# awaelchli/torch-optical-flow

Measured on AMD Instinct MI355X. Metric: image-pairs/sec + corr-lookup HBM GB/s, RAFT 12-iter @ Sintel 1024×436, higher is better.
Workload: dtype corr + convs split-fp16 (22-bit operands: fp16 hi + lo, 3 f16 MFMA per product, fp32 accumulate); lookup fp32; 1 GPU; raft-12iter-sintel-436x1024; pairs_per_gpu=8, global_batch=8, iters=12, padded=440x1024, parallelism=pairs sharded over 1 GPU(s), conv_benchmark=True, update_impl=split, hip_graph=True, steps_in_flight=1, full=False

## Files before the change

include/oflow.h:

```cpp
#ifndef OFLOW_H_
#define OFLOW_H_

#ifdef __cplusplus
extern "C" {
#endif

#define OFLOW_ABI_VERSION 1

#define OFLOW_OK 0
#define OFLOW_E_NULL (-1)
#define OFLOW_E_SHAPE (-2)
#define OFLOW_E_LEVELS (-3)
#define OFLOW_E_TINY (-4)
#define OFLOW_E_RADIUS (-5)
#define OFLOW_E_MODE (-6)
#define OFLOW_E_ALIGN (-7)

#define OFLOW_MAX_LEVELS 8
#define OFLOW_MAX_RADIUS 7

#define OFLOW_INTERP_BILINEAR 0
#define OFLOW_INTERP_NEAREST 1
#define OFLOW_INTERP_BICUBIC 2
#define OFLOW_PAD_ZEROS 0
#define OFLOW_PAD_BORDER 1
#define OFLOW_PAD_REFLECTION 2

#define OFLOW_IN_S32 0
#define OFLOW_IN_F32_NORM 1
#define OFLOW_IN_F32 2
#define OFLOW_IN_IMG7S2 3
#define OFLOW_IN_FLOW7 4
#define OFLOW_EPI_FLOW_HEAD 3

int oflow_abi_version(void);
const char* oflow_status_string(int status);

int oflow_corr_pyramid_dims(int H, int W, int num_levels, int* level_h, int* level_w);

int oflow_corr_pyramid_f32(const float* d_fmap1, const float* d_fmap2, int B, int C, int H, int W,
                           int num_levels, float* const* d_levels, void* stream);

int oflow_corr_lookup_f32(const float* const* d_levels, const int* level_h, const int* level_w,
                          int num_levels, const float* d_coords, int B, int H, int W, int radius,
                          float* d_out, void* stream);

long long oflow_corr_tiled_level_floats(int H_l, int W_l);
int oflow_corr_pyramid_tiled_f32(const float* d_fmap1, const float* d_fmap2, int B, int C, int H, int W,
                                 int num_levels, float* const* d_levels, void* stream);
int oflow_corr_pyramid_tiled_s32(const void* d_fmap1_s32, const void* d_fmap2_s32, int B, int C, int H, int W,
                                 int num_levels, float* const* d_levels, void* stream);
int oflow_corr_lookup_tiled_f32(const float* const* d_levels, const int* level_h, const int* level_w,
                                int num_levels, const float* d_coords, int B, int H, int W, int radius,
                                float* d_out, void* stream);
int oflow_corr_untile_f32(const float* d_tiled, float* d_out, long long Q, int H_l, int W_l, void* stream);

int oflow_grid_warp_f32(const float* d_frame, const float* d_flow, int B, int C, int H, int W, int mode,
                        int padding_mode, int align_corners, float* d_out, void* stream);

int oflow_grid_sample_f32(const float* d_input, const float* d_grid, int B, int C, int H, int W, int Ho, int Wo,
                          int mode, int padding_mode, int align_corners, float* d_out, void* stream);

int oflow_corr_otf_prepare_f16(const float* d_fmap1, const float* d_fmap2, int B, int C, int H, int W,
                               int num_levels, void* d_f1h, void* const* d_f2h, float* d_scratch, void* stream);
int oflow_corr_lookup_otf_f16(const void* d_f1h, const void* const* d_f2h, const int* level_h, const int* level_w,
                              int num_levels, const float* d_coords, int B, int C, int H, int W, int radius,
                              float* d_out, void* stream);

int oflow_bias_act_f32(const float* d_x, long long sx, const float* d_bias, float* d_y0, long long sy0, float* d_y1,
                       long long sy1, int B, int C, int P, int activation, float scale, void* stream);
int oflow_gru_reset_f32(const float* d_zr, long long szr, const float* d_br, const float* d_h, long long sh,
                        float* d_rh, long long srh, int B, int CH, int P, void* stream);
int oflow_gru_blend_f32(const float* d_zr, long long szr, const float* d_bz, const float* d_q, long long sq,
                        const float* d_bq, float* d_h, long long sh, int B, int CH, int P, void* stream);

int oflow_conv_s32(const void* d_x, long long x_pixel_stride, int in_groups, const void* d_wpack, int n_pad,
                   const float* d_wscale, const float* d_bias, int N, int B, int H, int W, int kh, int kw, int block_n,
                   int epilogue, int activation, float out_scale, void* d_y0, long long y0_pixel_stride, void* d_y1,
                   long long y1_pixel_stride, float* d_f32, long long f32_batch_stride, long long f32_channel_stride,
                   int f32_accumulate, float* d_gru_h, float* d_gru_z, int gru_channels, void* stream);
int oflow_pack_s32_f32(const float* d_x, long long x_batch_stride, int C, int B, int H, int W, int activation,
                       int dst_channel, void* d_y0, long long y0_pixel_stride, void* d_y1, long long y1_pixel_stride,
                       float* d_nhwc, int nhwc_pixel_stride, void* stream);
int oflow_flow_prep_s32(const float* d_coords, int B, int H, int W, void* d_patches, void* d_flow0,
                        long long flow0_pixel_stride, void* d_flow1, long long flow1_pixel_stride, void* stream);
int oflow_flow_head_col2im_f32(const float* d_y, const float* d_bias, int B, int H, int W, float* d_coords, void* stream);
int oflow_flow_head_finish_f32(const float* d_partial, int slabs, const float* d_bias, int B, int H, int W,
                               float* d_coords, void* d_flow0, long long flow0_pixel_stride, void* d_flow1,
                               long long flow1_pixel_stride, void* stream);

int oflow_normalize_images_f32(const float* d_x0, const float* d_x1, long long n, float* d_y0, float* d_y1, void* stream);

int oflow_replicate_pad_f32(const float* const* d_src, float* const* d_dst, int count, long long planes, int H, int W,
                            int top, int bottom, int left, int right, void* stream);

int oflow_set_range_flag(unsigned int* d_flag);

int oflow_range_flag_exchange(unsigned int* d_flag, unsigned int* d_out, void* stream);

int oflow_timing_event_create(void** ev);
int oflow_timing_event_destroy(void* ev);
int oflow_timing_event_record(void* ev, void* stream, int external);
int oflow_timing_event_elapsed_ms(void* start, void* end, float* ms);

int oflow_flow_head2_s32(const void* d_x, long long x_pixel_stride, int in_groups, const float* d_weight,
                         const float* d_bias, int B, int H, int W, float* d_coords, void* stream);
int oflow_flow_head2_tiled_s32(const void* d_x, long long x_pixel_stride, int in_groups, const float* d_wr,
                               const float* d_bias, int B, int H, int W, float* d_coords, void* stream);
int oflow_corr_lookup_tiled_nhwc_f32(const float* const* d_levels, const int* level_h, const int* level_w, int num_levels,
                                     const float* d_coords, int B, int H, int W, int radius, float* d_out, int row_floats,
                                     void* stream);
int oflow_corr_lookup_convc1_s32(const float* const* d_levels, const int* level_h, const int* level_w, int num_levels,
                                 const float* d_coords, int B, int H, int W, int radius, const void* d_wpack,
                                 const float* d_wscale, const float* d_bias, void* d_y, long long y_pixel_stride,
                                 void* stream);

int oflow_conv_s32_ex(const void* d_x, long long x_pixel_stride, int in_groups, const void* d_wpack, int n_pad,
                      const float* d_wscale, const float* d_bias, int N, int B, int H, int W, int kh, int kw,
                      int block_n, int epilogue, int activation, float out_scale, void* d_y0, long long y0_pixel_stride,
                      void* d_y1, long long y1_pixel_stride, float* d_f32, long long f32_batch_stride,
                      long long f32_channel_stride, int f32_accumulate, float* d_gru_h, float* d_gru_z,
                      int gru_channels, float* d_nhwc, int nhwc_pixel_stride, float* d_stats, const void* d_res,
                      long long res_pixel_stride, int res_activation, int s2d, void* stream);
int oflow_conv_s32_ex2(const void* d_x, long long x_pixel_stride, int in_groups, const void* d_wpack, int n_pad,
                       const float* d_wscale, const float* d_bias, int N, int B, int H, int W, int kh, int kw,
                       int block_n, int epilogue, int activation, float out_scale, void* d_y0, long long y0_pixel_stride,
                       void* d_y1, long long y1_pixel_stride, float* d_f32, long long f32_batch_stride,
                       long long f32_channel_stride, int f32_accumulate, float* d_gru_h, float* d_gru_z,
                       int gru_channels, float* d_nhwc, int nhwc_pixel_stride, float* d_stats, const void* d_res,
                       long long res_pixel_stride, int res_activation, int s2d, int in_format,
                       const float* d_in_scale, const float* d_in_shift, void* stream);
int oflow_conv_s32_ex3(const void* d_x, long long x_pixel_stride, int in_groups, const void* d_wpack, int n_pad,
                       const float* d_wscale, const float* d_bias, int N, int B, int H, int W, int kh, int kw,
                       int block_n, int epilogue, int activation, float out_scale, void* d_y0, long long y0_pixel_stride,
                       void* d_y1, long long y1_pixel_stride, float* d_f32, long long f32_batch_stride,
                       long long f32_channel_stride, int f32_accumulate, float* d_gru_h, float* d_gru_z,
                       int gru_channels, float* d_nhwc, int nhwc_pixel_stride, float* d_stats, const void* d_res,
                       long long res_pixel_stride, int res_activation, int s2d, int in_format,
                       const float* d_in_scale, const float* d_in_shift, const float* d_addend,
                       long long addend_pixel_stride, void* stream);
int oflow_conv_s32_ex4(const void* d_x, long long x_pixel_stride, int in_groups, const void* d_wpack, int n_pad,
                       const float* d_wscale, const float* d_bias, int N, int B, int H, int W, int kh, int kw,
                       int block_n, int epilogue, int activation, float out_scale, void* d_y0, long long y0_pixel_stride,
                       void* d_y1, long long y1_pixel_stride, float* d_f32, long long f32_batch_stride,
                       long long f32_channel_stride, int f32_accumulate, float* d_gru_h, float* d_gru_z,
                       int gru_channels, float* d_nhwc, int nhwc_pixel_stride, float* d_stats, const void* d_res,
                       long long res_pixel_stride, int res_activation, int s2d, int in_format,
                       const float* d_in_scale, const float* d_in_shift, const float* d_addend,
                       long long addend_pixel_stride, const void* d_wfrag, void* stream);
int oflow_conv_s32_ex5(const void* d_x, long long x_pixel_stride, int in_groups, const void* d_wpack, int n_pad,
                       const float* d_wscale, const float* d_bias, int N, int B, int H, int W, int kh, int kw,
                       int block_n, int epilogue, int activation, float out_scale, void* d_y0, long long y0_pixel_stride,
                       void* d_y1, long long y1_pixel_stride, float* d_f32, long long f32_batch_stride,
                       long long f32_channel_stride, int f32_accumulate, float* d_gru_h, float* d_gru_z,
                       int gru_channels, float* d_nhwc, int nhwc_pixel_stride, float* d_stats, const void* d_res,
                       long long res_pixel_stride, int res_activation, int s2d, int in_format,
                       const float* d_in_scale, const float* d_in_shift, const float* d_addend,
                       long long addend_pixel_stride, const void* d_wfrag, float* d_ksplit_slab,
                       unsigned* d_ksplit_ctr, long long ksplit_tiles, void* stream);
int oflow_conv_s32_ex6(const void* d_x, long long x_pixel_stride, int in_groups, const void* d_wpack, int n_pad,
                       const float* d_wscale, const float* d_bias, int N, int B, int H, int W, int kh, int kw,
                       int block_n, int epilogue, int activation, float out_scale, void* d_y0, long long y0_pixel_stride,
                       void* d_y1, long long y1_pixel_stride, float* d_f32, long long f32_batch_stride,
                       long long f32_channel_stride, int f32_accumulate, float* d_gru_h, float* d_gru_z,
                       int gru_channels, float* d_nhwc, int nhwc_pixel_stride, float* d_stats, const void* d_res,
                       long long res_pixel_stride, int res_activation, int s2d, int in_format,
                       const float* d_in_scale, const float* d_in_shift, const float* d_addend,
                       long long addend_pixel_stride, const void* d_wfrag, float* d_ksplit_slab,
                       unsigned* d_ksplit_ctr, long long ksplit_tiles, const float* d_fh_weights, float* d_fh_partial,
                       int fh_slabs, void* stream);
int oflow_stem_patches_s32(const float* d_img, int B, int C, int H, int W, void* d_out, int out_groups, void* stream);
int oflow_norm_stats_finalize(const float* d_partials, int B, int tiles, int n_pad, int C, double eps, float* d_alpha,
                              float* d_beta, void* stream);
int oflow_norm_apply_s32(const float* d_x, int C, int B, int H, int W, const float* d_alpha, const float* d_beta,
                         int activation, int res_mode, const void* d_res, long long res_pixel_stride, const float* d_x2,
                         const float* d_alpha2, const float* d_beta2, int res_activation, int s2d, void* d_y,
                         long long y_pixel_stride, void* stream);

int oflow_convex_upsample_f32(const float* d_flow, const float* d_mask, int B, int H, int W, float* d_out, void* stream);

int oflow_corr_lookup_backward_f32(const float* d_grad_out, const float* d_coords, int B, int H, int W, int radius,
                                   float* const* d_grad_levels, const int* level_h, const int* level_w, int num_levels,
                                   void* stream);
int oflow_corr_pyramid_grad_combine_f32(float* const* d_grad_levels, const int* level_h, const int* level_w,
                                        int num_levels, long long Q, void* stream);
int oflow_corr_fmap_grad_f32(const float* d_fmap1, const float* d_fmap2, const float* d_g0, int B, int C, int N,
                             float scale, float* d_grad_f1, float* d_grad_f2, void* stream);

int oflow_grid_warp_backward_f32(const float* d_grad_out, const float* d_frame, const float* d_flow, int B, int C, int H,
                                 int W, int mode, int padding_mode, int align_corners, float* d_grad_frame,
                                 float* d_grad_flow, void* stream);
int oflow_grid_sample_backward_f32(const float* d_grad_out, const float* d_input, const float* d_grid, int B, int C,
                                   int H, int W, int Ho, int Wo, int mode, int padding_mode, int align_corners,
                                   float* d_grad_input, float* d_grad_grid, void* stream);

#define OFLOW_FLOW_STATS_CHUNKS 128
#define OFLOW_FLOW2RGB_BAKER 0
#define OFLOW_FLOW2RGB_HSV 1
#define OFLOW_FLOW2RGB_MEISTER 2
int oflow_flow_stats_f32(const float* d_flow, int B, int H, int W, int clip, float clip_lo, float clip_hi,
                         int invert_y, float* d_partials, void* stream);
int oflow_flow2rgb_f32(const float* d_flow, int B, int H, int W, int method, int clip, float clip_lo, float clip_hi,
                       int invert_y, int have_denom, float denom, const float* d_partials, float* d_rgb, void* stream);
int oflow_flow_pack_f32(const float* d_flow, int B, int H, int W, int channels, int flip_rows, float* d_out,
                        void* stream);

#define OFLOW_FLOW_METRICS_PARTIALS 1024
#define OFLOW_MAX_PREDS 32
#define OFLOW_VALID_NONE 0
#define OFLOW_VALID_F32 1
#define OFLOW_VALID_U8 2
int oflow_flow_error_stats_f32(const float* d_pred, long long pred_sb, long long pred_sc, long long pred_sh,
                               const float* d_target, long long target_sb, long long target_sc, long long target_sh,
                               const void* d_valid, int valid_kind, long long valid_sb, long long valid_sh, int B, int H,
                               int W, float abs_threshold, float rel_threshold, float max_flow, float* d_epe_map,
                               double* d_workspace, double* d_accum, void* stream);
int oflow_sequence_loss_f32(const float* const* d_preds, int n_preds, const float* weights, const float* d_flow_gt,
                            const void* d_valid, int valid_kind, int B, int H, int W, float max_flow,
                            double* d_workspace, float* d_loss, double* d_stats, void* stream);
int oflow_sequence_loss_backward_f32(const float* d_grad_out, const float* const* d_preds, float* const* d_grads,
                                     int n_preds, const float* weights, const float* d_flow_gt, const void* d_valid,
                                     int valid_kind, int B, int H, int W, float max_flow, void* stream);

#ifdef __cplusplus
}
#endif

#endif
```

torch-optical-flow_amd/csrc/conv_s32.hip:

```cpp
#include "oflow_internal.h"

namespace oflow {
namespace {

typedef _Float16 half8 __attribute__((ext_vector_type(8)));
typedef float f32x16 __attribute__((ext_vector_type(16)));
typedef unsigned int u32x4 __attribute__((ext_vector_type(4)));

__device__ __forceinline__ int swz(int row) { return (row >> 1) & 7; }
#ifndef OFLOW_BREG_RING
#define OFLOW_BREG_RING 2
#endif
#ifndef OFLOW_VSLIDE
#define OFLOW_VSLIDE 1
#endif
#ifndef OFLOW_XCD_MAP
#define OFLOW_XCD_MAP 0
#endif
#ifndef OFLOW_STEM_SINGLE_A
#define OFLOW_STEM_SINGLE_A 1
#endif
#ifndef OFLOW_PAD_ROWS
#define OFLOW_PAD_ROWS 1
#endif
#ifndef OFLOW_HALO_DB
#define OFLOW_HALO_DB 0
#endif

constexpr int kTY = 4, kTX = 32;

#ifdef OFLOW_ABLATE
#define OFLOW_ABL(bit) ((a.exp_flags & (bit)) != 0)
#else
#define OFLOW_ABL(bit) false
#endif
constexpr int kAinGroups = 4;


struct ConvArgs {
  const uint8_t* x;
  long long xps;
  int kg;
  const uint8_t* w;
  int npad;
  const float* wsc;
  const float* bias;
  int N;
  int B, H, W, tiles_x, tiles_y;
  int act;
  float oscale;
  uint8_t* y0;
  long long y0ps;
  uint8_t* y1;
  long long y1ps;
  float* f;
  long long fbs, fcs;
  int faccum;
  float* h;
  float* z;
  int gch;
  const float* add;
  long long addps;
  float* fn;
  int fnps;
  float* stats;
  const uint8_t* res;
  long long resps;
  int res_act;
  int s2d;
  const float* ia;
  const float* ib;
  int ain;
  int cin;
  int wbytes;
  const uint8_t* wf;
  int exp_flags;
  float* ks_slab;
  unsigned* ks_ctr;
  long long ks_tiles;
  const float* fhw;
  float* fhy;
};
constexpr int kEpiFlowHead = OFLOW_EPI_FLOW_HEAD;
constexpr int kInS32 = OFLOW_IN_S32, kInF32Norm = OFLOW_IN_F32_NORM, kInF32 = OFLOW_IN_F32, kInImg = OFLOW_IN_IMG7S2,
              kInFlow = OFLOW_IN_FLOW7;
constexpr int kImgC = 3, kImgK = 7, kImgRows = (kTY - 1) * 2 + kImgK, kImgCols = (kTX - 1) * 2 + kImgK;
constexpr int kImgHalf = (kImgCols + 1) / 2, kImgPitch = 2 * kImgHalf, kImgPlane = kImgRows * kImgPitch;

__device__ __forceinline__ float sigmoid_hw(float v) {
  return __builtin_amdgcn_rcpf(1.0f + __builtin_amdgcn_exp2f(v * -1.4426950408889634f));
}
__device__ __forceinline__ float tanh_hw(float v) {
  return 1.0f - 2.0f * __builtin_amdgcn_rcpf(__builtin_amdgcn_exp2f(v * 2.8853900817779268f) + 1.0f);
}

__device__ __forceinline__ float act_fn(float v, int act) {
  if (act == 1) return v < 0.f ? 0.f : v;
  if (act == 2) return 1.0f / (1.0f + expf(-v));
  if (act == 3) return tanhf(v);
  return v;
}

__device__ __forceinline__ void split8(const float* v, half8& hi, half8& lo) { split_vec(v, hi, lo); }

__device__ __forceinline__ void store_s32(uint8_t* y, long long ps, long long P, int n, int N, const float* v, float& gm) {
  uint8_t* line = y + P * ps + (long long)(n >> 5) * 128 + ((n & 31) >> 3) * 16;
  if (n + 8 <= N) {
    half8 hi, lo;
    split8(v, hi, lo);
    gm = fmaxf(gm, fmaxf(fmaxf(fmaxf(fabsf(v[0]), fabsf(v[1])), fmaxf(fabsf(v[2]), fabsf(v[3]))),
                         fmaxf(fmaxf(fabsf(v[4]), fabsf(v[5])), fmaxf(fabsf(v[6]), fabsf(v[7])))));
    *reinterpret_cast<half8*>(line) = hi;
    *reinterpret_cast<half8*>(line + 64) = lo;
  } else {
    _Float16* hp = reinterpret_cast<_Float16*>(line);
    _Float16* lp = reinterpret_cast<_Float16*>(line + 64);
#pragma unroll
    for (int j = 0; j < 8; ++j) {
      if (n + j < N) {
        gm = fmaxf(gm, fabsf(v[j]));
        _Float16 h_, l_;
        split_f16(v[j], h_, l_);
        hp[j] = h_;
        lp[j] = l_;
      }
    }
  }
}

typedef __attribute__((address_space(4))) const float cfloat;
template <int T0, int T1>
__device__ __forceinline__ void flow_head_partials(const float* tp, cfloat* w, float* yp, long long plane, bool in) {
  constexpr int NO = 2 * (T1 - T0);
  float acc[2][NO];
#pragma unroll
  for (int j = 0; j < NO; ++j) acc[0][j] = acc[1][j] = 0.f;
  float wn[2][NO];
#pragma unroll
  for (int e = 0; e < 2; ++e)
#pragma unroll
    for (int j = 0; j < NO; ++j) wn[e][j] = w[e * 18 + 2 * T0 + j];
  float2 tn = *reinterpret_cast<const float2*>(tp);
#pragma unroll
  for (int e = 0; e < 2; ++e)
#pragma unroll
    for (int j = 0; j < NO; ++j) asm volatile("" : "+s"(wn[e][j]));
  asm volatile("" : "+v"(tn.x), "+v"(tn.y));
#pragma unroll 2
  for (int c0 = 0; c0 < 64; c0 += 2) {
    float wc[2][NO];
#pragma unroll
    for (int e = 0; e < 2; ++e)
#pragma unroll
      for (int j = 0; j < NO; ++j) wc[e][j] = wn[e][j];
    const float2 t = tn;
    const int c1 = c0 + 2 < 64 ? c0 + 2 : c0;
#pragma unroll
    for (int e = 0; e < 2; ++e)
#pragma unroll
      for (int j = 0; j < NO; ++j) wn[e][j] = w[(c1 + e) * 18 + 2 * T0 + j];
    tn = *reinterpret_cast<const float2*>(tp + c1);
    __builtin_amdgcn_sched_barrier(0);
#pragma unroll
    for (int j = 0; j < NO; ++j) {
      acc[0][j] = fmaf(t.x, wc[0][j], acc[0][j]);
      acc[1][j] = fmaf(t.y, wc[1][j], acc[1][j]);
    }
    __builtin_amdgcn_sched_barrier(0);
#pragma unroll
    for (int e = 0; e < 2; ++e)
#pragma unroll
      for (int j = 0; j < NO; ++j) asm volatile("" : "+s"(wn[e][j]));
    asm volatile("" : "+v"(tn.x), "+v"(tn.y));
  }
  if (in) {
#pragma unroll
    for (int j = 0; j < NO; ++j) yp[(2 * T0 + j) * plane] = acc[0][j] + acc[1][j];
  }
}

template <int KH, int KW, int BN, int WM, int WN, int EPI, int TY = kTY, int AIN = kInS32, bool BREG = false, int BD = 1>
__global__ __launch_bounds__(64 * WM * WN, WM * WN == 8 ? 1 : 2) void conv_s32_kernel(ConvArgs a) {
  constexpr int NTH = 64 * WM * WN;
  constexpr int T = KH * KW;
  constexpr int BM = TY * kTX;
  constexpr int PH = KH / 2, PW = KW / 2;
  constexpr int HY = TY + KH - 1, HX = kTX + KW - 1, NPIX = HY * HX;
  constexpr int AITEMS = NPIX * 8, APER = (AITEMS + NTH - 1) / NTH;
  constexpr int BITEMS = BN * 8, BPER = (BITEMS + NTH - 1) / NTH;
  constexpr int MT = TY / WM;
  constexpr int NT = BN / WN / 32;
  static_assert((WM * WN == 4 || WM * WN == 8) && MT >= 1 && NT >= 1, "bad wave grid");
  static_assert(NTH % 8 == 0, "an A item's 16-B chunk is tid & 7");
  constexpr bool WIN = AIN == kInImg || AIN == kInFlow;
  constexpr int WC = AIN == kInFlow ? 2 : kImgC, WS = AIN == kInFlow ? 1 : 2;
  constexpr int WROWS = (kTY - 1) * WS + kImgK, WCOLS = (kTX - 1) * WS + kImgK;
  constexpr int WHALF = WS == 2 ? (WCOLS + 1) / 2 : WCOLS, WPITCH = WS == 2 ? 2 * WHALF : WCOLS;
  constexpr int WPLANE = WROWS * WPITCH;
  constexpr int WKPAD = AIN == kInFlow ? 128 : 160;
  constexpr int WAPER = WIN ? BM * 4 / NTH : 1;
  static_assert(!WIN || (BM * 4) % NTH == 0, "window items");
  static_assert(AIN != kInImg || (WHALF == kImgHalf && WPITCH == kImgPitch && WPLANE == kImgPlane), "stem window");
  constexpr bool ADB = (T == 1) && !(WIN && OFLOW_STEM_SINGLE_A);
  constexpr int RS = 128;
  constexpr int RSA = (BREG || OFLOW_PAD_ROWS) ? 144 : RS, RSB = OFLOW_PAD_ROWS ? 144 : RS;
  constexpr int A_BYTES = NPIX * RSA, B_BYTES = BN * RSB;
  static_assert(!BREG || (T > 1 && (WM == 1 || WM == 2 || WM == 4) && BN == 32 * WN && AIN == kInS32),
                "register-direct B: T > 1, WM x WN waves of one 32-channel tile each");
  constexpr bool HDB = BREG && OFLOW_HALO_DB;
  constexpr int MAIN_BYTES = ((ADB || HDB) ? 2 : 1) * A_BYTES + (BREG ? 0 : 2 * B_BYTES);
  constexpr int TS = BN + 4;
  constexpr int EPI_BYTES = BM * TS * 4;
  constexpr int LDS_BYTES = MAIN_BYTES > EPI_BYTES ? MAIN_BYTES : EPI_BYTES;
  constexpr int kImgZero = WC * WPLANE;
  constexpr int IMG_FLOATS = (kImgZero + 1 + 3) & ~3;
  constexpr int AFF_BYTES = AIN == kInF32Norm ? kAinGroups * 32 * 8
                            : WIN ? IMG_FLOATS * 4 + WKPAD * 4
                            : 0;
  static_assert(!WIN || (T == 1 && TY == kTY), "window input: 1x1 geometry over the patch channels, 4-row tiles");
  __shared__ __attribute__((aligned(16))) uint8_t smem[LDS_BYTES + AFF_BYTES];
  __shared__ float2 sSB[BN];
  __shared__ float3 sStat[EPI == 0 ? WM * BN : 1];
  float2* sAff = reinterpret_cast<float2*>(smem + LDS_BYTES);
  float* sImg = reinterpret_cast<float*>(smem + LDS_BYTES);
  int* sKoff = reinterpret_cast<int*>(smem + LDS_BYTES + (WIN ? IMG_FLOATS * 4 : 0));
  uint8_t* sA = smem;
  uint8_t* sB = smem + (ADB ? 2 : 1) * A_BYTES;

  const int tid = threadIdx.x, lane = tid & 63, wave = tid >> 6;
  const int wm = wave / WN, wn = wave % WN;
  const int r = lane & 31, hh = lane >> 5;
  if constexpr (BREG) {
    if (a.ks_slab != nullptr) {
      const int z = blockIdx.z;
      a.x += (long long)z * a.kg * 128;
      a.wf += (long long)z * a.kg * T * a.npad * 128;
    }
  }
  auto aswz = [](int p) { return (BREG || OFLOW_PAD_ROWS) ? 0 : swz(p); };
  auto bswz = [](int n) { return OFLOW_PAD_ROWS ? 0 : swz(n); };

  int tile, cblk;
  if constexpr (OFLOW_XCD_MAP) {
    const int nblk = a.npad / BN, ntiles = a.tiles_x * a.tiles_y * a.B, bid = blockIdx.x;
    const int full = (ntiles >> 3) * 8 * nblk;
    if (bid < full) {
      const int grp = bid / (8 * nblk), rem = bid - grp * 8 * nblk;
      cblk = rem >> 3;
      tile = grp * 8 + (rem & 7);
    } else {
      const int ntail = ntiles & 7, rem = bid - full;
      cblk = rem / ntail;
      tile = (ntiles & ~7) + (rem - cblk * ntail);
    }
  } else {
    tile = blockIdx.x;
    cblk = blockIdx.y;
  }
  const int tx0 = (tile % a.tiles_x) * kTX;
  tile /= a.tiles_x;
  const int ty0 = (tile % a.tiles_y) * TY;
  const int b = tile / a.tiles_y;
  const int n0 = cblk * BN;
  const long long pix0 = (long long)b * a.H * a.W;

  u32x4 ra[APER], rb[BPER];
  const __amdgpu_buffer_rsrc_t rsA = __builtin_amdgcn_make_buffer_rsrc(
      const_cast<uint8_t*>(a.x + pix0 * a.xps), (short)0, (int)((long long)a.H * a.W * a.xps), 0x00020000);
  const __amdgpu_buffer_rsrc_t rsB =
      __builtin_amdgcn_make_buffer_rsrc(const_cast<uint8_t*>(a.w), (short)0, a.wbytes, 0x00020000);
  auto a_off = [&](int s_, int& col) {
    int t_ = tid;
    asm volatile("" : "+v"(t_));
    const int item = (AITEMS % NTH == 0) ? t_ + s_ * NTH : min(t_ + s_ * NTH, AITEMS - 1);
    const int p = item >> 3, c = item & 7;
    const int gy = ty0 - PH + p / HX, gx = tx0 - PW + p % HX;
    const int cy = min(max(gy, 0), a.H - 1), cx = min(max(gx, 0), a.W - 1);
    col = c * 16;
    return (cy * a.W + cx) * (int)a.xps + (AIN == kInF32 ? 0 : c * 16);
  };
  unsigned aok = 0u;
#pragma unroll
  for (int s_ = 0; s_ < APER; ++s_) {
    const int item = (AITEMS % NTH == 0) ? tid + s_ * NTH : min(tid + s_ * NTH, AITEMS - 1);
    const int p = item >> 3;
    const int gy = ty0 - PH + p / HX, gx = tx0 - PW + p % HX;
    const bool ok = static_cast<unsigned>(gy) < static_cast<unsigned>(a.H) && static_cast<unsigned>(gx) < static_cast<unsigned>(a.W);
    aok |= (ok ? 1u : 0u) << s_;
  }
  int boff[BPER];
#pragma unroll
  for (int s_ = 0; s_ < BPER; ++s_) boff[s_] = (n0 + (tid + s_ * NTH) / 8) * 128 + ((tid + s_ * NTH) & 7) * 16;
#define OFLOW_LOAD_A(RA, G)                                                                                          \
  if constexpr (!WIN) _Pragma("unroll") for (int s_ = 0; s_ < APER; ++s_) {                                        \
    int col_;                                                                                                        \
    const int off_ = a_off(s_, col_);                                                                                \
    if constexpr (AIN == kInF32)    \
      RA[s_] = __builtin_amdgcn_raw_buffer_load_b128(rsA, off_ + min((G) * 128 + col_, a.cin * 4 - 16), 0, 0);      \
    else                                                                                                             \
      RA[s_] = __builtin_amdgcn_raw_buffer_load_b128(rsA, off_, (G) * 128, 0);                                      \
  }
#define OFLOW_WRITE_A(RA, BUF, G)                                                                                    \
  if (!OFLOW_ABL(4)) {                                                                                               \
  float amx_ = 0.f;                                                                                                  \
  float2 af4_[4];                                                                                                    \
  if constexpr (AIN == kInF32Norm) _Pragma("unroll") for (int e_ = 0; e_ < 4; ++e_)                                  \
    af4_[e_] = sAff[(G) * 32 + 4 * (tid & 7) + e_];                                                                  \
  if constexpr (WIN) {                                                                                               \
                                                                                                        \
    _Pragma("unroll") for (int s_ = 0; s_ < WAPER; ++s_) {                                                           \
      const int item = tid + s_ * NTH;                                                                               \
      const int p = item % BM, cp = item / BM;                                                                       \
      const int pb_ = WS * (p >> 5) * WPITCH + (p & 31);                                                             \
      const int4 k0_ = *reinterpret_cast<const int4*>(sKoff + (G) * 32 + 8 * cp);                                    \
      const int4 k1_ = *reinterpret_cast<const int4*>(sKoff + (G) * 32 + 8 * cp + 4);                                \
      const int kov_[8] = {k0_.x, k0_.y, k0_.z, k0_.w, k1_.x, k1_.y, k1_.z, k1_.w};                                  \
      float v8_[8];                                                                                                  \
      _Pragma("unroll") for (int e_ = 0; e_ < 8; ++e_) {                                                             \
        v8_[e_] = sImg[kov_[e_] < 0 ? kImgZero : pb_ + kov_[e_]];                                                    \
        amx_ = fmaxf(amx_, fabsf(v8_[e_]));                                                                          \
      }                                                                                                              \
      half8 h8_, l8_;                                                                                                \
      split_vec(v8_, h8_, l8_);                                                                                      \
      uint8_t* rw_ = sA + (BUF) * A_BYTES + p * RSA;                                                                 \
      *reinterpret_cast<half8*>(rw_ + ((cp ^ aswz(p)) << 4)) = h8_;                                                  \
      *reinterpret_cast<half8*>(rw_ + (((4 + cp) ^ aswz(p)) << 4)) = l8_;                                            \
    }                                                                                                                \
  } else                                                                                                             \
  _Pragma("unroll") for (int s_ = 0; s_ < APER; ++s_) {                                                              \
    const int item = tid + s_ * NTH;                                                                            \
                                                     \
    const int p = item >> 3, c = item & 7;                                                                           \
    if (AITEMS % NTH == 0 || item < AITEMS) {                                                                   \
      if constexpr (AIN != kInS32) {                                                                                 \
                   \
        typedef _Float16 half4_ __attribute__((ext_vector_type(4)));                                                 \
        half4_ h4 = {0, 0, 0, 0}, l4 = {0, 0, 0, 0};                                                                 \
        if (((aok >> s_) & 1u) && (AIN != kInF32 || (G) * 32 + 4 * c < a.cin)) {                                     \
          const float* fv = reinterpret_cast<const float*>(&RA[s_]);                                                 \
          float mx_ = 0.f, v4_[4];                                                                                   \
          _Pragma("unroll") for (int e_ = 0; e_ < 4; ++e_) {                                                         \
            float v_ = fv[e_];                                                                                       \
            if constexpr (AIN == kInF32Norm) {                                                                       \
              const float2 af = af4_[e_];                                                                            \
              v_ = v_ * af.x + af.y;                                                                                 \
              v_ = v_ < 0.f ? 0.f : v_;                                                                              \
            }                                                                                                        \
            mx_ = fmaxf(mx_, fabsf(v_));                                                                             \
            v4_[e_] = v_;                                                                                            \
          }                                                                                                          \
          split_vec(v4_, h4, l4);                                                                                    \
          amx_ = fmaxf(amx_, mx_);                                                                                   \
        }                                                                                                            \
        uint8_t* rw_ = sA + (BUF) * A_BYTES + p * RSA + (c & 1) * 8;                                                 \
        *reinterpret_cast<half4_*>(rw_ + (((c >> 1) ^ aswz(p)) << 4)) = h4;                                          \
        *reinterpret_cast<half4_*>(rw_ + (((4 + (c >> 1)) ^ aswz(p)) << 4)) = l4;                                    \
      } else {                                                                                                       \
        *reinterpret_cast<u32x4*>(sA + (BUF) * A_BYTES + p * RSA + ((c ^ aswz(p)) << 4)) =                          \
            ((aok >> s_) & 1u) ? RA[s_] : u32x4{0u, 0u, 0u, 0u};                                                     \
      }                                                                                                              \
    }                                                                                                                \
  }                                                                                                                  \
  if constexpr (AIN != kInS32) range_guard(amx_);                                                                    \
  }
#define OFLOW_LOAD_B(RB, STEP)                                                                                       \
  _Pragma("unroll") for (int s_ = 0; s_ < BPER; ++s_) {                                                              \
    const int item = tid + s_ * NTH;                                                                            \
    if (BITEMS % NTH == 0 || item < BITEMS)                                                                     \
      RB[s_] = __builtin_amdgcn_raw_buffer_load_b128(rsB, boff[s_], (STEP) * a.npad * 128, 0);                      \
  }
#define OFLOW_WRITE_B(RB, BUF)                                                                                       \
  if (!OFLOW_ABL(32)) _Pragma("unroll") for (int s_ = 0; s_ < BPER; ++s_) {                                          \
    const int item = tid + s_ * NTH;                                                                            \
    const int n = item >> 3, c = item & 7;                                                                           \
    if (BITEMS % NTH == 0 || item < BITEMS)                                                                     \
      *reinterpret_cast<u32x4*>(sB + (BUF) * B_BYTES + n * RSB + ((c ^ bswz(n)) << 4)) = RB[s_];                    \
  }
#define OFLOW_READ_OPS(AH, AL, BH, BL, I, S_)                                                                        \
  {                                                                                                                  \
    const int ii_ = (I);                                                                                              \
    const int t_ = ii_ % T, ky_ = t_ / KW, kx_ = t_ - ky_ * KW;                                                       \
    const uint8_t* bufA_ = sA + (ADB ? (ii_ & 1) * A_BYTES : 0);                                                      \
    const uint8_t* bufB_ = sB + (ii_ & 1) * B_BYTES;                                                                  \
    const int chi_ = 2 * (S_) + hh, clo_ = 4 + 2 * (S_) + hh;                                                        \
    _Pragma("unroll") for (int mt_ = 0; mt_ < MT; ++mt_) {                                                           \
      const int p_ = (wm * MT + mt_ + ky_) * HX + r + kx_;                                                           \
      const uint8_t* row_ = bufA_ + p_ * RSA;                                                                        \
      AH[mt_] = *reinterpret_cast<const half8*>(row_ + ((chi_ ^ aswz(p_)) << 4));                                    \
      AL[mt_] = *reinterpret_cast<const half8*>(row_ + ((clo_ ^ aswz(p_)) << 4));                                    \
    }                                                                                                                \
    _Pragma("unroll") for (int nt_ = 0; nt_ < NT; ++nt_) {                                                           \
      const int n_ = wn * (BN / WN) + nt_ * 32 + r;                                                                  \
      const uint8_t* row_ = bufB_ + n_ * RSB;                                                                        \
      BH[nt_] = *reinterpret_cast<const half8*>(row_ + ((chi_ ^ bswz(n_)) << 4));                                    \
      BL[nt_] = *reinterpret_cast<const half8*>(row_ + ((clo_ ^ bswz(n_)) << 4));                                    \
    }                                                                                                                \
  }
#define OFLOW_MFMAS(AH, AL, BH, BL)                                                                                  \
  if (!OFLOW_ABL(2)) _Pragma("unroll") for (int mt = 0; mt < MT; ++mt)                                               \
    _Pragma("unroll") for (int nt = 0; nt < NT; ++nt) {                                                              \
      acc[mt][nt] = __builtin_amdgcn_mfma_f32_32x32x16_f16(AH[mt], BL[nt], acc[mt][nt], 0, 0, 0);                    \
      acc[mt][nt] = __builtin_amdgcn_mfma_f32_32x32x16_f16(AL[mt], BH[nt], acc[mt][nt], 0, 0, 0);                    \
      acc[mt][nt] = __builtin_amdgcn_mfma_f32_32x32x16_f16(AH[mt], BH[nt], acc[mt][nt], 0, 0, 0);                    \
    }

  f32x16 acc[MT][NT];
#pragma unroll
  for (int i = 0; i < MT; ++i)
#pragma unroll
    for (int j = 0; j < NT; ++j)
#pragma unroll
      for (int e = 0; e < 16; ++e) acc[i][j][e] = 0.f;

  const int S = a.kg * T;
  for (int c = tid; c < BN; c += NTH) {
    const int n = min(n0 + c, a.N - 1);
    sSB[c] = make_float2(a.wsc[n], a.bias ? a.bias[n] : 0.f);
  }
  if constexpr (AIN == kInF32Norm) {
    for (int e = tid; e < a.kg * 32; e += NTH)
      sAff[e] = make_float2(a.ia[(long long)b * a.kg * 32 + e], a.ib[(long long)b * a.kg * 32 + e]);
    __syncthreads();
  }
  if constexpr (AIN == kInImg) {
    const float* img = reinterpret_cast<const float*>(a.x) + (long long)b * kImgC * (2 * a.H) * (2 * a.W);
    const int iy0 = 2 * ty0 - kImgK / 2, ix0 = 2 * tx0 - kImgK / 2;
    constexpr int IMG_N = kImgC * kImgRows * kImgCols, IMG_PER = (IMG_N + NTH - 1) / NTH;
    if (a.exp_flags & 1) {
      for (int e = tid; e < IMG_N; e += NTH) {
        const int ch = e / (kImgRows * kImgCols), rem = e - ch * (kImgRows * kImgCols);
        const int ry = rem / kImgCols, rx = rem - ry * kImgCols;
        const int iy = iy0 + ry, ix = ix0 + rx;
        float v = 0.f;
        if (static_cast<unsigned>(iy) < static_cast<unsigned>(2 * a.H) && static_cast<unsigned>(ix) < static_cast<unsigned>(2 * a.W))
          v = img[((long long)ch * (2 * a.H) + iy) * (2 * a.W) + ix];
        sImg[ch * kImgPlane + ry * kImgPitch + (rx & 1) * kImgHalf + (rx >> 1)] = v;
      }
    } else {
    float iv[IMG_PER];
    int io[IMG_PER];
#pragma unroll
    for (int s_ = 0; s_ < IMG_PER; ++s_) {
      const int e = min(tid + s_ * NTH, IMG_N - 1);
      const int ch = e / (kImgRows * kImgCols), rem = e - ch * (kImgRows * kImgCols);
      const int ry = rem / kImgCols, rx = rem - ry * kImgCols;
      const int iy = iy0 + ry, ix = ix0 + rx;
      const bool in = static_cast<unsigned>(iy) < static_cast<unsigned>(2 * a.H) && static_cast<unsigned>(ix) < static_cast<unsigned>(2 * a.W);
      const int cy = min(max(iy, 0), 2 * a.H - 1), cx = min(max(ix, 0), 2 * a.W - 1);
      const float v = img[((long long)ch * (2 * a.H) + cy) * (2 * a.W) + cx];
      iv[s_] = in ? v : 0.f;
      io[s_] = ch * kImgPlane + ry * kImgPitch + (rx & 1) * kImgHalf + (rx >> 1);
    }
#pragma unroll
    for (int s_ = 0; s_ < IMG_PER; ++s_)
      if (tid + s_ * NTH < IMG_N) sImg[io[s_]] = iv[s_];
    }
  }
  if constexpr (AIN == kInFlow) {
    const float* co = reinterpret_cast<const float*>(a.x) + (long long)b * 2 * a.H * a.W;
    const int iy0 = ty0 - kImgK / 2, ix0 = tx0 - kImgK / 2;
    constexpr int FL_N = 2 * WROWS * WCOLS, FL_PER = (FL_N + NTH - 1) / NTH;
    float iv[FL_PER];
    int io[FL_PER];
#pragma unroll
    for (int s_ = 0; s_ < FL_PER; ++s_) {
      const int e = min(tid + s_ * NTH, FL_N - 1);
      const int ch = e / (WROWS * WCOLS), rem = e - ch * (WROWS * WCOLS);
      const int ry = rem / WCOLS, rx = rem - ry * WCOLS;
      const int iy = iy0 + ry, ix = ix0 + rx;
      const bool in = static_cast<unsigned>(iy) < static_cast<unsigned>(a.H) && static_cast<unsigned>(ix) < static_cast<unsigned>(a.W);
      const int cy = min(max(iy, 0), a.H - 1), cx = min(max(ix, 0), a.W - 1);
      const float v = co[((long long)ch * a.H + cy) * a.W + cx] - static_cast<float>(ch == 0 ? ix : iy);
      iv[s_] = in ? v : 0.f;
      io[s_] = ch * WPLANE + ry * WPITCH + rx;
    }
#pragma unroll
    for (int s_ = 0; s_ < FL_PER; ++s_)
      if (tid + s_ * NTH < FL_N) sImg[io[s_]] = iv[s_];
  }
  if constexpr (WIN) {
    for (int k = tid; k < WKPAD; k += NTH) {
      const int t = k / WC, ch = k - t * WC;
      const int ky = t / kImgK, kx = t - ky * kImgK;
      sKoff[k] = t < kImgK * kImgK
                     ? ch * WPLANE + ky * WPITCH + (WS == 2 ? (kx & 1) * WHALF + (kx >> 1) : kx)
                     : -1;
    }
    if (tid == 0) sImg[kImgZero] = 0.f;
    __syncthreads();
  }
  if constexpr (BREG) {
  const __amdgpu_buffer_rsrc_t rsW =
      __builtin_amdgcn_make_buffer_rsrc(const_cast<uint8_t*>(a.wf), (short)0, a.wbytes, 0x00020000);
  const int wlane = ((n0 >> 5) + wn) * 4096 + lane * 16;
  const int wstep = a.npad * 128;
  constexpr int RING = (T == 5 && KH == 5 && EPI == 0) ? 2 : OFLOW_BREG_RING;
  u32x4 bq[RING][4];
  auto load_b = [&](u32x4 (&d)[4], int step) {
#pragma unroll
    for (int e = 0; e < 4; ++e) d[e] = __builtin_amdgcn_raw_buffer_load_b128(rsW, wlane + e * 1024, step * wstep, 0);
  };
#define OFLOW_READ_A(AH, AL, I, S_)                                                                                   \
  {                                                                                                                  \
    const int ii_ = (I);                                                                                              \
    const int t_ = ii_ % T, ky_ = t_ / KW, kx_ = t_ - ky_ * KW;                                                       \
    const int chi_ = 2 * (S_) + hh, clo_ = 4 + 2 * (S_) + hh;                                                        \
    const uint8_t* sAb_ = sA + (HDB && ((ii_ / T) & 1) ? A_BYTES : 0);           \
    _Pragma("unroll") for (int mt_ = 0; mt_ < MT; ++mt_) {                                                           \
      const int p_ = (wm * MT + mt_ + ky_) * HX + r + kx_;                                                           \
      const uint8_t* row_ = sAb_ + p_ * RSA;                                                                         \
      AH[mt_] = *reinterpret_cast<const half8*>(row_ + (chi_ << 4));                                                 \
      AL[mt_] = *reinterpret_cast<const half8*>(row_ + (clo_ << 4));                                                 \
    }                                                                                                                \
  }
#define OFLOW_MFMAS_R(AH, AL, BC, S_)                                                                                 \
  if (!OFLOW_ABL(2)) _Pragma("unroll") for (int mt = 0; mt < MT; ++mt) {                                             \
    const half8 bh_ = __builtin_bit_cast(half8, BC[2 * (S_)]), bl_ = __builtin_bit_cast(half8, BC[2 * (S_) + 1]);     \
    acc[mt][0] = __builtin_amdgcn_mfma_f32_32x32x16_f16(AH[mt], bl_, acc[mt][0], 0, 0, 0);                           \
    acc[mt][0] = __builtin_amdgcn_mfma_f32_32x32x16_f16(AL[mt], bh_, acc[mt][0], 0, 0, 0);                           \
    acc[mt][0] = __builtin_amdgcn_mfma_f32_32x32x16_f16(AH[mt], bh_, acc[mt][0], 0, 0, 0);                           \
  }
#pragma unroll
  for (int q = 0; q < RING; ++q) load_b(bq[q], q < S ? q : S - 1);
  OFLOW_LOAD_A(ra, 0);
  OFLOW_WRITE_A(ra, 0, 0);
  OFLOW_LOAD_A(ra, a.kg > 1 ? 1 : 0);
  __syncthreads();
  constexpr int GPB = (T % RING == 0) ? 1 : RING;
  constexpr bool VSLIDE = OFLOW_VSLIDE && KW == 1 && KH > 1 && WM == 1 && !(EPI == 0 && KH == 5);
  if constexpr (VSLIDE) {
    constexpr int NR = MT + KH - 1;
    half8 V[NR][2][2];
    auto rd = [&](int hr, int sub, int grp) {
      const uint8_t* row_ = sA + (HDB && (grp & 1) ? A_BYTES : 0) + (hr * HX + r) * RSA;
      V[hr][sub][0] = *reinterpret_cast<const half8*>(row_ + ((2 * sub + hh) << 4));
      V[hr][sub][1] = *reinterpret_cast<const half8*>(row_ + ((4 + 2 * sub + hh) << 4));
    };
    auto mf = [&](int ky, int sub, u32x4 (&bc)[4]) {
      if (OFLOW_ABL(2)) return;
      const half8 bh_ = __builtin_bit_cast(half8, bc[2 * sub]), bl_ = __builtin_bit_cast(half8, bc[2 * sub + 1]);
#pragma unroll
      for (int mt = 0; mt < MT; ++mt) {
        acc[mt][0] = __builtin_amdgcn_mfma_f32_32x32x16_f16(V[mt + ky][sub][0], bl_, acc[mt][0], 0, 0, 0);
        acc[mt][0] = __builtin_amdgcn_mfma_f32_32x32x16_f16(V[mt + ky][sub][1], bh_, acc[mt][0], 0, 0, 0);
        acc[mt][0] = __builtin_amdgcn_mfma_f32_32x32x16_f16(V[mt + ky][sub][0], bh_, acc[mt][0], 0, 0, 0);
      }
    };
#pragma unroll
    for (int m = 0; m < MT; ++m) rd(m, 0, 0);
    for (int g0 = 0; g0 < a.kg; g0 += GPB) {
#pragma unroll
      for (int j = 0; j < GPB * T; ++j) {
        const int gg = g0 + j / T, t = j % T;
        if (GPB > 1 && j > 0 && t == 0 && gg >= a.kg) break;
        const int i_ = gg * T + t;
        u32x4 (&bc)[4] = bq[j % RING];
        if (t == 0) {
#pragma unroll
          for (int m = 0; m < MT; ++m) rd(m, 1, gg);
        } else {
          rd(t + MT - 1, 1, gg);
        }
        mf(t, 0, bc);
        if (t == T - 1) {
          if constexpr (HDB) {
            OFLOW_WRITE_A(ra, (gg + 1) & 1, gg + 1 < a.kg ? gg + 1 : gg);
          } else {
            __syncthreads();
            OFLOW_WRITE_A(ra, 0, gg + 1 < a.kg ? gg + 1 : gg);
          }
          const int g2 = gg + 2 < a.kg ? gg + 2 : a.kg - 1;
          OFLOW_LOAD_A(ra, g2);
          __syncthreads();
#pragma unroll
          for (int m = 0; m < MT; ++m) rd(m, 0, gg + 1);
        } else {
          rd(t + MT, 0, gg);
        }
        mf(t, 1, bc);
        load_b(bc, i_ + RING < S ? i_ + RING : S - 1);
      }
    }
  } else {
  half8 xah[MT], xal[MT], yah[MT], yal[MT];
  OFLOW_READ_A(xah, xal, 0, 0);
  for (int g0 = 0; g0 < a.kg; g0 += GPB) {
#pragma unroll
    for (int j = 0; j < GPB * T; ++j) {
      const int gg = g0 + j / T, t = j % T;
      if (GPB > 1 && j > 0 && t == 0 && gg >= a.kg) break;
      const int i_ = gg * T + t;
      u32x4 (&bc)[4] = bq[j % RING];
      OFLOW_READ_A(yah, yal, i_, 1);
      OFLOW_MFMAS_R(xah, xal, bc, 0);
      if (t == T - 1) {
        if constexpr (HDB) {
          OFLOW_WRITE_A(ra, (gg + 1) & 1, gg + 1 < a.kg ? gg + 1 : gg);
        } else {
          __syncthreads();
          OFLOW_WRITE_A(ra, 0, gg + 1 < a.kg ? gg + 1 : gg);
        }
        const int g2 = gg + 2 < a.kg ? gg + 2 : a.kg - 1;
        OFLOW_LOAD_A(ra, g2);
        __syncthreads();
      }
      OFLOW_READ_A(xah, xal, i_ + 1, 0);
      OFLOW_MFMAS_R(yah, yal, bc, 1);
      load_b(bc, i_ + RING < S ? i_ + RING : S - 1);
    }
  }
  }
#undef OFLOW_READ_A
#undef OFLOW_MFMAS_R
  } else {
  u32x4 rbr[BD][BPER];
  u32x4 rar[ADB ? BD : 1][APER];
  OFLOW_LOAD_B(rbr[0], 0);
  OFLOW_LOAD_A(rar[0], 0);
  OFLOW_WRITE_A(rar[0], 0, 0);
  OFLOW_WRITE_B(rbr[0], 0);
#pragma unroll
  for (int d = 1; d <= BD; ++d) {
    const int id = d < S ? d : S - 1;
    OFLOW_LOAD_B(rbr[d % BD], id);
    if constexpr (ADB) { OFLOW_LOAD_A(rar[d % BD], id); }
  }
  if constexpr (!ADB) { OFLOW_LOAD_A(rar[0], a.kg > 1 ? 1 : 0); }
  __syncthreads();
  half8 xah[MT], xal[MT], xbh[NT], xbl[NT];
  half8 yah[MT], yal[MT], ybh[NT], ybl[NT];
  OFLOW_READ_OPS(xah, xal, xbh, xbl, 0, 0);

  constexpr int GPB2 = (BD > 1 && (T % BD) != 0) ? BD : 1;
  for (int g0 = 0; g0 < a.kg; g0 += GPB2) {
#pragma unroll
    for (int j = 0; j < GPB2 * T; ++j) {
      const int g = g0 + j / T, t = j % T;
      if (GPB2 > 1 && j > 0 && t == 0 && g >= a.kg) break;
      const int i_ = g * T + t;
      u32x4 (&rb)[BPER] = rbr[(j + 1) % BD];
      OFLOW_WRITE_B(rb, (i_ + 1) & 1);
      if constexpr (ADB) { OFLOW_WRITE_A(rar[(j + 1) % BD], (i_ + 1) & 1, i_ + 1 < S ? i_ + 1 : S - 1); }
      {
        const int i2 = i_ + 1 + BD < S ? i_ + 1 + BD : S - 1;
        OFLOW_LOAD_B(rb, i2);
        if constexpr (ADB) { OFLOW_LOAD_A(rar[(j + 1) % BD], i2); }
      }
      OFLOW_READ_OPS(yah, yal, ybh, ybl, i_, 1);
      OFLOW_MFMAS(xah, xal, xbh, xbl);
      if constexpr (!ADB) {
        if (t == T - 1) {
          __syncthreads();
          OFLOW_WRITE_A(rar[0], 0, g + 1 < a.kg ? g + 1 : g);
          const int g2 = g + 2 < a.kg ? g + 2 : a.kg - 1;
          OFLOW_LOAD_A(rar[0], g2);
        }
      }
      if (!OFLOW_ABL(64)) __syncthreads();
      OFLOW_READ_OPS(xah, xal, xbh, xbl, i_ + 1, 0);
      OFLOW_MFMAS(yah, yal, ybh, ybl);
    }
  }
  }
#undef OFLOW_MFMAS
#undef OFLOW_READ_OPS
#undef OFLOW_LOAD_A
#undef OFLOW_WRITE_A
#undef OFLOW_LOAD_B
#undef OFLOW_WRITE_B

  if constexpr (BREG) {
    if (a.ks_slab != nullptr) {
      typedef __attribute__((address_space(1))) unsigned gu32;
      __shared__ unsigned sTicket;
      const int tile_id = blockIdx.y * gridDim.x + blockIdx.x;
      gu32* ctr = (gu32*)(a.ks_ctr) + 2 * tile_id;
      if (tid == 0) sTicket = __hip_atomic_fetch_add(ctr, 1u, __ATOMIC_RELAXED, __HIP_MEMORY_SCOPE_AGENT);
      __syncthreads();
      const unsigned ticket = sTicket;
      const __amdgpu_buffer_rsrc_t rsS = __builtin_amdgcn_make_buffer_rsrc(
          a.ks_slab + (size_t)tile_id * (BM * BN), (short)0, BM * BN * 4, 0x00020000);
      const int sbase = wave * (MT * NT * 4096) + lane * 16;
      if ((ticket & 1u) == 0u) {
#pragma unroll
        for (int mt = 0; mt < MT; ++mt)
#pragma unroll
          for (int nt = 0; nt < NT; ++nt)
#pragma unroll
            for (int e4 = 0; e4 < 4; ++e4) {
              const u32x4 v = {__float_as_uint(acc[mt][nt][4 * e4]), __float_as_uint(acc[mt][nt][4 * e4 + 1]),
                               __float_as_uint(acc[mt][nt][4 * e4 + 2]), __float_as_uint(acc[mt][nt][4 * e4 + 3])};
              __builtin_amdgcn_raw_buffer_store_b128(v, rsS, sbase + ((mt * NT + nt) * 4 + e4) * 1024, 0, 16);
            }
        asm volatile("s_waitcnt vmcnt(0)" ::: "memory");
        __syncthreads();
        if (tid == 0) __hip_atomic_fetch_add(ctr + 1, 1u, __ATOMIC_RELAXED, __HIP_MEMORY_SCOPE_AGENT);
        return;
      }
      if (tid == 0) {
        const unsigned want = (ticket >> 1) + 1u;
        for (unsigned spin = 0; spin < (1u << 24); ++spin) {
          if (static_cast<int>(__hip_atomic_load(ctr + 1, __ATOMIC_RELAXED, __HIP_MEMORY_SCOPE_AGENT) - want) >= 0) break;
          __builtin_amdgcn_s_sleep(1);
        }
        __builtin_amdgcn_fence(__ATOMIC_ACQUIRE, "agent");
        asm volatile("s_waitcnt vmcnt(0)" ::: "memory");
      }
      __syncthreads();
#pragma unroll
      for (int mt = 0; mt < MT; ++mt)
#pragma unroll
        for (int nt = 0; nt < NT; ++nt) {
          u32x4 pv[4];
#pragma unroll
          for (int e4 = 0; e4 < 4; ++e4)
            pv[e4] = __builtin_amdgcn_raw_buffer_load_b128(rsS, sbase + ((mt * NT + nt) * 4 + e4) * 1024, 0, 0);
#pragma unroll
          for (int e4 = 0; e4 < 4; ++e4)
#pragma unroll
            for (int j = 0; j < 4; ++j) acc[mt][nt][4 * e4 + j] += __uint_as_float(pv[e4][j]);
        }
    }
  }

  constexpr int C8 = BN / 8;
  constexpr int KIT = (BM * C8 + NTH - 1) / NTH;
  constexpr bool GRU = EPI == 1 || EPI == 2;
  const bool has_add = GRU && a.add != nullptr;
  u32x4 ad[GRU ? KIT : 1][2];
  if (has_add) {
#pragma unroll
    for (int k = 0; k < (GRU ? KIT : 0); ++k) {
      const int item = tid + k * NTH;
      const int pl = item / C8, n = n0 + (item - pl * C8) * 8;
      const int y = ty0 + pl / kTX, x = tx0 + (pl % kTX);
      if (item >= BM * C8 || n >= a.N || y >= a.H || x >= a.W) continue;
      const u32x4* ap = reinterpret_cast<const u32x4*>(a.add + (pix0 + (long long)y * a.W + x) * a.addps + n);
      ad[k][0] = ap[0];
      ad[k][1] = ap[1];
    }
  }
  __syncthreads();
  float* sT = reinterpret_cast<float*>(smem);
#pragma unroll
  for (int mt = 0; mt < MT; ++mt)
#pragma unroll
    for (int nt = 0; nt < NT; ++nt) {
      const int nl = wn * (BN / WN) + nt * 32 + r;
      const int pbase = (wm * MT + mt) * kTX;
      if constexpr (EPI == kEpiFlowHead) {
        const float2 sb = sSB[nl];
#pragma unroll
        for (int e = 0; e < 16; ++e) {
          const int m = (e & 3) + 8 * (e >> 2) + 4 * hh;
          const float v = fmaf(acc[mt][nt][e], sb.x, sb.y);
          sT[(pbase + m) * TS + nl] = v < 0.f ? 0.f : v;
        }
      } else {
#pragma unroll
      for (int e = 0; e < 16; ++e) {
        const int m = (e & 3) + 8 * (e >> 2) + 4 * hh;
        sT[(pbase + m) * TS + nl] = acc[mt][nt][e];
      }
      }
    }
  if constexpr (EPI == 0 && TY >= kTY) {
    if (a.stats != nullptr && !OFLOW_ABL(8)) {
#pragma unroll
      for (int nt = 0; nt < NT; ++nt) {
        const int nl = wn * (BN / WN) + nt * 32 + r;
        const float2 sb = sSB[nl];
        float cnt = 0.f, sum = 0.f, q = 0.f;
        const bool full = ty0 + TY <= a.H && tx0 + kTX <= a.W;
        if (full) {
#pragma unroll
          for (int mt = 0; mt < MT; ++mt)
#pragma unroll
            for (int e = 0; e < 16; ++e) sum += acc[mt][nt][e] * sb.x + sb.y;
          cnt = 16.f * MT;
        } else {
#pragma unroll
          for (int mt = 0; mt < MT; ++mt) {
            const bool yok = ty0 + wm * MT + mt < a.H;
#pragma unroll
            for (int e = 0; e < 16; ++e) {
              const bool ok = yok && tx0 + (e & 3) + 8 * (e >> 2) + 4 * hh < a.W;
              sum += ok ? acc[mt][nt][e] * sb.x + sb.y : 0.f;
              cnt += ok ? 1.f : 0.f;
            }
          }
        }
        const float mean = cnt > 0.f ? sum / cnt : 0.f;
        if (full) {
#pragma unroll
          for (int mt = 0; mt < MT; ++mt)
#pragma unroll
            for (int e = 0; e < 16; ++e) {
              const float d = (acc[mt][nt][e] * sb.x + sb.y) - mean;
              float dd = d * d;
              asm volatile("" : "+v"(dd));
              q += dd;
            }
        } else {
#pragma unroll
          for (int mt = 0; mt < MT; ++mt) {
            const bool yok = ty0 + wm * MT + mt < a.H;
#pragma unroll
            for (int e = 0; e < 16; ++e) {
              const bool ok = yok && tx0 + (e & 3) + 8 * (e >> 2) + 4 * hh < a.W;
              const float d = (acc[mt][nt][e] * sb.x + sb.y) - mean;
              q += ok ? d * d : 0.f;
            }
          }
        }
        const float nb = __shfl_xor(cnt, 32), mb = __shfl_xor(mean, 32), qb = __shfl_xor(q, 32);
        const float n0_ = hh ? nb : cnt, m0_ = hh ? mb : mean, q0_ = hh ? qb : q;
        const float n1_ = hh ? cnt : nb, m1_ = hh ? mean : mb, q1_ = hh ? q : qb;
        const float nn = n0_ + n1_;
// ... 89 lines not shown
          float N0 = 0.f, M0 = 0.f, Q0 = 0.f;
#pragma unroll
          for (int j = 0; j < WPS; ++j) {
            const float3 t = sStat[(sub * WPS + j) * BN + c];
            const float nn = N0 + t.x;
            if (t.x > 0.f) {
              if (N0 > 0.f) {
                const float d = t.y - M0;
                M0 = M0 + d * (t.x / nn);
                Q0 = Q0 + t.z + d * d * (N0 * t.x / nn);
              } else {
                M0 = t.y;
                Q0 = t.z;
              }
              N0 = nn;
            }
          }
          if (n < a.N && ty0 + sub * kTY < a.H) {
            const int tiles4_y = (a.H + kTY - 1) / kTY;
            const int tile_in_img = (ty0 / kTY + sub) * a.tiles_x + tx0 / kTX;
            float* st = a.stats + (((long long)b * a.tiles_x * tiles4_y + tile_in_img) * a.npad + n) * 3;
            st[0] = N0;
            st[1] = M0;
            st[2] = Q0;
          }
        }
      }
    }
    if ((a.y0 == nullptr && a.fn == nullptr) || OFLOW_ABL(16)) return;
  }

  if (OFLOW_ABL(16)) return;
  u32x4 pre[EPI == 0 ? 1 : KIT][EPI == 2 ? 4 : 2];
#pragma unroll
  for (int k = 0; k < (EPI == 0 ? 0 : KIT); ++k) {
    const int item = tid + k * NTH;
    const int pl = item / C8, nl = (item - pl * C8) * 8, n = n0 + nl;
    const int y = ty0 + pl / kTX, x = tx0 + (pl % kTX);
    if (item >= BM * C8 || n >= a.N || y >= a.H || x >= a.W) continue;
    const long long P = pix0 + (long long)y * a.W + x;
    if constexpr (EPI == 1) {
      if (n >= a.gch) {
        const u32x4* hp = reinterpret_cast<const u32x4*>(a.h + P * a.gch + (n - a.gch));
        pre[k][0] = hp[0];
        pre[k][1] = hp[1];
      }
    } else if constexpr (EPI == 2) {
      const u32x4* hp = reinterpret_cast<const u32x4*>(a.h + P * a.gch + n);
      const u32x4* zp = reinterpret_cast<const u32x4*>(a.z + P * a.gch + n);
      pre[k][0] = hp[0];
      pre[k][1] = hp[1];
      pre[k][2] = zp[0];
      pre[k][3] = zp[1];
    }
  }
  const bool hwx = (a.exp_flags & 256) == 0;
  constexpr int UNR = EPI == 0 ? 1 : KIT;
  float gmx = 0.f;
  constexpr bool FIXED_OCT = NTH % C8 == 0;
  float2 sbv[8];
  if constexpr (FIXED_OCT) {
#pragma unroll
    for (int j = 0; j < 8; ++j) sbv[j] = sSB[(tid % C8) * 8 + j];
  }
#pragma unroll UNR
  for (int k = 0; k < KIT; ++k) {
    const int item = tid + k * NTH;
    const int pl = item / C8, c8 = item - pl * C8;
    const int nl = c8 * 8, n = n0 + nl;
    const int y = ty0 + pl / kTX, x = tx0 + (pl % kTX);
    if (item >= BM * C8 || n >= a.N || y >= a.H || x >= a.W) continue;
    const long long P = pix0 + (long long)y * a.W + x;
    const float* pf = reinterpret_cast<const float*>(&pre[EPI == 0 ? 0 : k][0]);
    const float4 t0 = *reinterpret_cast<const float4*>(&sT[pl * TS + nl]);
    const float4 t1 = *reinterpret_cast<const float4*>(&sT[pl * TS + nl + 4]);
    float v[8] = {t0.x, t0.y, t0.z, t0.w, t1.x, t1.y, t1.z, t1.w};
    if (!has_add) {
#pragma unroll
      for (int j = 0; j < 8; ++j) {
        const float2 sb = FIXED_OCT ? sbv[j] : sSB[nl + j];
        v[j] = v[j] * sb.x + sb.y;
      }
    }
    if constexpr (EPI == 0) {
#pragma unroll
      for (int j = 0; j < 8; ++j) v[j] = act_fn(v[j], a.act) * a.oscale;
      if (a.res) {
        const uint8_t* rl = a.res + P * a.resps + (long long)(n >> 5) * 128 + ((n & 31) >> 3) * 16;
        const half8 rh = *reinterpret_cast<const half8*>(rl), rlo = *reinterpret_cast<const half8*>(rl + 64);
#pragma unroll
        for (int j = 0; j < 8; ++j) {
          v[j] = v[j] + (static_cast<float>(rh[j]) + static_cast<float>(rlo[j]));
          if (a.res_act) v[j] = act_fn(v[j], a.res_act);
        }
      }
      if (a.fn) {
        float* fp = a.fn + P * a.fnps + n;
        if (n + 8 <= a.N) {
          *reinterpret_cast<float4*>(fp) = make_float4(v[0], v[1], v[2], v[3]);
          *reinterpret_cast<float4*>(fp + 4) = make_float4(v[4], v[5], v[6], v[7]);
        } else {
#pragma unroll
          for (int j = 0; j < 8; ++j)
            if (n + j < a.N) fp[j] = v[j];
        }
      }
      if (a.y0) {
        long long Pd = P;
        int nd = n;
        if (a.s2d) {
          const int W2 = a.W >> 1, H2 = a.H >> 1;
          Pd = ((long long)b * H2 + (y >> 1)) * W2 + (x >> 1);
          nd = n + ((y & 1) * 2 + (x & 1)) * a.N;
        }
        store_s32(a.y0, a.y0ps, Pd, nd, a.s2d ? 4 * a.N : a.N, v, gmx);
        if (a.y1) store_s32(a.y1, a.y1ps, Pd, nd, a.s2d ? 4 * a.N : a.N, v, gmx);
      }
    } else if constexpr (EPI == 1) {
      if (n < a.gch) {
        float4* zp = reinterpret_cast<float4*>(a.z + P * a.gch + n);
        float zv[8];
#pragma unroll
        for (int j = 0; j < 8; ++j) zv[j] = hwx ? sigmoid_hw(v[j]) : 1.0f / (1.0f + expf(-v[j]));
        zp[0] = make_float4(zv[0], zv[1], zv[2], zv[3]);
        zp[1] = make_float4(zv[4], zv[5], zv[6], zv[7]);
      } else {
        float rh[8];
#pragma unroll
        for (int j = 0; j < 8; ++j) rh[j] = (hwx ? sigmoid_hw(v[j]) : 1.0f / (1.0f + expf(-v[j]))) * pf[j];
        store_s32(a.y0, a.y0ps, P, n - a.gch, a.gch, rh, gmx);
      }
    } else {
      float* hp = a.h + P * a.gch + n;
      float hn[8];
#pragma unroll
      for (int j = 0; j < 8; ++j) {
        const float q = hwx ? tanh_hw(v[j]) : tanhf(v[j]);
        const float z = pf[8 + j];
        hn[j] = (1.0f - z) * pf[j] + z * q;
      }
#pragma unroll
      for (int j = 0; j < 8; ++j) hp[j] = hn[j];
      store_s32(a.y0, a.y0ps, P, n, a.N, hn, gmx);
    }
  }
  range_guard(gmx);
}

inline dim3 conv_grid(const ConvArgs& a, int bn) {
  const int ntiles = a.tiles_x * a.tiles_y * a.B;
  return OFLOW_XCD_MAP ? dim3(ntiles * (a.npad / bn)) : dim3(ntiles, a.npad / bn);
}

template <int KH, int KW, int BN, int WM, int WN, int EPI, int TY, int AIN>
void launch_staged(const ConvArgs& a, dim3 grid, hipStream_t s) {
  hipLaunchKernelGGL((conv_s32_kernel<KH, KW, BN, WM, WN, EPI, TY, AIN, false, 2>), grid, dim3(64 * WM * WN), 0, s, a);
}

template <int KH, int KW, int BN, int WM, int WN, int EPI, int TY = kTY, bool BREG = false>
int launch_conv(const ConvArgs& a0, hipStream_t s) {
  ConvArgs a = a0;
  if constexpr (BREG) {
    a.tiles_y = (a.H + TY - 1) / TY;
    dim3 grid = conv_grid(a, BN);
    if (a.ks_slab != nullptr) {
      if (OFLOW_XCD_MAP || (long long)grid.x * grid.y > a.ks_tiles) return OFLOW_E_SHAPE;
      grid.z = 2;
    }
    hipLaunchKernelGGL((conv_s32_kernel<KH, KW, BN, WM, WN, EPI, TY, kInS32, true>), grid, dim3(64 * WM * WN), 0, s, a);
    return launch_status();
  } else {
  a.tiles_y = (a.H + TY - 1) / TY;
  dim3 grid = conv_grid(a, BN);
  if constexpr (KH == 3 && KW == 3 && EPI == 0) {
    if (a.ain == kInF32Norm) {
      launch_staged<KH, KW, BN, WM, WN, EPI, TY, kInF32Norm>(a, grid, s);
      return launch_status();
    }
  }
  if constexpr (KH == 1 && KW == 1 && EPI == 0 && BN == 64 && TY == kTY) {
    if (a.ain == kInImg) {
      launch_staged<KH, KW, BN, WM, WN, EPI, TY, kInImg>(a, grid, s);
      return launch_status();
    }
  }
  if constexpr (KH == 1 && KW == 1 && EPI == 0 && BN == 128 && TY == kTY) {
    if (a.ain == kInFlow) {
      launch_staged<KH, KW, BN, WM, WN, EPI, TY, kInFlow>(a, grid, s);
      return launch_status();
    }
  }
  if constexpr (KH == 1 && KW == 1 && EPI == 0 && BN == 128) {
    if (a.ain == kInF32) {
      launch_staged<KH, KW, BN, WM, WN, EPI, TY, kInF32>(a, grid, s);
      return launch_status();
    }
  }
  if (a.ain != kInS32) return OFLOW_E_MODE;
  launch_staged<KH, KW, BN, WM, WN, EPI, TY, kInS32>(a, grid, s);
  return launch_status();
  }
}

int g_small_grid_px = 16384;
int g_stats_8row = 1;
int g_conv_exp_flags = 0;
int g_bn64_8row = 0;
inline bool small_grid(const ConvArgs& a, int bn) {
  return (long long)a.B * a.H * a.W < g_small_grid_px && a.stats == nullptr && a.ain == kInS32 && a.npad % 64 == 0 &&
         bn >= 64 && a.ks_slab == nullptr;
}

inline bool use_breg(const ConvArgs& a, int bn, int taps) {
  return a.wf != nullptr && (bn == 128 || bn == 64 || bn == 32) && taps > 1 && a.ain == kInS32 && a.stats == nullptr &&
         !small_grid(a, bn);
}

template <int KH, int KW, int EPI>
int launch_bn(const ConvArgs& a, int bn, hipStream_t s) {
  if (small_grid(a, bn)) return launch_conv<KH, KW, 64, 2, 2, EPI, 2>(a, s);
  if constexpr (KH * KW > 1 && KH * KW != 4)
    if (use_breg(a, bn, KH * KW)) {
      if (bn == 128) return launch_conv<KH, KW, 128, 1, 4, EPI, kTY, true>(a, s);
      if constexpr (KH == 3 && KW == 3) {
        if (bn == 64) return launch_conv<KH, KW, 64, 2, 2, EPI, kTY, true>(a, s);
        return launch_conv<KH, KW, 32, 4, 1, EPI, kTY, true>(a, s);
      }
    }
  switch (bn) {
    case 128: return launch_conv<KH, KW, 128, 2, 2, EPI>(a, s);
    case 96: return launch_conv<KH, KW, 96, 4, 1, EPI>(a, s);
    case 64:
      if constexpr (KH * KW > 1)
        if (a.stats == nullptr ? g_bn64_8row != 0 : g_stats_8row != 0) return launch_conv<KH, KW, 64, 4, 1, EPI, 8>(a, s);
      return launch_conv<KH, KW, 64, 2, 2, EPI>(a, s);
    case 32: return launch_conv<KH, KW, 32, 4, 1, EPI>(a, s);
    default: return OFLOW_E_SHAPE;
  }
}

int dispatch_conv(const ConvArgs& a, int kh, int kw, int block_n, int epilogue, hipStream_t s) {
  const int key = kh * 16 + kw;
  switch (epilogue) {
    case 0:
      switch (key) {
        case 0x11: return launch_bn<1, 1, 0>(a, block_n, s);
        case 0x22: return launch_bn<2, 2, 0>(a, block_n, s);
        case 0x33: return launch_bn<3, 3, 0>(a, block_n, s);
        case 0x15: return launch_bn<1, 5, 0>(a, block_n, s);
        case 0x51: return launch_bn<5, 1, 0>(a, block_n, s);
        default: return OFLOW_E_SHAPE;
      }
    case 1:
      if (block_n != 128) return OFLOW_E_SHAPE;
      if (small_grid(a, block_n)) {
        if (key == 0x15) return launch_conv<1, 5, 64, 2, 2, 1, 2>(a, s);
        if (key == 0x51) return launch_conv<5, 1, 64, 2, 2, 1, 2>(a, s);
      }
      if (use_breg(a, block_n, kh * kw)) {
        if (key == 0x15) return launch_conv<1, 5, 128, 1, 4, 1, kTY, true>(a, s);
        if (key == 0x51) return launch_conv<5, 1, 128, 1, 4, 1, kTY, true>(a, s);
      }
      if (key == 0x15) return launch_conv<1, 5, 128, 2, 2, 1>(a, s);
      if (key == 0x51) return launch_conv<5, 1, 128, 2, 2, 1>(a, s);
      return OFLOW_E_SHAPE;
    case kEpiFlowHead:
      if (key != 0x33) return OFLOW_E_SHAPE;
      if (block_n == 64) return launch_conv<3, 3, 64, 2, 2, kEpiFlowHead>(a, s);
      if (block_n == 128) return a.wf != nullptr ? launch_conv<3, 3, 128, 1, 4, kEpiFlowHead, kTY, true>(a, s) : OFLOW_E_MODE;
      return OFLOW_E_SHAPE;
    default:
      if (block_n != 128) return OFLOW_E_SHAPE;
      if (small_grid(a, block_n)) {
        if (key == 0x15) return launch_conv<1, 5, 64, 2, 2, 2, 2>(a, s);
        if (key == 0x51) return launch_conv<5, 1, 64, 2, 2, 2, 2>(a, s);
      }
      if (use_breg(a, block_n, kh * kw)) {
        if (key == 0x15) return launch_conv<1, 5, 128, 1, 4, 2, kTY, true>(a, s);
        if (key == 0x51) return launch_conv<5, 1, 128, 1, 4, 2, kTY, true>(a, s);
      }
      if (key == 0x15) return launch_conv<1, 5, 128, 2, 2, 2>(a, s);
      if (key == 0x51) return launch_conv<5, 1, 128, 2, 2, 2>(a, s);
      return OFLOW_E_SHAPE;
  }
}

int build_conv_args(ConvArgs& a, const void* d_x, long long x_pixel_stride, int in_groups, const void* d_wpack,
                    int n_pad, const float* d_wscale, const float* d_bias, int N, int B, int H, int W, int kh, int kw,
                    int block_n, int epilogue, int activation, float out_scale, void* d_y0, long long y0_pixel_stride,
                    void* d_y1, long long y1_pixel_stride, float* d_f32, long long f32_batch_stride,
                    long long f32_channel_stride, int f32_accumulate, float* d_gru_h, float* d_gru_z, int gru_channels,
                    float* d_nhwc, int nhwc_pixel_stride, float* d_stats, const void* d_res, long long res_pixel_stride,
                    int res_activation, int s2d) {
  if (!d_x || !d_wpack || !d_wscale) return OFLOW_E_NULL;
  if (B <= 0 || H <= 0 || W <= 0 || N <= 0 || in_groups <= 0 || n_pad < N || n_pad % block_n) return OFLOW_E_SHAPE;
  if (activation < 0 || activation > 3 || res_activation < 0 || res_activation > 3 || epilogue < 0 || epilogue > 2)
    return OFLOW_E_MODE;
  if ((x_pixel_stride & 15) || ((uintptr_t)d_x & 15) || ((uintptr_t)d_wpack & 15)) return OFLOW_E_ALIGN;
  if (epilogue == 0 && !d_y0 && !d_f32 && !d_nhwc && !d_stats) return OFLOW_E_NULL;
  if (epilogue != 0 && (!d_y0 || !d_gru_h || !d_gru_z || gru_channels <= 0 || gru_channels % 8)) return OFLOW_E_NULL;
  if (epilogue != 0 && (((uintptr_t)d_gru_h & 15) || ((uintptr_t)d_gru_z & 15))) return OFLOW_E_ALIGN;
  if (epilogue == 1 && N != 2 * gru_channels) return OFLOW_E_SHAPE;
  if (epilogue == 2 && N != gru_channels) return OFLOW_E_SHAPE;
  if (epilogue != 0 && (d_nhwc || d_stats || d_res || s2d)) return OFLOW_E_MODE;
  if (s2d && ((H | W) & 1 || N % 8)) return OFLOW_E_SHAPE;
  if (d_nhwc && (nhwc_pixel_stride < N || ((uintptr_t)d_nhwc & 15) || (nhwc_pixel_stride & 3))) return OFLOW_E_ALIGN;
  if ((d_y0 && ((y0_pixel_stride & 127) || ((uintptr_t)d_y0 & 15))) ||
      (d_y1 && ((y1_pixel_stride & 127) || ((uintptr_t)d_y1 & 15))) ||
      (d_res && ((res_pixel_stride & 127) || ((uintptr_t)d_res & 15))))
    return OFLOW_E_ALIGN;
  a = ConvArgs{};
  a.x = static_cast<const uint8_t*>(d_x);
  a.xps = x_pixel_stride;
  a.kg = in_groups;
  a.w = static_cast<const uint8_t*>(d_wpack);
  a.npad = n_pad;
  a.wsc = d_wscale;
  a.bias = d_bias;
  a.N = N;
  a.B = B;
  a.H = H;
  a.W = W;
  a.tiles_x = (W + kTX - 1) / kTX;
  a.tiles_y = (H + kTY - 1) / kTY;
  a.act = activation;
  a.oscale = out_scale;
  a.y0 = static_cast<uint8_t*>(d_y0);
  a.y0ps = y0_pixel_stride;
  a.y1 = static_cast<uint8_t*>(d_y1);
  a.y1ps = y1_pixel_stride;
  a.f = d_f32;
  a.fbs = f32_batch_stride;
  a.fcs = f32_channel_stride;
  a.faccum = f32_accumulate;
  a.h = d_gru_h;
  a.z = d_gru_z;
  a.gch = gru_channels;
  a.fn = d_nhwc;
  a.fnps = nhwc_pixel_stride;
  a.stats = d_stats;
  a.res = static_cast<const uint8_t*>(d_res);
  a.resps = res_pixel_stride;
  a.res_act = res_activation;
  a.s2d = s2d;
  a.cin = in_groups * 32;
  const long long wbytes = (long long)in_groups * kh * kw * n_pad * 128;
  if (wbytes >= (1ll << 31) || (long long)H * W * x_pixel_stride >= (1ll << 31)) return OFLOW_E_SHAPE;
  a.wbytes = static_cast<int>(wbytes);
  a.exp_flags = g_conv_exp_flags;
  (void)block_n;
  return OFLOW_OK;
}

}
OFLOW_RANGE_FLAG_SETTER(conv)
}

using namespace oflow;

extern "C" int oflow_conv_s32_ex5(const void* d_x, long long x_pixel_stride, int in_groups, const void* d_wpack,
                                  int n_pad, const float* d_wscale, const float* d_bias, int N, int B, int H, int W, int kh,
                                  int kw, int block_n, int epilogue, int activation, float out_scale, void* d_y0,
                                  long long y0_pixel_stride, void* d_y1, long long y1_pixel_stride, float* d_f32,
                                  long long f32_batch_stride, long long f32_channel_stride, int f32_accumulate,
                                  float* d_gru_h, float* d_gru_z, int gru_channels, float* d_nhwc, int nhwc_pixel_stride,
                                  float* d_stats, const void* d_res, long long res_pixel_stride, int res_activation,
                                  int s2d, int in_format, const float* d_in_scale, const float* d_in_shift,
                                  const float* d_addend, long long addend_pixel_stride, const void* d_wfrag,
                                  float* d_ksplit_slab, unsigned* d_ksplit_ctr, long long ksplit_tiles, void* stream);

extern "C" int oflow_conv_s32_ex4(const void* d_x, long long x_pixel_stride, int in_groups, const void* d_wpack,
                                  int n_pad, const float* d_wscale, const float* d_bias, int N, int B, int H, int W, int kh,
                                  int kw, int block_n, int epilogue, int activation, float out_scale, void* d_y0,
                                  long long y0_pixel_stride, void* d_y1, long long y1_pixel_stride, float* d_f32,
                                  long long f32_batch_stride, long long f32_channel_stride, int f32_accumulate,
                                  float* d_gru_h, float* d_gru_z, int gru_channels, float* d_nhwc, int nhwc_pixel_stride,
                                  float* d_stats, const void* d_res, long long res_pixel_stride, int res_activation,
                                  int s2d, int in_format, const float* d_in_scale, const float* d_in_shift,
                                  const float* d_addend, long long addend_pixel_stride, const void* d_wfrag, void* stream) {
  return oflow_conv_s32_ex5(d_x, x_pixel_stride, in_groups, d_wpack, n_pad, d_wscale, d_bias, N, B, H, W, kh, kw,
                            block_n, epilogue, activation, out_scale, d_y0, y0_pixel_stride, d_y1, y1_pixel_stride,
                            d_f32, f32_batch_stride, f32_channel_stride, f32_accumulate, d_gru_h, d_gru_z, gru_channels,
                            d_nhwc, nhwc_pixel_stride, d_stats, d_res, res_pixel_stride, res_activation, s2d, in_format,
                            d_in_scale, d_in_shift, d_addend, addend_pixel_stride, d_wfrag, nullptr, nullptr, 0, stream);
}

extern "C" int oflow_conv_s32_ex5(const void* d_x, long long x_pixel_stride, int in_groups, const void* d_wpack,
                                  int n_pad, const float* d_wscale, const float* d_bias, int N, int B, int H, int W, int kh,
                                  int kw, int block_n, int epilogue, int activation, float out_scale, void* d_y0,
                                  long long y0_pixel_stride, void* d_y1, long long y1_pixel_stride, float* d_f32,
                                  long long f32_batch_stride, long long f32_channel_stride, int f32_accumulate,
                                  float* d_gru_h, float* d_gru_z, int gru_channels, float* d_nhwc, int nhwc_pixel_stride,
                                  float* d_stats, const void* d_res, long long res_pixel_stride, int res_activation,
                                  int s2d, int in_format, const float* d_in_scale, const float* d_in_shift,
                                  const float* d_addend, long long addend_pixel_stride, const void* d_wfrag,
                                  float* d_ksplit_slab, unsigned* d_ksplit_ctr, long long ksplit_tiles, void* stream) {
  ConvArgs a;
  const int st = build_conv_args(a, d_x, x_pixel_stride, in_groups, d_wpack, n_pad, d_wscale, d_bias, N, B, H, W, kh, kw,
                                 block_n, epilogue, activation, out_scale, d_y0, y0_pixel_stride, d_y1, y1_pixel_stride,
                                 d_f32, f32_batch_stride, f32_channel_stride, f32_accumulate, d_gru_h, d_gru_z,
                                 gru_channels, d_nhwc, nhwc_pixel_stride, d_stats, d_res, res_pixel_stride,
                                 res_activation, s2d);
  if (st != OFLOW_OK) return st;
  if (d_wfrag) {
    if ((uintptr_t)d_wfrag & 15) return OFLOW_E_ALIGN;
    if (n_pad % 32) return OFLOW_E_SHAPE;
    a.wf = static_cast<const uint8_t*>(d_wfrag);
  }
  if (in_format < kInS32 || in_format > kInFlow) return OFLOW_E_MODE;
  if (in_format == kInFlow) {
    if (kh != 1 || kw != 1 || epilogue != 0 || block_n != 128 || in_groups != (kImgK * kImgK * 2 + 31) / 32)
      return OFLOW_E_MODE;
    if ((long long)2 * B * H * W >= (1ll << 31) || d_addend) return OFLOW_E_SHAPE;
    a.ain = in_format;
    return dispatch_conv(a, kh, kw, block_n, epilogue, static_cast<hipStream_t>(stream));
  }
  if (in_format == kInImg) {
    if (kh != 1 || kw != 1 || epilogue != 0 || block_n != 64 || in_groups != (kImgK * kImgK * kImgC + 31) / 32)
      return OFLOW_E_MODE;
    if ((long long)kImgC * 4 * H * W >= (1ll << 31)) return OFLOW_E_SHAPE;
    a.ain = in_format;
    if (d_addend) return OFLOW_E_MODE;
    return dispatch_conv(a, kh, kw, block_n, epilogue, static_cast<hipStream_t>(stream));
  }
  if (in_format != kInF32 && (x_pixel_stride & 127)) return OFLOW_E_ALIGN;
  if (in_format == kInF32Norm && x_pixel_stride != (long long)in_groups * 128) return OFLOW_E_SHAPE;
  if (in_format == kInF32) {
    const long long cin = x_pixel_stride / 4;
    if ((x_pixel_stride & 15) || cin > (long long)in_groups * 32 || cin <= (long long)(in_groups - 1) * 32) return OFLOW_E_SHAPE;
    a.cin = static_cast<int>(cin);
  }
  if (in_format == kInF32Norm) {
    if (!d_in_scale || !d_in_shift) return OFLOW_E_NULL;
    if (kh != 3 || kw != 3 || epilogue != 0 || in_groups > kAinGroups) return OFLOW_E_MODE;
    a.ia = d_in_scale;
    a.ib = d_in_shift;
  } else if (in_format == kInF32) {
    if (kh != 1 || kw != 1 || epilogue != 0 || block_n != 128) return OFLOW_E_MODE;
  }
  a.ain = in_format;
  if (d_addend) {
    if (epilogue == 0) return OFLOW_E_MODE;
    if (N % 8) return OFLOW_E_SHAPE;
    if (((uintptr_t)d_addend & 15) || (addend_pixel_stride & 3) || addend_pixel_stride < N) return OFLOW_E_ALIGN;
    a.add = d_addend;
    a.addps = addend_pixel_stride;
  }
  if (d_ksplit_slab || d_ksplit_ctr) {
    if (!d_ksplit_slab || !d_ksplit_ctr) return OFLOW_E_NULL;
    if (((uintptr_t)d_ksplit_slab & 15) || ((uintptr_t)d_ksplit_ctr & 7)) return OFLOW_E_ALIGN;
    if (ksplit_tiles <= 0) return OFLOW_E_SHAPE;
    a.ks_slab = d_ksplit_slab;
    const bool breg = in_format == kInS32 && a.wf != nullptr && use_breg(a, block_n, kh * kw) && kh * kw != 4 &&
                      (block_n == 128 || (kh == 3 && kw == 3)) && (epilogue == 0 || kh * kw == 5);
    a.ks_slab = nullptr;
    if (breg && (in_groups % 2) == 0) {
      if ((long long)B * ((H + kTY - 1) / kTY) * ((W + kTX - 1) / kTX) * (n_pad / block_n) > ksplit_tiles)
        return OFLOW_E_SHAPE;
      a.ks_slab = d_ksplit_slab;
      a.ks_ctr = d_ksplit_ctr;
      a.ks_tiles = ksplit_tiles;
      a.kg = in_groups / 2;
      a.wbytes /= 2;
    }
  }
  return dispatch_conv(a, kh, kw, block_n, epilogue, static_cast<hipStream_t>(stream));
}

extern "C" int oflow_conv_s32_ex6(const void* d_x, long long x_pixel_stride, int in_groups, const void* d_wpack,
                                  int n_pad, const float* d_wscale, const float* d_bias, int N, int B, int H, int W, int kh,
                                  int kw, int block_n, int epilogue, int activation, float out_scale, void* d_y0,
                                  long long y0_pixel_stride, void* d_y1, long long y1_pixel_stride, float* d_f32,
                                  long long f32_batch_stride, long long f32_channel_stride, int f32_accumulate,
                                  float* d_gru_h, float* d_gru_z, int gru_channels, float* d_nhwc, int nhwc_pixel_stride,
                                  float* d_stats, const void* d_res, long long res_pixel_stride, int res_activation,
                                  int s2d, int in_format, const float* d_in_scale, const float* d_in_shift,
                                  const float* d_addend, long long addend_pixel_stride, const void* d_wfrag,
                                  float* d_ksplit_slab, unsigned* d_ksplit_ctr, long long ksplit_tiles,
                                  const float* d_fh_weights, float* d_fh_partial, int fh_slabs, void* stream) {
  if (epilogue != kEpiFlowHead)
    return oflow_conv_s32_ex5(d_x, x_pixel_stride, in_groups, d_wpack, n_pad, d_wscale, d_bias, N, B, H, W, kh, kw,
                              block_n, epilogue, activation, out_scale, d_y0, y0_pixel_stride, d_y1, y1_pixel_stride,
                              d_f32, f32_batch_stride, f32_channel_stride, f32_accumulate, d_gru_h, d_gru_z,
                              gru_channels, d_nhwc, nhwc_pixel_stride, d_stats, d_res, res_pixel_stride, res_activation,
                              s2d, in_format, d_in_scale, d_in_shift, d_addend, addend_pixel_stride, d_wfrag,
                              d_ksplit_slab, d_ksplit_ctr, ksplit_tiles, stream);
  if (!d_fh_weights || !d_fh_partial) return OFLOW_E_NULL;
  if (N != 256 || n_pad != 256 || fh_slabs != N / 64 || kh != 3 || kw != 3 || (block_n != 64 && block_n != 128))
    return OFLOW_E_SHAPE;
  if (in_format != kInS32 || activation != 1 || out_scale != 1.0f || d_y0 || d_y1 || d_f32 || d_gru_h || d_gru_z ||
      d_nhwc || d_stats || d_res || s2d || d_addend || d_ksplit_slab || d_ksplit_ctr)
    return OFLOW_E_MODE;
  if ((x_pixel_stride & 127) || ((uintptr_t)d_fh_weights & 3) || ((uintptr_t)d_fh_partial & 3)) return OFLOW_E_ALIGN;
  ConvArgs a;
  const int st = build_conv_args(a, d_x, x_pixel_stride, in_groups, d_wpack, n_pad, d_wscale, d_bias, N, B, H, W, kh, kw,
                                 block_n, 0, activation, out_scale, nullptr, 0, nullptr, 0, d_fh_partial, 0, 0, 0, nullptr,
                                 nullptr, 0, nullptr, 0, nullptr, nullptr, 0, 0, 0);
  if (st != OFLOW_OK) return st;
  a.f = nullptr;
  a.fhw = d_fh_weights;
  a.fhy = d_fh_partial;
  if (d_wfrag) {
    if ((uintptr_t)d_wfrag & 15) return OFLOW_E_ALIGN;
    a.wf = static_cast<const uint8_t*>(d_wfrag);
  }
  a.ain = kInS32;
  return dispatch_conv(a, kh, kw, block_n, epilogue, static_cast<hipStream_t>(stream));
}

extern "C" int oflow_conv_s32_ex3(const void* d_x, long long x_pixel_stride, int in_groups, const void* d_wpack,
                                  int n_pad, const float* d_wscale, const float* d_bias, int N, int B, int H, int W, int kh,
                                  int kw, int block_n, int epilogue, int activation, float out_scale, void* d_y0,
                                  long long y0_pixel_stride, void* d_y1, long long y1_pixel_stride, float* d_f32,
                                  long long f32_batch_stride, long long f32_channel_stride, int f32_accumulate,
                                  float* d_gru_h, float* d_gru_z, int gru_channels, float* d_nhwc, int nhwc_pixel_stride,
                                  float* d_stats, const void* d_res, long long res_pixel_stride, int res_activation,
                                  int s2d, int in_format, const float* d_in_scale, const float* d_in_shift,
                                  const float* d_addend, long long addend_pixel_stride, void* stream) {
  return oflow_conv_s32_ex4(d_x, x_pixel_stride, in_groups, d_wpack, n_pad, d_wscale, d_bias, N, B, H, W, kh, kw,
                            block_n, epilogue, activation, out_scale, d_y0, y0_pixel_stride, d_y1, y1_pixel_stride,
                            d_f32, f32_batch_stride, f32_channel_stride, f32_accumulate, d_gru_h, d_gru_z, gru_channels,
                            d_nhwc, nhwc_pixel_stride, d_stats, d_res, res_pixel_stride, res_activation, s2d, in_format,
                            d_in_scale, d_in_shift, d_addend, addend_pixel_stride, nullptr, stream);
}

extern "C" int oflow_conv_s32_ex2(const void* d_x, long long x_pixel_stride, int in_groups, const void* d_wpack,
                                  int n_pad, const float* d_wscale, const float* d_bias, int N, int B, int H, int W, int kh,
                                  int kw, int block_n, int epilogue, int activation, float out_scale, void* d_y0,
                                  long long y0_pixel_stride, void* d_y1, long long y1_pixel_stride, float* d_f32,
                                  long long f32_batch_stride, long long f32_channel_stride, int f32_accumulate,
                                  float* d_gru_h, float* d_gru_z, int gru_channels, float* d_nhwc, int nhwc_pixel_stride,
                                  float* d_stats, const void* d_res, long long res_pixel_stride, int res_activation,
                                  int s2d, int in_format, const float* d_in_scale, const float* d_in_shift,
                                  void* stream) {
  return oflow_conv_s32_ex3(d_x, x_pixel_stride, in_groups, d_wpack, n_pad, d_wscale, d_bias, N, B, H, W, kh, kw,
                            block_n, epilogue, activation, out_scale, d_y0, y0_pixel_stride, d_y1, y1_pixel_stride,
                            d_f32, f32_batch_stride, f32_channel_stride, f32_accumulate, d_gru_h, d_gru_z, gru_channels,
                            d_nhwc, nhwc_pixel_stride, d_stats, d_res, res_pixel_stride, res_activation, s2d, in_format,
                            d_in_scale, d_in_shift, nullptr, 0, stream);
}

extern "C" int oflow_conv_s32_ex(const void* d_x, long long x_pixel_stride, int in_groups, const void* d_wpack,
                                 int n_pad, const float* d_wscale, const float* d_bias, int N, int B, int H, int W, int kh,
                                 int kw, int block_n, int epilogue, int activation, float out_scale, void* d_y0,
                                 long long y0_pixel_stride, void* d_y1, long long y1_pixel_stride, float* d_f32,
                                 long long f32_batch_stride, long long f32_channel_stride, int f32_accumulate,
                                 float* d_gru_h, float* d_gru_z, int gru_channels, float* d_nhwc, int nhwc_pixel_stride,
                                 float* d_stats, const void* d_res, long long res_pixel_stride, int res_activation,
                                 int s2d, void* stream) {
  return oflow_conv_s32_ex2(d_x, x_pixel_stride, in_groups, d_wpack, n_pad, d_wscale, d_bias, N, B, H, W, kh, kw,
                            block_n, epilogue, activation, out_scale, d_y0, y0_pixel_stride, d_y1, y1_pixel_stride,
                            d_f32, f32_batch_stride, f32_channel_stride, f32_accumulate, d_gru_h, d_gru_z, gru_channels,
                            d_nhwc, nhwc_pixel_stride, d_stats, d_res, res_pixel_stride, res_activation, s2d, kInS32,
                            nullptr, nullptr, stream);
}

extern "C" int oflow_conv_s32(const void* d_x, long long x_pixel_stride, int in_groups, const void* d_wpack, int n_pad,
                              const float* d_wscale, const float* d_bias, int N, int B, int H, int W, int kh, int kw,
                              int block_n, int epilogue, int activation, float out_scale, void* d_y0,
                              long long y0_pixel_stride, void* d_y1, long long y1_pixel_stride, float* d_f32,
                              long long f32_batch_stride, long long f32_channel_stride, int f32_accumulate,
                              float* d_gru_h, float* d_gru_z, int gru_channels, void* stream) {
// ... 11 lines not shown
```

torch-optical-flow_amd/csrc/encoder_s32.hip:

```cpp
#include "oflow_internal.h"

namespace oflow {
namespace {

typedef _Float16 half8 __attribute__((ext_vector_type(8)));

__device__ __forceinline__ float act_fn(float v, int act) {
  if (act == 1) return v < 0.f ? 0.f : v;
  if (act == 2) return 1.0f / (1.0f + expf(-v));
  if (act == 3) return tanhf(v);
  return v;
}

__device__ __forceinline__ void put8(uint8_t* line, const float* v) {
  range_guard8(v);
  half8 hi, lo;
  split_vec(v, hi, lo);
  *reinterpret_cast<half8*>(line) = hi;
  *reinterpret_cast<half8*>(line + 64) = lo;
}

constexpr int kStemPX = 64, kStemMaxC = 4;
template <int C>
__global__ __launch_bounds__(256) void stem_patches_kernel(const float* __restrict__ img, int B, int H, int W, int Ho,
                                                           int Wo, int G, uint8_t* out) {
  constexpr int KS = 7, PAD = 3, ST = 2, IX = ST * kStemPX + KS - ST;
  __shared__ float sImg[C][KS][IX];
  const int xb = blockIdx.x, oy = blockIdx.y, b = blockIdx.z;
  const int ox0 = xb * kStemPX;
  const int iy0 = oy * ST - PAD, ix0 = ox0 * ST - PAD;
  const float* src = img + (long long)b * C * H * W;
  for (int e = threadIdx.x; e < C * KS * IX; e += 256) {
    const int c = e / (KS * IX), rem = e - c * (KS * IX);
    const int ky = rem / IX, xx = rem - ky * IX;
    const int iy = iy0 + ky, ix = ix0 + xx;
    float v = 0.f;
    if (static_cast<unsigned>(iy) < static_cast<unsigned>(H) && static_cast<unsigned>(ix) < static_cast<unsigned>(W))
      v = src[((long long)c * H + iy) * W + ix];
    sImg[c][ky][xx] = v;
  }
  __syncthreads();
  const int npx = min(kStemPX, Wo - ox0);
  uint8_t* dst = out + (((long long)b * Ho + oy) * Wo + ox0) * G * 128;
  for (int item = threadIdx.x; item < npx * G * 8; item += 256) {
    const int line = item >> 3, piece = item & 7, q = piece & 3;
    const int px = line / G, g = line - px * G;
    float v[8];
#pragma unroll
    for (int e = 0; e < 8; ++e) v[e] = 0.f;
#pragma unroll
    for (int gg = 0; gg < (KS * KS * C + 31) / 32; ++gg) {
#pragma unroll
      for (int qq = 0; qq < 4; ++qq) {
        if (g == gg && q == qq) {
#pragma unroll
          for (int e = 0; e < 8; ++e) {
            const int k = gg * 32 + qq * 8 + e;
            const int t = k / C, c = k - t * C;
            if (t < KS * KS) v[e] = sImg[c][t / KS][px * ST + t % KS];
          }
        }
      }
    }
    half8 h;
    if (piece < 4) range_guard8(v);
#pragma unroll
    for (int e = 0; e < 8; ++e) {
      _Float16 h_, l_;
      split_f16(v[e], h_, l_);
      h[e] = piece < 4 ? h_ : l_;
    }
    *reinterpret_cast<half8*>(dst + (long long)line * 128 + (piece < 4 ? q * 16 : 64 + q * 16)) = h;
  }
}

constexpr int kStatWaves = 16;
__global__ __launch_bounds__(64 * kStatWaves) void norm_stats_kernel(const float* __restrict__ part, int B, int tiles,
                                                                     int npad, int C, double eps, float* alpha,
                                                                     float* beta) {
  __shared__ double sN[kStatWaves][64], sS[kStatWaves][64], sQ[kStatWaves][64];
  const int lane = threadIdx.x & 63, wave = threadIdx.x >> 6;
  const int cblocks = (C + 63) / 64;
  const int b = blockIdx.x / cblocks, c = (blockIdx.x - b * cblocks) * 64 + lane;
  double n = 0.0, s = 0.0, q = 0.0;
  if (c < C) {
    const float* base = part + ((long long)b * tiles * npad + c) * 3;
    const long long tstride = (long long)npad * 3;
    int t = wave;
    for (; t + 3 * kStatWaves < tiles; t += 4 * kStatWaves) {
      float pv[4][3];
#pragma unroll
      for (int u = 0; u < 4; ++u) {
        const float* p = base + (t + u * kStatWaves) * tstride;
        pv[u][0] = p[0];
        pv[u][1] = p[1];
        pv[u][2] = p[2];
      }
#pragma unroll
      for (int u = 0; u < 4; ++u) {
        const double nb = pv[u][0], mb = pv[u][1];
        n += nb;
        s += nb * mb;
        q += static_cast<double>(pv[u][2]) + nb * mb * mb;
      }
    }
    for (; t < tiles; t += kStatWaves) {
      const float* p = base + t * tstride;
      const double nb = p[0], mb = p[1];
      n += nb;
      s += nb * mb;
      q += static_cast<double>(p[2]) + nb * mb * mb;
    }
  }
  sN[wave][lane] = n;
  sS[wave][lane] = s;
  sQ[wave][lane] = q;
  __syncthreads();
  if (wave == 0 && c < C) {
    for (int w = 1; w < kStatWaves; ++w) {
      n += sN[w][lane];
      s += sS[w][lane];
      q += sQ[w][lane];
    }
    const double mean = n > 0.0 ? s / n : 0.0;
    double var = n > 0.0 ? q / n - mean * mean : 0.0;
    if (var < 0.0) var = 0.0;
    const float invstd = static_cast<float>(1.0 / sqrt(var + eps));
    alpha[(long long)b * C + c] = invstd;
    beta[(long long)b * C + c] = -static_cast<float>(mean) * invstd;
  }
}

__global__ __launch_bounds__(256) void norm_apply_kernel(const float* __restrict__ x, int C, int B, int H, int W,
                                                         const float* __restrict__ alpha, const float* __restrict__ beta,
                                                         int act, int res_mode, const uint8_t* res, long long resps,
                                                         const float* __restrict__ x2, const float* __restrict__ alpha2,
                                                         const float* __restrict__ beta2, int res_act, int s2d,
                                                         uint8_t* y, long long yps) {
  const int C8 = C / 8;
  const int HW = H * W, P = B * HW;
  const int item = blockIdx.x * blockDim.x + threadIdx.x;
  if (item >= P * C8) return;
  const int p = item / C8, c8 = item - p * C8;
  const int b = p / HW;
  const int c0 = c8 * 8;
  auto ld8 = [](const float* q, float (&o)[8]) {
    const float4 u0 = reinterpret_cast<const float4*>(q)[0], u1 = reinterpret_cast<const float4*>(q)[1];
    o[0] = u0.x; o[1] = u0.y; o[2] = u0.z; o[3] = u0.w; o[4] = u1.x; o[5] = u1.y; o[6] = u1.z; o[7] = u1.w;
  };
  float v[8], al[8], be[8];
  ld8(x + (long long)p * C + c0, v);
  ld8(alpha + b * C + c0, al);
  ld8(beta + b * C + c0, be);
#pragma unroll
  for (int j = 0; j < 8; ++j) v[j] = act_fn(v[j] * al[j] + be[j], act);
  if (res_mode == 1) {
    const uint8_t* rl = res + p * resps + (long long)(c0 >> 5) * 128 + ((c0 & 31) >> 3) * 16;
    const half8 rh = *reinterpret_cast<const half8*>(rl), rlo = *reinterpret_cast<const half8*>(rl + 64);
#pragma unroll
    for (int j = 0; j < 8; ++j) v[j] = act_fn(v[j] + (static_cast<float>(rh[j]) + static_cast<float>(rlo[j])), res_act);
  } else if (res_mode >= 2) {
    float r[8], a2[8], b2[8];
    ld8(x2 + (long long)p * C + c0, r);
    ld8(alpha2 + b * C + c0, a2);
    ld8(beta2 + b * C + c0, b2);
#pragma unroll
    for (int j = 0; j < 8; ++j) {
      float rn = r[j] * a2[j] + b2[j];
      if (res_mode == 3) rn = act_fn(rn, 1);
      v[j] = act_fn(rn + v[j], res_act);
    }
  }
  long long pd = p;
  int cd = c0;
  if (s2d) {
    const int pix = p - b * HW;
    const int yy = pix / W, xx = pix - yy * W;
    pd = ((long long)b * (H >> 1) + (yy >> 1)) * (W >> 1) + (xx >> 1);
    cd = c0 + ((yy & 1) * 2 + (xx & 1)) * C;
  }
  put8(y + pd * yps + (long long)(cd >> 5) * 128 + ((cd & 31) >> 3) * 16, v);
}

}
OFLOW_RANGE_FLAG_SETTER(encoder)
}

using namespace oflow;

extern "C" int oflow_stem_patches_s32(const float* d_img, int B, int C, int H, int W, void* d_out, int out_groups,
                                      void* stream) {
  if (!d_img || !d_out) return OFLOW_E_NULL;
  if (B <= 0 || C <= 0 || H <= 0 || W <= 0 || out_groups * 32 < 49 * C) return OFLOW_E_SHAPE;
  if ((uintptr_t)d_out & 15) return OFLOW_E_ALIGN;
  if (C > kStemMaxC || B > 65535) return OFLOW_E_SHAPE;
  const int Ho = (H - 1) / 2 + 1, Wo = (W - 1) / 2 + 1;
  if (Ho > 65535) return OFLOW_E_SHAPE;
  const dim3 grid((Wo + kStemPX - 1) / kStemPX, Ho, B);
  hipStream_t s = static_cast<hipStream_t>(stream);
  uint8_t* o = static_cast<uint8_t*>(d_out);
  switch (C) {
    case 1: hipLaunchKernelGGL(stem_patches_kernel<1>, grid, dim3(256), 0, s, d_img, B, H, W, Ho, Wo, out_groups, o); break;
    case 2: hipLaunchKernelGGL(stem_patches_kernel<2>, grid, dim3(256), 0, s, d_img, B, H, W, Ho, Wo, out_groups, o); break;
    case 3: hipLaunchKernelGGL(stem_patches_kernel<3>, grid, dim3(256), 0, s, d_img, B, H, W, Ho, Wo, out_groups, o); break;
    default: hipLaunchKernelGGL(stem_patches_kernel<4>, grid, dim3(256), 0, s, d_img, B, H, W, Ho, Wo, out_groups, o); break;
  }
  return launch_status();
}

extern "C" int oflow_norm_stats_finalize(const float* d_partials, int B, int tiles, int n_pad, int C, double eps,
                                         float* d_alpha, float* d_beta, void* stream) {
  if (!d_partials || !d_alpha || !d_beta) return OFLOW_E_NULL;
  if (B <= 0 || tiles <= 0 || C <= 0 || n_pad < C) return OFLOW_E_SHAPE;
  hipLaunchKernelGGL(norm_stats_kernel, dim3(B * ((C + 63) / 64)), dim3(64 * kStatWaves), 0, static_cast<hipStream_t>(stream),
                     d_partials, B, tiles, n_pad, C, eps, d_alpha, d_beta);
  return launch_status();
}

extern "C" int oflow_norm_apply_s32(const float* d_x, int C, int B, int H, int W, const float* d_alpha,
                                    const float* d_beta, int activation, int res_mode, const void* d_res,
                                    long long res_pixel_stride, const float* d_x2, const float* d_alpha2,
                                    const float* d_beta2, int res_activation, int s2d, void* d_y,
                                    long long y_pixel_stride, void* stream) {
  if (!d_x || !d_alpha || !d_beta || !d_y) return OFLOW_E_NULL;
  if (B <= 0 || C <= 0 || C % 8 || H <= 0 || W <= 0) return OFLOW_E_SHAPE;
  if (activation < 0 || activation > 3 || res_activation < 0 || res_activation > 3 || res_mode < 0 || res_mode > 3)
    return OFLOW_E_MODE;
  if (res_mode == 1 && !d_res) return OFLOW_E_NULL;
  if (res_mode >= 2 && (!d_x2 || !d_alpha2 || !d_beta2)) return OFLOW_E_NULL;
  if (s2d && ((H | W) & 1)) return OFLOW_E_SHAPE;
  if (((uintptr_t)d_x & 15) || ((uintptr_t)d_y & 15) || (y_pixel_stride & 127) ||
      (d_res && (((uintptr_t)d_res & 15) || (res_pixel_stride & 127))) || (d_x2 && ((uintptr_t)d_x2 & 15)) ||
      (((uintptr_t)d_alpha | (uintptr_t)d_beta) & 15) || (((uintptr_t)d_alpha2 | (uintptr_t)d_beta2) & 15))
    return OFLOW_E_ALIGN;
  const long long items = (long long)B * H * W * (C / 8);
  if ((items + 255) / 256 * 256 >= (1ll << 31)) return OFLOW_E_SHAPE;
  hipLaunchKernelGGL(norm_apply_kernel, dim3((unsigned)((items + 255) / 256)), dim3(256), 0, static_cast<hipStream_t>(stream),
                     d_x, C, B, H, W, d_alpha, d_beta, activation, res_mode, static_cast<const uint8_t*>(d_res),
                     res_pixel_stride, d_x2, d_alpha2, d_beta2, res_activation, s2d, static_cast<uint8_t*>(d_y),
                     y_pixel_stride);
  return launch_status();
}
```

torch-optical-flow_amd/methods/raft/model/extractor.py:

```python
from __future__ import annotations

import os

from typing import Optional, List, Sequence, Tuple, Union

import torch
import torch.nn as nn
from torch import Tensor

from optical_flow import _native

from .update import CONV_BLOCKS, parse_block_overrides


def _norm_layer(norm_fn: str, planes: int, groups: int) -> nn.Module:
    if norm_fn == "group":
        return nn.GroupNorm(num_groups=groups, num_channels=planes)
    if norm_fn == "batch":
        return nn.BatchNorm2d(planes)
    if norm_fn == "instance":
        return nn.InstanceNorm2d(planes)
    if norm_fn == "none":
        return nn.Sequential()
    raise ValueError(f"unknown norm_fn {norm_fn!r}")
# ... 25 lines not shown

class BasicEncoder(nn.Module):

    def __init__(self, output_dim: int = 128, norm_fn: str = "batch", dropout: float = 0.0) -> None:
        super().__init__()
        self.norm_fn = norm_fn
        self.norm1 = _norm_layer(norm_fn, 64, 8)
        self.conv1 = nn.Conv2d(3, 64, kernel_size=7, stride=2, padding=3)
        self.relu1 = nn.ReLU(inplace=True)
        self.in_planes = 64
        self.layer1 = self._make_layer(64, stride=1)
        self.layer2 = self._make_layer(96, stride=2)
        self.layer3 = self._make_layer(128, stride=2)
        self.conv2 = nn.Conv2d(128, output_dim, kernel_size=1)
        self.dropout = nn.Dropout2d(p=dropout) if dropout > 0 else None
        for m in self.modules():
            if isinstance(m, nn.Conv2d):
                nn.init.kaiming_normal_(m.weight, mode="fan_out", nonlinearity="relu")
            elif isinstance(m, (nn.BatchNorm2d, nn.InstanceNorm2d, nn.GroupNorm)):
                if m.weight is not None:
                    nn.init.constant_(m.weight, 1)
                if m.bias is not None:
                    nn.init.constant_(m.bias, 0)

    def _make_layer(self, dim: int, stride: int = 1) -> nn.Module:
        blocks = (ResidualBlock(self.in_planes, dim, self.norm_fn, stride=stride), ResidualBlock(dim, dim, self.norm_fn, 1))
        self.in_planes = dim
        return nn.Sequential(*blocks)

    def forward(self, x: Union[Tensor, Sequence[Tensor]]) -> Union[Tensor, Tuple[Tensor, ...]]:
        is_list = isinstance(x, (tuple, list))
        if is_list:
            batch_dim = x[0].shape[0]
            x = torch.cat(list(x), dim=0)
        x = self.relu1(self.norm1(self.conv1(x)))
        x = self.layer3(self.layer2(self.layer1(x)))
        x = self.conv2(x)
        if self.training and self.dropout is not None:
            x = self.dropout(x)
        if is_list:
            return torch.split(x, [batch_dim, batch_dim], dim=0)
        return x




def _s2d_weight(w: Tensor) -> Tensor:
    n, c = w.shape[:2]
    out = torch.zeros((n, 4, c, 2, 2), device=w.device, dtype=w.dtype)
    for kyp in range(2):
        for a in range(2):
            ky = 2 * kyp + a - 1
            if not 0 <= ky <= 2:
                continue
            for kxp in range(2):
                for b in range(2):
                    kx = 2 * kxp + b - 1
                    if 0 <= kx <= 2:
                        out[:, a * 2 + b, :, kyp, kxp] = w[:, :, ky, kx]
    return out.reshape(n, 4 * c, 2, 2)


def _fold_bn(conv: nn.Conv2d, bn: nn.Module):
    w = conv.weight.detach().double()
    b = conv.bias.detach().double() if conv.bias is not None else torch.zeros(w.shape[0], device=w.device, dtype=w.dtype)
    alpha = bn.weight.detach().double() / torch.sqrt(bn.running_var.detach().double() + bn.eps)
    beta = bn.bias.detach().double() - bn.running_mean.detach().double() * alpha
    return (w * alpha.view(-1, 1, 1, 1)).float(), (b * alpha + beta).float()


_ENC_BN_OVERRIDE = {int(k): v for k, v in
                    parse_block_overrides("OFLOW_ENC_BN", {str(b) for b in CONV_BLOCKS}).items()}


class SplitEncoder:

    def __init__(self, enc: BasicEncoder) -> None:
        if enc.norm_fn not in ("instance", "batch"):
            raise RuntimeError(f"SplitEncoder: norm_fn {enc.norm_fn!r} not supported")
        if enc.norm_fn == "batch" and enc.training:
            raise RuntimeError("SplitEncoder: batch norm needs eval mode (running statistics)")
        self.enc = enc
        self.inorm = enc.norm_fn == "instance"
        from .update import cached_pack, tensor_key

        key = tuple(tensor_key(q) for q in enc.parameters()) + tuple(tensor_key(q) for q in enc.buffers())
        self.w = cached_pack(enc, key, lambda: self._pack(enc))

    def _cw(self, conv: nn.Conv2d, norm, **kw):
        if self.inorm or norm is None:
            w, b = conv.weight, conv.bias
        else:
            w, b = _fold_bn(conv, norm)
        if kw.pop("s2d", False):
            w = _s2d_weight(w.detach().float())
        n = w.shape[0]
        return _native.ConvWeights(w, b, ((n + 31) // 32) * 32, **kw)

    def _pack(self, enc: BasicEncoder):
        W = {"stem": self._cw(enc.conv1, enc.norm1, patches=True)}
        for li, layer in enumerate((enc.layer1, enc.layer2, enc.layer3)):
            for bi, blk in enumerate(layer):
                s2 = blk.downsample is not None
                W[f"{li}.{bi}.conv1"] = self._cw(blk.conv1, blk.norm1, s2d=s2)
                W[f"{li}.{bi}.conv2"] = self._cw(blk.conv2, blk.norm2)
                if s2:
                    W[f"{li}.{bi}.down"] = self._cw(blk.downsample[0], blk.downsample[1])
        W["head"] = _native.ConvWeights(enc.conv2.weight, enc.conv2.bias, ((enc.conv2.out_channels + 31) // 32) * 32)
        return W

    @staticmethod
    def _bn(n: int) -> int:
        bn = {64: 64, 96: 96, 128: 128}.get(n, 128 if n % 128 == 0 else 64 if n % 64 == 0 else 32)
        return _ENC_BN_OVERRIDE.get(bn, bn)

    def _conv_norm(self, x, cw, shape, act, out=None, res=None, s2d=False, raw_only=False):
        b, h, w = shape
        bn = self._bn(cw.n)
        V = _native.S32Slice
        dev = x.device
        if self.inorm:
            raw = torch.empty((b * h * w, cw.n), device=dev, dtype=torch.float32)
            tiles = _native.conv_tiles(h, w)
            part = torch.empty((b, tiles, cw.n_pad, 3), device=dev, dtype=torch.float32)
            _native.conv_s32(x, cw, bn, nhwc=raw, stats=part)
            alpha, beta = _native.norm_stats(part, b, tiles, cw.n_pad, cw.n, 1e-5)
            if raw_only:
                return raw, alpha, beta
            if out is None:
                out = _native.s32_empty(b, h // 2 if s2d else h, w // 2 if s2d else w, (cw.n * (4 if s2d else 1) + 31) // 32, dev)
            if isinstance(res, _native.NhwcNormIn):
                _native.norm_apply(raw, (b, cw.n, h, w), alpha, beta, act, V(out), res_raw=(res.raw, res.scale, res.shift),
                                   res_act="relu", s2d=s2d, res_raw_relu=True)
            elif isinstance(res, tuple):
                _native.norm_apply(raw, (b, cw.n, h, w), alpha, beta, act, V(out), res_raw=res, res_act="relu", s2d=s2d)
            else:
                _native.norm_apply(raw, (b, cw.n, h, w), alpha, beta, act, V(out), res=res, res_act="relu" if res is not None else "none", s2d=s2d)
            return out
        if raw_only:
            out = _native.s32_empty(b, h, w, (cw.n + 31) // 32, dev)
            _native.conv_s32(x, cw, bn, y0=V(out))
            return out
        if out is None:
            out = _native.s32_empty(b, h // 2 if s2d else h, w // 2 if s2d else w, (cw.n * (4 if s2d else 1) + 31) // 32, dev)
        _native.conv_s32(x, cw, bn, act=act, y0=V(out), res=res, res_act="relu" if res is not None else "none", s2d=s2d)
        return out

    def _conv1(self, x, cw, shape):
        if self.inorm:
            raw, alpha, beta = self._conv_norm(x, cw, shape, "relu", raw_only=True)
            return _native.NhwcNormIn(raw, *shape, alpha, beta)
        return _native.S32Slice(self._conv_norm(x, cw, shape, "relu"))

    def stem_patches(self, x: Tensor) -> Tensor:
        x = x.float().contiguous()
        n, _, hh, ww = x.shape
        patches = _native.s32_empty(n, hh // 2, ww // 2, self.w["stem"].kg, x.device)
        _native.stem_patches(x, patches)
        return patches

    def __call__(self, x: Union[Tensor, Sequence[Tensor]], patches: Optional[Tensor] = None,
                 split_out: bool = False, stem_from_image: bool = False) -> Union[Tensor, Tuple[Tensor, ...]]:
        is_list = isinstance(x, (tuple, list))
        if is_list:
            batch_dim = x[0].shape[0]
            n, _, hh, ww = x[0].shape
            n *= len(x)
            if patches is None or tuple(patches.shape[:4]) != (n, hh // 2, ww // 2, self.w["stem"].kg):
                x = torch.cat(list(x), dim=0)
        if not isinstance(x, (tuple, list)):
            x = x.float().contiguous()
            n, _, hh, ww = x.shape
            dev = x.device
        else:
            dev = x[0].device
        if hh % 8 or ww % 8:
            raise RuntimeError("SplitEncoder: H and W must be multiples of 8")
        V = _native.S32Slice
        h, w = hh // 2, ww // 2
        if stem_from_image:
            if isinstance(x, (tuple, list)):
                x = torch.cat([t.float() for t in x], dim=0)
            stem_in = _native.ImgIn(x.float().contiguous())
            self.patches = None
        else:
            if patches is None or tuple(patches.shape[:4]) != (n, h, w, self.w["stem"].kg):
                patches = _native.s32_empty(n, h, w, self.w["stem"].kg, dev)
                _native.stem_patches(x, patches)
            self.patches = patches
            stem_in = V(patches)
        cur = (self._conv1(stem_in, self.w["stem"], (n, h, w)) if self.inorm
               else self._conv_norm(stem_in, self.w["stem"], (n, h, w), "relu"))
        layers = (self.enc.layer1, self.enc.layer2, self.enc.layer3)
        for li, layer in enumerate(layers):
            for bi, blk in enumerate(layer):
                last_of_stage = bi == len(layer) - 1
                out_s2d = last_of_stage and li + 1 < len(layers)
                pre = f"{li}.{bi}."
                if blk.downsample is None:
                    x_in = cur if isinstance(cur, _native.NhwcNormIn) else V(cur)
                    t = self._conv1(x_in, self.w[pre + "conv1"], (n, h, w))
                    cur = self._conv_norm(t, self.w[pre + "conv2"], (n, h, w), "relu", res=x_in, s2d=out_s2d)
                else:
                    h, w = h // 2, w // 2
                    t = self._conv1(V(cur), self.w[pre + "conv1"], (n, h, w))
                    cin = self.w[pre + "down"].kg
                    d = self._conv_norm(V(cur, 0, cin), self.w[pre + "down"], (n, h, w), "none", raw_only=True)
                    res = d if self.inorm else V(d)
                    cur = self._conv_norm(t, self.w[pre + "conv2"], (n, h, w), "relu", res=res, s2d=out_s2d)
                if out_s2d:
                    pass
        head = self.w["head"]
        if split_out:
            out = _native.s32_empty(n, h, w, (head.n + 31) // 32, dev)
            _native.conv_s32(V(cur), head, self._bn(head.n), y0=V(out))
        else:
            out = torch.empty((n, head.n, h, w), device=dev, dtype=torch.float32)
            _native.conv_s32(V(cur), head, self._bn(head.n), f32=out)
        if is_list:
            return torch.split(out, [batch_dim, batch_dim], dim=0)
        return out
```

torch-optical-flow_amd/optical_flow/_native.py:

```python
from __future__ import annotations

import ctypes
import os
from typing import List, Optional, Sequence

import torch

from . import _ops

_LIB_PATH = os.environ.get(
    "OFLOW_LIB", os.path.join(os.path.dirname(os.path.abspath(__file__)), "_lib", "liboflow_hip.so")
)
ABI_VERSION = 1
MAX_LEVELS = 8
MAX_RADIUS = 7
FLOW_HEAD2_MAX_PIXELS = 16384
E_TINY = -4

INTERP = {"bilinear": 0, "nearest": 1, "bicubic": 2}
PADDING = {"zeros": 0, "border": 1, "reflection": 2}

SYMBOLS = (
    "oflow_abi_version",
    "oflow_status_string",
    "oflow_corr_pyramid_dims",
    "oflow_corr_pyramid_f32",
    "oflow_corr_lookup_f32",
    "oflow_corr_tiled_level_floats",
    "oflow_corr_pyramid_tiled_f32",
    "oflow_corr_lookup_tiled_f32",
    "oflow_corr_untile_f32",
    "oflow_grid_warp_f32",
    "oflow_grid_sample_f32",
    "oflow_corr_otf_prepare_f16",
    "oflow_corr_lookup_otf_f16",
    "oflow_bias_act_f32",
    "oflow_gru_reset_f32",
    "oflow_gru_blend_f32",
    "oflow_conv_s32",
    "oflow_pack_s32_f32",
    "oflow_flow_prep_s32",
    "oflow_conv_s32_ex",
    "oflow_stem_patches_s32",
    "oflow_norm_stats_finalize",
    "oflow_norm_apply_s32",
    "oflow_convex_upsample_f32",
    "oflow_conv_s32_ex2",
    "oflow_corr_lookup_tiled_nhwc_f32",
    "oflow_corr_lookup_backward_f32",
    "oflow_corr_pyramid_grad_combine_f32",
    "oflow_flow_stats_f32",
    "oflow_flow2rgb_f32",
    "oflow_flow_pack_f32",
    "oflow_corr_lookup_convc1_s32",
    "oflow_corr_pyramid_tiled_s32",
    "oflow_flow_head2_s32",
    "oflow_flow_head2_tiled_s32",
    "oflow_conv_s32_ex3",
    "oflow_conv_s32_ex4",
    "oflow_conv_s32_ex5",
    "oflow_normalize_images_f32",
    "oflow_replicate_pad_f32",
    "oflow_corr_fmap_grad_f32",
    "oflow_grid_warp_backward_f32",
    "oflow_grid_sample_backward_f32",
    "oflow_set_range_flag",
    "oflow_range_flag_exchange",
    "oflow_flow_head_col2im_f32",
    "oflow_conv_s32_ex6",
    "oflow_flow_head_finish_f32",
    "oflow_timing_event_create",
    "oflow_timing_event_destroy",
    "oflow_timing_event_record",
    "oflow_timing_event_elapsed_ms",
    "oflow_flow_error_stats_f32",
    "oflow_sequence_loss_f32",
    "oflow_sequence_loss_backward_f32",
)

_lib = None
_recorder = None
_flops = None


def set_flop_counter(counter):
    global _flops
    _flops = counter


def _count(exec_f16: int, useful: int, fma: int = 0) -> None:
    _flops["exec_f16"] = _flops.get("exec_f16", 0) + exec_f16
    _flops["useful"] = _flops.get("useful", 0) + useful
    _flops["fma_f32"] = _flops.get("fma_f32", 0) + fma


def set_event_recorder(recorder):
    global _recorder
    _recorder = recorder


class TimingEvent:

    __slots__ = ("ev",)

    def __init__(self):
        ev = ctypes.c_void_p()
        _check(load().oflow_timing_event_create(ctypes.byref(ev)), "timing_event_create")
        self.ev = ev

    def record(self, stream: "torch.cuda.Stream") -> None:
        _check(load().oflow_timing_event_record(self.ev, ctypes.c_void_p(stream.cuda_stream), 1), "timing_event_record")

    def elapsed_time(self, end: "TimingEvent") -> float:
        ms = ctypes.c_float()
        _check(load().oflow_timing_event_elapsed_ms(self.ev, end.ev, ctypes.byref(ms)), "timing_event_elapsed_ms")
        return float(ms.value)

    def __del__(self):
        try:
            if _lib is not None and self.ev:
                _lib.oflow_timing_event_destroy(self.ev)
        except Exception:
            pass


_TIMED_DEFAULT = ("corr_lookup", "corr_lookup_convc1", "corr_pyramid", "corr_lookup_otf", "corr_otf_prepare", "grid_warp")


class _Timed:
    __slots__ = ("what", "stream", "ev0")

    def __init__(self, what: str, device: torch.device):
        self.what = what
        on = _recorder is not None and (what in _TIMED_DEFAULT or _recorder.get("*", False))
        self.stream = torch.cuda.current_stream(device) if on else None
        self.ev0 = None

    def __enter__(self):
        if self.stream is not None:
            self.ev0 = TimingEvent() if _recorder.get("_native") else torch.cuda.Event(enable_timing=True)
            self.ev0.record(self.stream)
        return self

    def __exit__(self, *exc):
        if self.stream is not None and exc[0] is None and _recorder is not None:
            ev1 = TimingEvent() if _recorder.get("_native") else torch.cuda.Event(enable_timing=True)
            ev1.record(self.stream)
            _recorder.setdefault(self.what, []).append((self.ev0, ev1))
        return False


def library_path() -> str:
    return _LIB_PATH


def load() -> ctypes.CDLL:
    global _lib
    if _lib is not None:
        return _lib
    if not os.path.exists(_LIB_PATH):
        raise RuntimeError(
            f"liboflow_hip.so not found at {_LIB_PATH}: build it with `make -C torch-optical-flow_amd/csrc` "
            "(or __graft_entry__.build()); the MI355X path has no CPU fallback"
        )
    lib = ctypes.CDLL(_LIB_PATH)
    P, I, F = ctypes.c_void_p, ctypes.c_int, ctypes.c_float
    IP = ctypes.POINTER(ctypes.c_int)
    PP = ctypes.POINTER(ctypes.c_void_p)
    lib.oflow_abi_version.restype = I
    lib.oflow_abi_version.argtypes = []
    lib.oflow_status_string.restype = ctypes.c_char_p
    lib.oflow_status_string.argtypes = [I]
    lib.oflow_corr_pyramid_dims.restype = I
    lib.oflow_corr_pyramid_dims.argtypes = [I, I, I, IP, IP]
    lib.oflow_corr_pyramid_f32.restype = I
    lib.oflow_corr_pyramid_f32.argtypes = [P, P, I, I, I, I, I, PP, P]
    lib.oflow_corr_lookup_f32.restype = I
    lib.oflow_corr_lookup_f32.argtypes = [PP, IP, IP, I, P, I, I, I, I, P, P]
    lib.oflow_corr_tiled_level_floats.restype = ctypes.c_longlong
    lib.oflow_corr_tiled_level_floats.argtypes = [I, I]
    lib.oflow_corr_pyramid_tiled_f32.restype = I
    lib.oflow_corr_pyramid_tiled_f32.argtypes = [P, P, I, I, I, I, I, PP, P]
    lib.oflow_corr_lookup_tiled_f32.restype = I
    lib.oflow_corr_lookup_tiled_f32.argtypes = [PP, IP, IP, I, P, I, I, I, I, P, P]
    lib.oflow_corr_untile_f32.restype = I
    lib.oflow_corr_untile_f32.argtypes = [P, P, ctypes.c_longlong, I, I, P]
    lib.oflow_grid_warp_f32.restype = I
    lib.oflow_grid_warp_f32.argtypes = [P, P, I, I, I, I, I, I, I, P, P]
    lib.oflow_grid_sample_f32.restype = I
    lib.oflow_grid_sample_f32.argtypes = [P, P, I, I, I, I, I, I, I, I, I, P, P]
    lib.oflow_corr_otf_prepare_f16.restype = I
    lib.oflow_corr_otf_prepare_f16.argtypes = [P, P, I, I, I, I, I, P, PP, P, P]
    L = ctypes.c_longlong
    lib.oflow_bias_act_f32.restype = I
    lib.oflow_bias_act_f32.argtypes = [P, L, P, P, L, P, L, I, I, I, I, F, P]
    lib.oflow_gru_reset_f32.restype = I
    lib.oflow_gru_reset_f32.argtypes = [P, L, P, P, L, P, L, I, I, I, P]
    lib.oflow_gru_blend_f32.restype = I
    lib.oflow_gru_blend_f32.argtypes = [P, L, P, P, L, P, P, L, I, I, I, P]
    lib.oflow_conv_s32.restype = I
    lib.oflow_conv_s32.argtypes = [P, L, I, P, I, P, P, I, I, I, I, I, I, I, I, I, F, P, L, P, L, P, L, L, I, P, P, I, P]
    lib.oflow_conv_s32_ex.restype = I
    lib.oflow_conv_s32_ex.argtypes = [P, L, I, P, I, P, P, I, I, I, I, I, I, I, I, I, F, P, L, P, L, P, L, L, I, P, P, I,
                                      P, I, P, P, L, I, I, P]
    lib.oflow_stem_patches_s32.restype = I
    lib.oflow_stem_patches_s32.argtypes = [P, I, I, I, I, P, I, P]
    lib.oflow_norm_stats_finalize.restype = I
    lib.oflow_norm_stats_finalize.argtypes = [P, I, I, I, I, ctypes.c_double, P, P, P]
    lib.oflow_norm_apply_s32.restype = I
    lib.oflow_norm_apply_s32.argtypes = [P, I, I, I, I, P, P, I, I, P, L, P, P, P, I, I, P, L, P]
    lib.oflow_pack_s32_f32.restype = I
    lib.oflow_pack_s32_f32.argtypes = [P, L, I, I, I, I, I, I, P, L, P, L, P, I, P]
    lib.oflow_flow_prep_s32.restype = I
    lib.oflow_flow_prep_s32.argtypes = [P, I, I, I, P, P, L, P, L, P]
    lib.oflow_corr_lookup_otf_f16.restype = I
    lib.oflow_corr_lookup_otf_f16.argtypes = [P, PP, IP, IP, I, P, I, I, I, I, I, P, P]
    lib.oflow_conv_s32_ex2.restype = I
    lib.oflow_conv_s32_ex2.argtypes = list(lib.oflow_conv_s32_ex.argtypes[:-1]) + [I, P, P, P]
    lib.oflow_conv_s32_ex3.restype = I
    lib.oflow_conv_s32_ex3.argtypes = list(lib.oflow_conv_s32_ex2.argtypes[:-1]) + [P, L, P]
    lib.oflow_conv_s32_ex4.restype = I
    lib.oflow_normalize_images_f32.restype = I
    lib.oflow_normalize_images_f32.argtypes = [P, P, L, P, P, P]
    lib.oflow_replicate_pad_f32.restype = I
    lib.oflow_replicate_pad_f32.argtypes = [P, P, I, L, I, I, I, I, I, I, P]
    lib.oflow_conv_s32_ex4.argtypes = list(lib.oflow_conv_s32_ex3.argtypes[:-1]) + [P, P]
    lib.oflow_conv_s32_ex5.restype = I
    lib.oflow_conv_s32_ex5.argtypes = list(lib.oflow_conv_s32_ex4.argtypes[:-1]) + [P, P, L, P]
    lib.oflow_corr_lookup_backward_f32.restype = I
    lib.oflow_corr_lookup_backward_f32.argtypes = [P, P, I, I, I, I, PP, IP, IP, I, P]
    lib.oflow_corr_pyramid_grad_combine_f32.restype = I
    lib.oflow_corr_pyramid_grad_combine_f32.argtypes = [PP, IP, IP, I, L, P]
    lib.oflow_corr_lookup_tiled_nhwc_f32.restype = I
    lib.oflow_corr_lookup_tiled_nhwc_f32.argtypes = [PP, IP, IP, I, P, I, I, I, I, P, I, P]
    lib.oflow_convex_upsample_f32.restype = I
    lib.oflow_flow_head2_s32.restype = I
    lib.oflow_flow_head2_s32.argtypes = [P, ctypes.c_longlong, I, P, P, I, I, I, P, P]
    lib.oflow_flow_head2_tiled_s32.restype = I
    lib.oflow_flow_head2_tiled_s32.argtypes = [P, ctypes.c_longlong, I, P, P, I, I, I, P, P]
    lib.oflow_corr_pyramid_tiled_s32.restype = I
    lib.oflow_corr_pyramid_tiled_s32.argtypes = [P, P, I, I, I, I, I, PP, P]
    lib.oflow_corr_lookup_convc1_s32.restype = I
    lib.oflow_corr_lookup_convc1_s32.argtypes = [PP, IP, IP, I, P, I, I, I, I, P, P, P, P, ctypes.c_longlong, P]
    lib.oflow_convex_upsample_f32.argtypes = [P, P, I, I, I, P, P]
    lib.oflow_flow_stats_f32.restype = I
    lib.oflow_flow_stats_f32.argtypes = [P, I, I, I, I, F, F, I, P, P]
    lib.oflow_flow2rgb_f32.restype = I
    lib.oflow_flow2rgb_f32.argtypes = [P, I, I, I, I, I, F, F, I, I, F, P, P, P]
    lib.oflow_flow_pack_f32.restype = I
    lib.oflow_flow_pack_f32.argtypes = [P, I, I, I, I, I, P, P]
    lib.oflow_set_range_flag.restype = I
    lib.oflow_set_range_flag.argtypes = [P]
    lib.oflow_range_flag_exchange.restype = I
    lib.oflow_range_flag_exchange.argtypes = [P, P, P]
    lib.oflow_timing_event_create.restype = I
    lib.oflow_timing_event_create.argtypes = [ctypes.POINTER(ctypes.c_void_p)]
    lib.oflow_timing_event_destroy.restype = I
    lib.oflow_timing_event_destroy.argtypes = [P]
    lib.oflow_timing_event_record.restype = I
    lib.oflow_timing_event_record.argtypes = [P, P, I]
    lib.oflow_timing_event_elapsed_ms.restype = I
    lib.oflow_timing_event_elapsed_ms.argtypes = [P, P, ctypes.POINTER(ctypes.c_float)]
    lib.oflow_flow_head_col2im_f32.restype = I
    lib.oflow_flow_head_col2im_f32.argtypes = [P, P, I, I, I, P, P]
    lib.oflow_conv_s32_ex6.restype = I
    lib.oflow_conv_s32_ex6.argtypes = list(lib.oflow_conv_s32_ex5.argtypes[:-1]) + [P, P, I, P]
    lib.oflow_flow_head_finish_f32.restype = I
    lib.oflow_flow_head_finish_f32.argtypes = [P, I, P, I, I, I, P, P, L, P, L, P]
    FP = ctypes.POINTER(F)
    lib.oflow_flow_error_stats_f32.restype = I
    lib.oflow_flow_error_stats_f32.argtypes = [P, L, L, L, P, L, L, L, P, I, L, L, I, I, I, F, F, F, P, P, P, P]
    lib.oflow_sequence_loss_f32.restype = I
    lib.oflow_sequence_loss_f32.argtypes = [PP, I, FP, P, P, I, I, I, I, F, P, P, P, P]
    lib.oflow_sequence_loss_backward_f32.restype = I
    lib.oflow_sequence_loss_backward_f32.argtypes = [P, PP, PP, I, FP, P, P, I, I, I, I, F, P]
    v = lib.oflow_abi_version()
    if v != ABI_VERSION:
        raise RuntimeError(f"liboflow_hip.so ABI version {v}, expected {ABI_VERSION}: rebuild the library")
    _ops.load()
    _lib = lib
    return lib


def ops():
    if _lib is None:
        load()
    return torch.ops.oflow


def _run(what: str, device: torch.device, op, *args):
    if _recorder is None:
        return op(*args)
    with _Timed(what, device):
        return op(*args)


def _tensor(t, name: str, what: str) -> torch.Tensor:
    if not isinstance(t, torch.Tensor):
        raise TypeError(f"{what}: {name} must be a torch.Tensor")
    return t


def _no_grad_input(t: torch.Tensor, name: str, what: str) -> None:
    if t.requires_grad and torch.is_grad_enabled():
        raise RuntimeError(
            f"{what}: {name} requires grad; this layout is inference-only (no backward): use CorrBlock's canonical "
            "pyramid (corr_pyramid / corr_lookup have autograd), or run under torch.no_grad()"
        )


def _check(status: int, what: str) -> None:
    if status == 0:
        return
    msg = load().oflow_status_string(status).decode()
    if status == E_TINY:
        raise ValueError(f"{what}: {msg}")
    raise RuntimeError(f"{what} failed ({status}): {msg}")


def _gpu_f32(t: torch.Tensor, name: str, what: str) -> torch.Tensor:
    if not isinstance(t, torch.Tensor):
        raise TypeError(f"{what}: {name} must be a torch.Tensor")
    if t.device.type != "cuda":
        raise RuntimeError(
            f"{what}: {name} is on {t.device}; this MI355X build runs only on ROCm GPU tensors (no CPU fallback)"
        )
    if t.requires_grad and torch.is_grad_enabled():
        raise RuntimeError(
            f"{what}: {name} requires grad; this entry point is an inference layout with no autograd formula: use "
            "CorrBlock / optical_flow.warp (native backward kernels), or run under torch.no_grad() / "
            "torch.inference_mode(), or detach the input"
        )
    if t.dtype != torch.float32:
        t = t.float()
    return t.contiguous()


def _stream(device: torch.device) -> ctypes.c_void_p:
    return ctypes.c_void_p(torch.cuda.current_stream(device).cuda_stream)


def pyramid_dims(h: int, w: int, num_levels: int):
    hs = (ctypes.c_int * MAX_LEVELS)()
    ws = (ctypes.c_int * MAX_LEVELS)()
    _check(load().oflow_corr_pyramid_dims(h, w, num_levels, hs, ws), "corr_pyramid_dims")
    return [(hs[i], ws[i]) for i in range(num_levels)]


def corr_pyramid(fmap1: torch.Tensor, fmap2: torch.Tensor, num_levels: int = 4) -> List[torch.Tensor]:
    f1, f2 = _tensor(fmap1, "fmap1", "corr_pyramid"), _tensor(fmap2, "fmap2", "corr_pyramid")
    return list(_run("corr_pyramid", f1.device, ops().corr_pyramid, f1, f2, int(num_levels)))


class TiledPyramid:

    __slots__ = ("levels", "dims", "queries")

    def __init__(self, levels, dims, queries):
        self.levels, self.dims, self.queries = levels, dims, queries

    def batch_slice(self, b0: int, b1: int) -> "TiledPyramid":
        hw = self.dims[0][0] * self.dims[0][1]
        return TiledPyramid([t[b0 * hw : b1 * hw] for t in self.levels], self.dims, (b1 - b0) * hw)

    def untile(self, l: int) -> torch.Tensor:
        hl, wl = self.dims[l]
        src = self.levels[l]
        out = torch.empty((self.queries, 1, hl, wl), device=src.device, dtype=torch.float32)
        if out.numel():
            with torch.cuda.device(src.device):
                _check(load().oflow_corr_untile_f32(src.data_ptr(), out.data_ptr(), self.queries, hl, wl, _stream(src.device)), "untile")
        return out


def corr_pyramid_tiled(fmap1: torch.Tensor, fmap2: torch.Tensor, num_levels: int = 4) -> TiledPyramid:
    what = "corr_pyramid"
    f1, f2 = _tensor(fmap1, "fmap1", what), _tensor(fmap2, "fmap2", what)
    _no_grad_input(f1, "fmap1", what)
    _no_grad_input(f2, "fmap2", what)
    levels = list(_run(what, f1.device, ops().corr_pyramid_tiled, f1, f2, int(num_levels)))
    return TiledPyramid(levels, pyramid_dims(f1.shape[2], f1.shape[3], num_levels), int(levels[0].shape[0]))


def corr_pyramid_tiled_s32(f1: torch.Tensor, f2: torch.Tensor, num_levels: int = 4) -> TiledPyramid:
    what = "corr_pyramid"
    for t in (f1, f2):
        if t.dtype != torch.float16 or t.dim() != 6 or tuple(t.shape[-2:]) != (2, 32) or not t.is_contiguous():
            raise RuntimeError(f"{what}: S32 feature maps must be contiguous fp16 (B, H, W, G, 2, 32)")
        if t.device.type != "cuda":
            raise RuntimeError(f"{what}: S32 feature maps must be on the GPU (no CPU fallback)")
    if f1.shape != f2.shape or f1.device != f2.device:
        raise RuntimeError(f"{what}: feature maps differ in shape or device")
    b, h, w, g = (int(v) for v in f1.shape[:4])
    dims = pyramid_dims(h, w, num_levels)
    lib = load()
    per_q = [int(lib.oflow_corr_tiled_level_floats(hl, wl)) for hl, wl in dims]
    q = b * h * w
    store = torch.empty((q * sum(per_q),), device=f1.device, dtype=torch.float32)
    levels, off = [], 0
    for n in per_q:
        levels.append(store[off * q : (off + n) * q].view(q, n))
        off += n
    ptrs = (ctypes.c_void_p * MAX_LEVELS)(*[t.data_ptr() for t in levels])
    if _flops is not None:
        _count(3 * 2 * b * (h * w) ** 2 * g * 32, 2 * b * (h * w) ** 2 * g * 32)
    with torch.cuda.device(f1.device), _Timed(what, f1.device):
        _check(lib.oflow_corr_pyramid_tiled_s32(f1.data_ptr(), f2.data_ptr(), b, g * 32, h, w, int(num_levels), ptrs,
                                                _stream(f1.device)), what)
    return TiledPyramid(levels, dims, q)


def corr_lookup_tiled(pyr: TiledPyramid, coords: torch.Tensor, radius: int) -> torch.Tensor:
    co = _tensor(coords, "coords", "corr_lookup")
    _no_grad_input(co, "coords", "corr_lookup")
    return _run("corr_lookup", co.device, ops().corr_lookup_tiled, pyr.levels, co, int(radius))


# ... 24 lines not shown
    fl = _gpu_f32(flow, "flow", what)
    mk = _gpu_f32(mask, "mask", what)
    if fl.dim() != 4 or fl.shape[1] != 2 or mk.dim() != 4 or mk.shape[1] != 576 or mk.shape[0] != fl.shape[0] or mk.shape[2:] != fl.shape[2:]:
        raise RuntimeError(f"{what}: flow {tuple(flow.shape)} must be (B, 2, H, W) and mask {tuple(mask.shape)} (B, 576, H, W)")
    if fl.device != mk.device:
        raise RuntimeError(f"{what}: flow and mask are on different devices")
    b, _, h, w = fl.shape
    out = torch.empty((b, 2, 8 * h, 8 * w), device=fl.device, dtype=torch.float32)
    if out.numel() == 0:
        return out
    with torch.cuda.device(fl.device), _Timed("upsample_flow", fl.device):
        _check(load().oflow_convex_upsample_f32(fl.data_ptr(), mk.data_ptr(), b, h, w, out.data_ptr(), _stream(fl.device)), what)
    return out


FLOW2RGB_METHODS = {"baker": 0, "hsv": 1, "meister": 2}
FLOW_STATS_CHUNKS = 128


def _flow_b2hw(flow: torch.Tensor, what: str) -> torch.Tensor:
    fl = _gpu_f32(flow, "flow", what)
    if fl.dim() != 4 or fl.shape[1] != 2:
        raise RuntimeError(f"{what}: flow {tuple(flow.shape)} must be (B, 2, H, W)")
    return fl


def flow2rgb(flow: torch.Tensor, method: str, clip, denom, invert_y: bool) -> torch.Tensor:
    what = "flow2rgb"
    if method not in FLOW2RGB_METHODS:
        raise ValueError(f"Unknown method: '{method}'.")
    fl = _flow_b2hw(flow, what)
    b, _, h, w = fl.shape
    out = torch.empty((b, 3, h, w), device=fl.device, dtype=torch.float32)
    if out.numel() == 0:
        return out
    do_clip = clip is not None
    lo, hi = (float(clip[0]), float(clip[1])) if do_clip else (0.0, 0.0)
    have_denom = denom is not None
    denom = float(denom) if have_denom else 0.0
    need_stats = (not have_denom) or method == "meister"
    lib = load()
    with torch.cuda.device(fl.device), _Timed("flow2rgb", fl.device):
        stream = _stream(fl.device)
        parts = None
        if need_stats:
            parts = torch.empty((b, FLOW_STATS_CHUNKS, 2), device=fl.device, dtype=torch.float32)
            _check(lib.oflow_flow_stats_f32(fl.data_ptr(), b, h, w, int(do_clip), lo, hi, int(bool(invert_y)),
                                            parts.data_ptr(), stream), what)
        _check(lib.oflow_flow2rgb_f32(fl.data_ptr(), b, h, w, FLOW2RGB_METHODS[method], int(do_clip), lo, hi,
                                      int(bool(invert_y)), int(have_denom), denom,
                                      parts.data_ptr() if parts is not None else None, out.data_ptr(), stream), what)
    return out


def flow_pack(flow: torch.Tensor, channels: int, flip_rows: bool) -> torch.Tensor:
    what = "flow_pack"
    fl = _flow_b2hw(flow, what)
    b, _, h, w = fl.shape
    out = torch.empty((b, h, w, channels), device=fl.device, dtype=torch.float32)
    if out.numel() == 0:
        return out
    with torch.cuda.device(fl.device), _Timed("flow_pack", fl.device):
        _check(load().oflow_flow_pack_f32(fl.data_ptr(), b, h, w, int(channels), int(bool(flip_rows)),
                                          out.data_ptr(), _stream(fl.device)), what)
    return out


def grid_sample(inp: torch.Tensor, grid: torch.Tensor, mode: str, padding_mode: str, align_corners: bool) -> torch.Tensor:
    what = "grid_sample"
    m, p = _modes(mode, padding_mode, what)
    x, g = _tensor(inp, "input", what), _tensor(grid, "grid", what)
    return _run("grid_sample", x.device, ops().grid_sample, x, g, m, p, bool(align_corners))


def otf_prepare(fmap1: torch.Tensor, fmap2: torch.Tensor, num_levels: int = 4):
    what = "corr_otf_prepare"
    f1, f2 = _tensor(fmap1, "fmap1", what), _tensor(fmap2, "fmap2", what)
    _no_grad_input(f1, "fmap1", what)
    _no_grad_input(f2, "fmap2", what)
    f1h, f2h = _run(what, f1.device, ops().corr_otf_prepare, f1, f2, int(num_levels))
    return f1h, list(f2h)


def corr_lookup_otf(f1h: torch.Tensor, f2h: Sequence[torch.Tensor], coords: torch.Tensor, radius: int) -> torch.Tensor:
    co = _tensor(coords, "coords", "corr_lookup_otf")
    _no_grad_input(co, "coords", "corr_lookup_otf")
    return _run("corr_lookup_otf", co.device, ops().corr_lookup_otf, f1h, list(f2h), co, int(radius))


ACT = {"none": 0, "relu": 1, "sigmoid": 2, "tanh": 3}

_range_flags = {}


def range_flag(device: torch.device) -> torch.Tensor:
    device = torch.device(device)
    idx = device.index if device.index is not None else torch.cuda.current_device()
    flag = _range_flags.get(idx)
    if flag is None:
        flag = torch.zeros(1, dtype=torch.int32, device=torch.device("cuda", idx))
        with torch.cuda.device(idx):
            torch.cuda.synchronize(idx)
            _check(load().oflow_set_range_flag(ctypes.c_void_p(flag.data_ptr())), "set_range_flag")
        _range_flags[idx] = flag
    return flag


class RangeSnapshot:

    __slots__ = ("dev_word", "host", "event", "device")

    def __init__(self, device: torch.device) -> None:
        self.device = device
        self.dev_word = torch.empty(1, dtype=torch.int32, device=device)
        self.host = torch.empty(1, dtype=torch.int32, pin_memory=True)
        self.event = torch.cuda.Event()

    def take(self) -> "RangeSnapshot":
        flag = range_flag(self.device)
        stream = torch.cuda.current_stream(self.device)
        with torch.cuda.device(self.device):
            _check(load().oflow_range_flag_exchange(ctypes.c_void_p(flag.data_ptr()),
                                                    ctypes.c_void_p(self.dev_word.data_ptr()),
                                                    ctypes.c_void_p(stream.cuda_stream)), "range_flag_exchange")
            self.host.copy_(self.dev_word, non_blocking=True)
            self.event.record(stream)
        return self

    def done(self) -> bool:
        return self.event.query()

    def overflowed(self) -> bool:
        self.event.synchronize()
        return bool(int(self.host[0]))


RANGE_ERROR = ("a split-fp16 operand exceeded the fp16 range (|x| >= 65520) -- an activation outside the range these "
               "kernels represent exactly; the output is not valid (OFLOW_CHECK=1 names the convolution)")


def range_flag_raise_if_set(device: torch.device, what: str = "RAFT forward", all_streams: bool = False) -> None:
    device = torch.device(device)
    if all_streams:
        torch.cuda.synchronize(device)
    if RangeSnapshot(device).take().overflowed():
        raise RuntimeError(f"{what}: {RANGE_ERROR}")


CHECK_RANGE = os.environ.get("OFLOW_CHECK", "0") not in ("", "0")
F16_MAX = 65504.0
CONV_BREG = True
CONV_BREG64 = False
CONV_BREG32 = False


def _range_check(x, what: str) -> None:
    if isinstance(x, S32Slice):
        v = x.t[:, :, :, x.g0 : x.g0 + x.ng, 0]
    elif isinstance(x, NhwcNormIn):
        b, h, w = x.bhw
        c = x.raw.shape[1]
        v = torch.relu(x.raw.view(b, h * w, c) * x.scale.view(b, 1, c) + x.shift.view(b, 1, c))
    else:
        v = x.raw
    m = float(v.abs().amax().float()) if v.numel() else 0.0
    if not m <= F16_MAX:
        raise RuntimeError(
            f"{what}: input max |x| = {m:g} is outside the fp16 range (65504) of the split-fp16 operands (OFLOW_CHECK)"
        )


def _chan_view(t: torch.Tensor, what: str):
    if t.device.type != "cuda" or t.dtype != torch.float32 or t.dim() != 4:
        raise RuntimeError(f"{what}: expected a 4-D fp32 ROCm tensor, got {t.dtype} {tuple(t.shape)} on {t.device}")
    b, c, h, w = t.shape
    if t.stride(3) != 1 or t.stride(2) != w or t.stride(1) != h * w:
        raise RuntimeError(f"{what}: the (C, H, W) part must be contiguous")
    return t.data_ptr(), t.stride(0), c, h * w


def bias_act_(x: torch.Tensor, bias, act: str = "relu", scale: float = 1.0, out=None, out2=None) -> torch.Tensor:
    px, sx, c, p = _chan_view(x, "bias_act")
    y = x if out is None else out
    py, sy, cy, py_ = _chan_view(y, "bias_act out")
    p2, s2 = (0, 0)
    if out2 is not None:
        p2, s2, c2, _ = _chan_view(out2, "bias_act out2")
        if c2 != c:
            raise RuntimeError("bias_act: out2 channel count differs")
    if cy != c or py_ != p or y.shape[0] != x.shape[0]:
        raise RuntimeError("bias_act: output shape differs from input")
    if bias is not None and (bias.numel() != c or bias.dtype != torch.float32 or not bias.is_contiguous()):
        raise RuntimeError("bias_act: bias must be a contiguous fp32 vector of C elements")
    with torch.cuda.device(x.device):
        _check(
            load().oflow_bias_act_f32(
                px, sx, bias.data_ptr() if bias is not None else None, py, sy, p2 or None, s2, x.shape[0], c, p,
                ACT[act], float(scale), _stream(x.device)
            ),
            "bias_act",
        )
    return y


def gru_reset(zr: torch.Tensor, br: torch.Tensor, h: torch.Tensor, rh: torch.Tensor) -> None:
    pz, sz, c2, p = _chan_view(zr, "gru_reset zr")
    ph, sh, ch, p1 = _chan_view(h, "gru_reset h")
    pr, sr, cr, p2 = _chan_view(rh, "gru_reset rh")
    if c2 != 2 * ch or cr != ch or p1 != p or p2 != p or br.numel() != ch:
        raise RuntimeError("gru_reset: inconsistent shapes")
    with torch.cuda.device(h.device):
        _check(load().oflow_gru_reset_f32(pz, sz, br.data_ptr(), ph, sh, pr, sr, h.shape[0], ch, p, _stream(h.device)), "gru_reset")


def gru_blend_(zr: torch.Tensor, bz: torch.Tensor, q: torch.Tensor, bq: torch.Tensor, h: torch.Tensor) -> None:
    pz, sz, c2, p = _chan_view(zr, "gru_blend zr")
    pq, sq, cq, p1 = _chan_view(q, "gru_blend q")
    ph, sh, ch, p2 = _chan_view(h, "gru_blend h")
    if c2 != 2 * ch or cq != ch or p1 != p or p2 != p or bz.numel() != ch or bq.numel() != ch:
        raise RuntimeError("gru_blend: inconsistent shapes")
    with torch.cuda.device(h.device):
        _check(
            load().oflow_gru_blend_f32(pz, sz, bz.data_ptr(), pq, sq, bq.data_ptr(), ph, sh, h.shape[0], ch, p, _stream(h.device)),
            "gru_blend",
        )




class S32Slice:

    __slots__ = ("t", "g0", "ng")

    def __init__(self, t: torch.Tensor, g0: int = 0, ng: int = -1):
        if t.dtype != torch.float16 or t.dim() != 6 or tuple(t.shape[-2:]) != (2, 32) or not t.is_contiguous():
            raise RuntimeError(f"S32 tensor must be contiguous fp16 (B, H, W, G, 2, 32), got {t.dtype} {tuple(t.shape)}")
        self.t, self.g0 = t, int(g0)
        self.ng = int(t.shape[3]) - self.g0 if ng < 0 else int(ng)
        if self.g0 < 0 or self.g0 + self.ng > t.shape[3]:
            raise RuntimeError("S32Slice: group range outside the tensor")

    @property
    def ptr(self) -> int:
        return self.t.data_ptr() + self.g0 * 128

    @property
    def ps(self) -> int:
        return int(self.t.shape[3]) * 128

    def channel_ptr(self, c: int) -> int:
        return self.ptr + (c // 32) * 128 + (c % 32) * 2

    @property
    def bhw(self):
        return tuple(int(v) for v in self.t.shape[:3])

    @property
    def device(self):
        return self.t.device


class F32In:

    __slots__ = ("raw", "bhw")
    in_format = 2

    def __init__(self, raw: torch.Tensor, b: int, h: int, w: int):
        if raw.dtype != torch.float32 or not raw.is_contiguous() or raw.shape[0] != b * h * w or raw.shape[1] % 4:
            raise RuntimeError("F32In: raw must be contiguous fp32 [B*H*W, C], C % 4 == 0")
        self.raw, self.bhw = raw, (int(b), int(h), int(w))

    @property
    def ptr(self) -> int:
        return self.raw.data_ptr()

    @property
    def ps(self) -> int:
        return int(self.raw.shape[1]) * 4

    @property
    def ng(self) -> int:
        return (int(self.raw.shape[1]) + 31) // 32

    @property
    def device(self):
        return self.raw.device


class ImgIn:

    __slots__ = ("raw", "bhw")
    in_format = 3

    def __init__(self, img: torch.Tensor):
        if img.dtype != torch.float32 or img.dim() != 4 or img.shape[1] != 3 or not img.is_contiguous():
            raise RuntimeError("ImgIn: the image must be contiguous fp32 (B, 3, H, W)")
        b, _, hh, ww = img.shape
        if hh % 2 or ww % 2:
            raise RuntimeError("ImgIn: H and W must be even")
        self.raw, self.bhw = img, (int(b), int(hh) // 2, int(ww) // 2)

    @property
    def ptr(self) -> int:
        return self.raw.data_ptr()

    @property
    def ps(self) -> int:
        return 0

    @property
    def ng(self) -> int:
        return 5

    @property
    def device(self):
        return self.raw.device


class FlowIn:

    __slots__ = ("raw", "bhw")
    in_format = 4

    def __init__(self, coords: torch.Tensor):
        if coords.dtype != torch.float32 or coords.dim() != 4 or coords.shape[1] != 2 or not coords.is_contiguous():
            raise RuntimeError("FlowIn: coords must be contiguous fp32 (B, 2, H, W)")
        b, _, hh, ww = coords.shape
        self.raw, self.bhw = coords, (int(b), int(hh), int(ww))

    @property
    def ptr(self) -> int:
        return self.raw.data_ptr()

    @property
    def ps(self) -> int:
        return 0

    @property
    def ng(self) -> int:
        return 4

    @property
    def device(self):
        return self.raw.device


class NhwcNormIn:

    __slots__ = ("raw", "bhw", "scale", "shift")
    in_format = 1

    def __init__(self, raw: torch.Tensor, b: int, h: int, w: int, scale: torch.Tensor, shift: torch.Tensor):
        c = raw.shape[1]
        if raw.dtype != torch.float32 or not raw.is_contiguous() or raw.shape[0] != b * h * w or c % 32:
            raise RuntimeError("NhwcNormIn: raw must be contiguous fp32 [B*H*W, C], C % 32 == 0")
        for t in (scale, shift):
            if t.dtype != torch.float32 or not t.is_contiguous() or t.numel() != b * c:
                raise RuntimeError("NhwcNormIn: scale / shift must be contiguous fp32 [B, C]")
        self.raw, self.bhw, self.scale, self.shift = raw, (int(b), int(h), int(w)), scale, shift

    @property
    def ptr(self) -> int:
        return self.raw.data_ptr()

    @property
    def ps(self) -> int:
        return int(self.raw.shape[1]) * 4

    @property
    def ng(self) -> int:
        return int(self.raw.shape[1]) // 32

    @property
    def device(self):
        return self.raw.device


def s32_empty(b: int, h: int, w: int, groups: int, device, zero: bool = False) -> torch.Tensor:
    f = torch.zeros if zero else torch.empty
    return f((b, h, w, groups, 2, 32), device=device, dtype=torch.float16)


def s32_from_f32(x: torch.Tensor, groups: int = -1) -> torch.Tensor:
    b, c, h, w = x.shape
    g = (c + 31) // 32 if groups < 0 else groups
    v = torch.zeros((b, h, w, g * 32), device=x.device, dtype=torch.float32)
    v[..., :c] = x.permute(0, 2, 3, 1)
    hi = v.half()
    lo = (v - hi.float()).half()
    return torch.stack([hi.view(b, h, w, g, 32), lo.view(b, h, w, g, 32)], dim=4).contiguous()


def s32_to_f32(t: torch.Tensor, channels: int = -1) -> torch.Tensor:
    b, h, w, g = t.shape[:4]
    v = (t[:, :, :, :, 0].float() + t[:, :, :, :, 1].float()).reshape(b, h, w, g * 32)
    c = g * 32 if channels < 0 else channels
    return v[..., :c].permute(0, 3, 1, 2).contiguous()


class ConvWeights:

    __slots__ = ("pack", "wscale", "bias", "n", "n_pad", "kh", "kw", "kg", "layout", "cin", "_frag")

    def __init__(self, weight: torch.Tensor, bias, n_pad: int, patches: bool = False):
        w = weight.detach().float()
        if patches:
            n, c, kh, kw = w.shape
            w = w.permute(0, 2, 3, 1).reshape(n, kh * kw * c, 1, 1)
        n, c, kh, kw = w.shape
        if n_pad < n:
            raise RuntimeError("ConvWeights: n_pad < out channels")
        amax = w.abs().amax(dim=(1, 2, 3))
        e = torch.where(amax > 0, torch.ceil(torch.log2(amax)), torch.zeros_like(amax)).clamp(-100, 100)
        scale = torch.exp2(14.0 - e)
        ws = w * scale.view(-1, 1, 1, 1)
        kg = (c + 31) // 32
        t = kh * kw
        full = torch.zeros((n_pad, kg * 32, t), device=w.device, dtype=torch.float32)
        full[:n, :c] = ws.reshape(n, c, t)
        full = full.view(n_pad, kg, 32, t).permute(1, 3, 0, 2).contiguous()
        hi = full.half()
        lo = (full - hi.float()).half()
        self.pack = torch.stack([hi, lo], dim=3).contiguous()
        inv = torch.ones(n_pad, device=w.device, dtype=torch.float32)
        inv[:n] = 1.0 / scale
        self.wscale = inv
        self.bias = None if bias is None else bias.detach().float().contiguous()
        self.n, self.n_pad, self.kh, self.kw, self.kg = n, n_pad, kh, kw, kg
        self.cin = c
        self.layout = "conv"
        self._frag = None
        if t > 1 and n_pad % 32 == 0:
            self.frag()

    def frag(self) -> torch.Tensor:
        if self._frag is None:
            if self.layout != "conv" or self.n_pad % 32:
                raise RuntimeError("ConvWeights.frag: needs a conv-layout pack with n_pad a multiple of 32")
            kg, t = self.pack.shape[:2]
            f = self.pack.reshape(kg, t, self.n_pad // 32, 32, 2, 2, 2, 8)
            self._frag = f.permute(0, 1, 2, 5, 4, 6, 3, 7).contiguous()
        return self._frag


def convc1_level_weights(conv: torch.nn.Conv2d, num_levels: int, radius: int) -> "ConvWeights":
    kk = (2 * radius + 1) ** 2
    g = (kk + 31) // 32
    w = conv.weight.detach().float()
    if tuple(w.shape[1:]) != (num_levels * kk, 1, 1):
        raise RuntimeError(f"convc1_level_weights: expected a 1x1 conv over {num_levels * kk} channels, got {tuple(w.shape)}")
    wp = w.new_zeros((w.shape[0], num_levels * g * 32, 1, 1))
    for l in range(num_levels):
        wp[:, l * g * 32 : l * g * 32 + kk] = w[:, l * kk : (l + 1) * kk]
    cw = ConvWeights(wp, conv.bias, w.shape[0])
    lg = cw.pack.shape[0]
    frag = cw.pack.reshape(lg, 4, 2, 32, 2, 2, 2, 8)
    cw.pack = frag.permute(0, 1, 2, 5, 4, 6, 3, 7).contiguous()
    cw.layout = "convc1_frag"
    cw.cin = num_levels * kk
    return cw


def corr_lookup_convc1(pyr: "TiledPyramid", coords: torch.Tensor, radius: int, cw: "ConvWeights", y: "S32Slice") -> None:
    what = "corr_lookup_convc1"
    co = _gpu_f32(coords, "coords", what)
    b, two, h, w = co.shape
    if two != 2 or b * h * w != pyr.queries:
        raise RuntimeError(f"{what}: coords (B, 2, H, W) must cover the pyramid's {pyr.queries} queries")
    kk = (2 * radius + 1) ** 2
    if (cw.layout != "convc1_frag" or cw.n != 256 or cw.n_pad != 256 or cw.kh * cw.kw != 1
            or cw.kg != len(pyr.levels) * ((kk + 31) // 32)):
        raise RuntimeError(f"{what}: weights must be convc1_level_weights of this pyramid / radius")
    if y.ng != 8 or y.bhw != (b, h, w) or y.device != co.device:
        raise RuntimeError(f"{what}: destination must be an 8-group S32 slice of shape ({b}, {h}, {w})")
    n = len(pyr.levels)
    ptrs = (ctypes.c_void_p * MAX_LEVELS)(*[t.data_ptr() for t in pyr.levels])
    hs = (ctypes.c_int * MAX_LEVELS)(*[d[0] for d in pyr.dims])
    ws = (ctypes.c_int * MAX_LEVELS)(*[d[1] for d in pyr.dims])
    if _flops is not None:
        _count(3 * 2 * b * h * w * 256 * cw.kg * 32, 2 * b * h * w * 256 * cw.cin)
    with torch.cuda.device(co.device), _Timed(what, co.device):
        _check(
            load().oflow_corr_lookup_convc1_s32(
                ptrs, hs, ws, n, co.data_ptr(), b, h, w, int(radius), cw.pack.data_ptr(), cw.wscale.data_ptr(),
                cw.bias.data_ptr() if cw.bias is not None else None, y.ptr, y.ps, _stream(co.device),
            ),
            what,
        )


def conv_tiles(h: int, w: int) -> int:
    return ((h + 3) // 4) * ((w + 31) // 32)


class KSplit:

    def __init__(self, b: int, h: int, w: int, device, block_n: int = 128, blocks: int = 1) -> None:
        self.tiles = b * conv_tiles(h, w) * blocks
        self.block_n = block_n
        self.slab = torch.empty(self.tiles * 128 * block_n, device=device, dtype=torch.float32)
        self.ctr = torch.zeros(2 * self.tiles, device=device, dtype=torch.int32)


def conv_s32(x: S32Slice, cw: ConvWeights, block_n: int, act: str = "none", out_scale: float = 1.0, y0=None, y1=None,
             f32=None, f32_accumulate: bool = False, epilogue: int = 0, gru_h=None, gru_z=None, nhwc=None, stats=None,
             res=None, res_act: str = "none", s2d: bool = False, addend=None, ksplit: "KSplit" = None) -> None:
    what = "conv_s32"
    if CHECK_RANGE:
        _range_check(x, f"{what} {cw.kh}x{cw.kw}")
    if x.ng != cw.kg:
        raise RuntimeError(f"{what}: input has {x.ng} groups, weights expect {cw.kg}")
    b, h, w = x.bhw
    nin = isinstance(x, NhwcNormIn)
    in_format = getattr(x, "in_format", 0)
    hw_out = (h // 2, w // 2) if s2d else (h, w)
    for d in (y0, y1):
        if d is not None and (tuple(d.t.shape[:3]) != (b, *hw_out) or d.t.device != x.device):
            raise RuntimeError(f"{what}: destination shape/device mismatch")
    if res is not None and (tuple(res.t.shape[:3]) != (b, h, w) or res.ng * 32 < cw.n):
        raise RuntimeError(f"{what}: residual shape mismatch")
    fp, fbs, fcs = 0, 0, 0
    if f32 is not None:
        if f32.dtype != torch.float32 or f32.dim() != 4 or tuple(f32.shape[2:]) != (h, w) or f32.shape[0] != b:
            raise RuntimeError(f"{what}: fp32 destination must be (B, C, H, W) fp32")
        if f32.stride(3) != 1 or f32.stride(2) != w or f32.shape[1] < cw.n and epilogue == 0:
            raise RuntimeError(f"{what}: fp32 destination planes must be contiguous with >= N channels")
        fp, fbs, fcs = f32.data_ptr(), f32.stride(0), f32.stride(1)
    if nhwc is not None and (nhwc.dtype != torch.float32 or not nhwc.is_contiguous() or nhwc.numel() != b * h * w * cw.n):
        raise RuntimeError(f"{what}: nhwc destination must be contiguous fp32 [P, {cw.n}]")
    if stats is not None and (stats.dtype != torch.float32 or stats.numel() < b * conv_tiles(h, w) * cw.n_pad * 3):
        raise RuntimeError(f"{what}: stats partials buffer too small")
    gh = gz = 0
    gch = 0
    if epilogue:
        gch = cw.n // 2 if epilogue == 1 else cw.n
        for tt in (gru_h, gru_z):
            if tt is None or tt.dtype != torch.float32 or not tt.is_contiguous() or tt.numel() != b * h * w * gch:
                raise RuntimeError(f"{what}: GRU state tensors must be contiguous fp32 [P, {gch}]")
        gh, gz = gru_h.data_ptr(), gru_z.data_ptr()
    ap, aps = 0, 0
    if addend is not None:
        if (not epilogue or addend.dtype != torch.float32 or addend.dim() != 2 or addend.stride(1) != 1
                or addend.shape[0] != b * h * w or addend.shape[1] < cw.n or addend.stride(0) % 4
                or addend.data_ptr() % 16 or addend.device != x.device):
            raise RuntimeError(f"{what}: addend must be a GRU-epilogue fp32 [P, >= {cw.n}] view with 16-B aligned rows")
        ap, aps = addend.data_ptr(), addend.stride(0)
    dev = x.device
    wf = (cw.frag().data_ptr() if CONV_BREG and (int(block_n) == 128 or (CONV_BREG64 and int(block_n) == 64)
                                                 or (CONV_BREG32 and int(block_n) == 32))
          and cw.kh * cw.kw > 1 and not nin
          and in_format == 0 and cw.layout == "conv" else None)
    if _flops is not None:
        taps, p_out = cw.kh * cw.kw, b * h * w
        n_exec = -(-cw.n_pad // int(block_n)) * int(block_n)
        _count(3 * 2 * p_out * n_exec * cw.kg * 32 * taps, 2 * p_out * cw.n * cw.cin * taps)
    ks_slab = ks_ctr = None
    ks_tiles = 0
    if ksplit is not None and wf is not None:
        if ksplit.slab.device != dev or ksplit.block_n < int(block_n):
            raise RuntimeError(f"{what}: split-K scratch on another device or for narrower channel blocks")
        ks_slab, ks_ctr = ksplit.slab.data_ptr(), ksplit.ctr.data_ptr()
        ks_tiles = ksplit.tiles * (ksplit.block_n // int(block_n))
    with torch.cuda.device(dev), _Timed(f"conv{cw.kh}x{cw.kw}", dev):
        _check(
            load().oflow_conv_s32_ex5(
                x.ptr, x.ps, cw.kg, cw.pack.data_ptr(), cw.n_pad, cw.wscale.data_ptr(),
                cw.bias.data_ptr() if cw.bias is not None else None, cw.n, b, h, w, cw.kh, cw.kw, int(block_n),
                int(epilogue), ACT[act], float(out_scale), y0.ptr if y0 is not None else None, y0.ps if y0 is not None else 0,
                y1.ptr if y1 is not None else None, y1.ps if y1 is not None else 0, fp or None, fbs, fcs,
                int(bool(f32_accumulate)), gh or None, gz or None, gch,
                nhwc.data_ptr() if nhwc is not None else None, cw.n,
                stats.data_ptr() if stats is not None else None,
                res.ptr if res is not None else None, res.ps if res is not None else 0, ACT[res_act], int(bool(s2d)),
                in_format, x.scale.data_ptr() if nin else None, x.shift.data_ptr() if nin else None,
                ap or None, aps, wf, ks_slab, ks_ctr, ks_tiles, _stream(dev),
            ),
            what,
        )


def flow_head2(x: "S32Slice", weight: torch.Tensor, bias: torch.Tensor, coords: torch.Tensor) -> None:
    what = "flow_head2"
    b, h, w = x.bhw
    if weight.dtype != torch.float32 or not weight.is_contiguous() or tuple(weight.shape) != (2, x.ng * 32, 3, 3):
        raise RuntimeError(f"{what}: weight must be contiguous fp32 (2, {x.ng * 32}, 3, 3)")
    if bias is None or bias.dtype != torch.float32 or tuple(bias.shape) != (2,):
        raise RuntimeError(f"{what}: bias must be fp32 (2,)")
    if coords.dtype != torch.float32 or not coords.is_contiguous() or tuple(coords.shape) != (b, 2, h, w):
        raise RuntimeError(f"{what}: coords must be contiguous fp32 ({b}, 2, {h}, {w})")
    if _flops is not None:
        fl = 2 * b * h * w * 2 * x.ng * 32 * 9
        _count(0, fl, fl)
    with torch.cuda.device(coords.device), _Timed("conv3x3", coords.device):
        _check(load().oflow_flow_head2_s32(x.ptr, x.ps, x.ng, weight.data_ptr(), bias.data_ptr(), b, h, w,
                                           coords.data_ptr(), _stream(coords.device)), what)


def flow_head2_tiled_weights(weight: torch.Tensor) -> torch.Tensor:
    o, c = weight.shape[:2]
    if o != 2 or c % 32 or tuple(weight.shape[2:]) != (3, 3):
        raise RuntimeError("flow_head2_tiled_weights: weight must be (2, C, 3, 3) with C a multiple of 32")
    w = weight.detach().float().reshape(2, c // 32, 8, 4, 3, 3)
    return w.permute(1, 2, 4, 5, 0, 3).contiguous()


def flow_head2_tiled(x: "S32Slice", wr: torch.Tensor, bias: torch.Tensor, coords: torch.Tensor) -> None:
    what = "flow_head2_tiled"
    b, h, w = x.bhw
    if wr.dtype != torch.float32 or not wr.is_contiguous() or wr.numel() != 2 * x.ng * 32 * 9 or wr.data_ptr() % 16:
        raise RuntimeError(f"{what}: wr must be flow_head2_tiled_weights of a (2, {x.ng * 32}, 3, 3) weight")
    if bias is None or bias.dtype != torch.float32 or tuple(bias.shape) != (2,):
        raise RuntimeError(f"{what}: bias must be fp32 (2,)")
    if coords.dtype != torch.float32 or not coords.is_contiguous() or tuple(coords.shape) != (b, 2, h, w):
        raise RuntimeError(f"{what}: coords must be contiguous fp32 ({b}, 2, {h}, {w})")
    if _flops is not None:
        fl = 2 * b * h * w * 2 * x.ng * 32 * 9
        _count(0, fl, fl)
    with torch.cuda.device(coords.device), _Timed("conv3x3", coords.device):
        _check(load().oflow_flow_head2_tiled_s32(x.ptr, x.ps, x.ng, wr.data_ptr(), bias.data_ptr(), b, h, w,
                                                 coords.data_ptr(), _stream(coords.device)), what)


def flow_head_col2im(y: torch.Tensor, bias: torch.Tensor, coords: torch.Tensor) -> None:
    what = "flow_head_col2im"
    b, _, h, w = coords.shape
    if coords.dtype != torch.float32 or not coords.is_contiguous() or coords.shape[1] != 2 or coords.device.type != "cuda":
        raise RuntimeError(f"{what}: coords must be contiguous fp32 (B, 2, H, W) on the GPU")
    if y.dtype != torch.float32 or not y.is_contiguous() or tuple(y.shape) != (b, 18, h, w) or y.device != coords.device:
        raise RuntimeError(f"{what}: y must be contiguous fp32 ({b}, 18, {h}, {w})")
    if bias is None or bias.dtype != torch.float32 or tuple(bias.shape) != (2,) or bias.device != coords.device:
        raise RuntimeError(f"{what}: bias must be fp32 (2,) on the coords' device")
    with torch.cuda.device(coords.device), _Timed("flow_head_col2im", coords.device):
        _check(load().oflow_flow_head_col2im_f32(y.data_ptr(), bias.data_ptr(), b, h, w, coords.data_ptr(),
                                                 _stream(coords.device)), what)


FLOW_HEAD_SLABS = 4


def flow_head_fused_weights(weight: torch.Tensor) -> torch.Tensor:
    if tuple(weight.shape) != (2, 64 * FLOW_HEAD_SLABS, 3, 3):
        raise RuntimeError(f"flow_head_fused_weights: weight must be (2, {64 * FLOW_HEAD_SLABS}, 3, 3)")
    return weight.detach().float().permute(1, 2, 3, 0).reshape(FLOW_HEAD_SLABS, 64, 18).contiguous()


def flow_head_partial_empty(b: int, h: int, w: int, device) -> torch.Tensor:
    return torch.empty((FLOW_HEAD_SLABS, b, 18, h, w), device=device, dtype=torch.float32)


def conv_s32_flow_head(x: "S32Slice", cw: "ConvWeights", block_n: int, w2r: torch.Tensor, partial) -> None:
    what = "conv_s32_flow_head"
    if x.ng != cw.kg:
        raise RuntimeError(f"{what}: input has {x.ng} groups, weights expect {cw.kg}")
    b, h, w = x.bhw
    dev = x.device
    if (w2r.dtype != torch.float32 or not w2r.is_contiguous() or tuple(w2r.shape[1:]) != (64, 18) or w2r.device != dev):
        raise RuntimeError(f"{what}: w2r must be flow_head_fused_weights(conv2.weight) on the input's device")
    slabs, pp = 0, None
    if partial is not None:
        if (partial.dtype != torch.float32 or not partial.is_contiguous() or partial.dim() != 5
                or tuple(partial.shape[1:]) != (b, 18, h, w) or partial.device != dev):
            raise RuntimeError(f"{what}: partial must be contiguous fp32 (slabs, {b}, 18, {h}, {w}) on the input's device")
        slabs, pp = int(partial.shape[0]), partial.data_ptr()
    if w2r.shape[0] != FLOW_HEAD_SLABS:
        slabs = -1
    wf = cw.frag().data_ptr() if int(block_n) == 128 and cw.layout == "conv" else None
    if _flops is not None:
        n_exec = -(-cw.n_pad // int(block_n)) * int(block_n)
        _count(3 * 2 * b * h * w * n_exec * cw.kg * 32 * 9, 2 * b * h * w * cw.n * cw.cin * 9)
        fl = 2 * b * h * w * 2 * cw.n * 9
        _count(0, fl, fl)
    with torch.cuda.device(dev), _Timed("conv3x3", dev):
        _check(
            load().oflow_conv_s32_ex6(
                x.ptr, x.ps, cw.kg, cw.pack.data_ptr(), cw.n_pad, cw.wscale.data_ptr(),
                cw.bias.data_ptr() if cw.bias is not None else None, cw.n, b, h, w, cw.kh, cw.kw, int(block_n),
                3, ACT["relu"], 1.0, None, 0, None, 0, None, 0, 0, 0, None, None, 0, None, cw.n, None, None, 0, 0, 0,
                0, None, None, None, 0, wf, None, None, 0, w2r.data_ptr(), pp, slabs, _stream(dev),
            ),
            what,
        )


def flow_head_finish(partial: torch.Tensor, bias: torch.Tensor, coords: torch.Tensor, flow0=None, flow1=None) -> None:
    what = "flow_head_finish"
    if (coords.dtype != torch.float32 or coords.dim() != 4 or coords.shape[1] != 2 or not coords.is_contiguous()
            or coords.device.type != "cuda"):
        raise RuntimeError(f"{what}: coords must be contiguous fp32 (B, 2, H, W) on the GPU")
    b, _, h, w = coords.shape
    if (partial.dtype != torch.float32 or not partial.is_contiguous() or partial.dim() != 5
            or tuple(partial.shape[1:]) != (b, 18, h, w) or partial.device != coords.device):
        raise RuntimeError(f"{what}: partial must be contiguous fp32 (slabs, {b}, 18, {h}, {w})")
    if bias is None or bias.dtype != torch.float32 or tuple(bias.shape) != (2,) or bias.device != coords.device:
        raise RuntimeError(f"{what}: bias must be fp32 (2,) on the coords' device")
    for fl in (flow0, flow1):
        if fl is not None and (fl[0].bhw != (b, h, w) or fl[0].device != coords.device):
            raise RuntimeError(f"{what}: flow destination shape/device mismatch")
    f0 = (flow0[0].channel_ptr(flow0[1]), flow0[0].ps) if flow0 is not None else (None, 0)
    f1 = (flow1[0].channel_ptr(flow1[1]), flow1[0].ps) if flow1 is not None else (None, 0)
    with torch.cuda.device(coords.device), _Timed("flow_head_finish", coords.device):
        _check(load().oflow_flow_head_finish_f32(partial.data_ptr(), int(partial.shape[0]), bias.data_ptr(), b, h, w,
                                                 coords.data_ptr(), f0[0], f0[1], f1[0], f1[1],
                                                 _stream(coords.device)), what)


def stem_patches(img: torch.Tensor, out: torch.Tensor) -> torch.Tensor:
    x = _gpu_f32(img, "image", "stem_patches")
    b, c, h, w = x.shape
    if out.dtype != torch.float16 or tuple(out.shape[:3]) != (b, (h + 1) // 2, (w + 1) // 2):
        raise RuntimeError("stem_patches: output must be S32 (B, ceil(H/2), ceil(W/2), G, 2, 32)")
    with torch.cuda.device(x.device), _Timed("stem_patches", x.device):
        _check(load().oflow_stem_patches_s32(x.data_ptr(), b, c, h, w, out.data_ptr(), int(out.shape[3]), _stream(x.device)), "stem_patches")
    return out


def norm_stats(partials: torch.Tensor, b: int, tiles: int, n_pad: int, c: int, eps: float):
    alpha = torch.empty((b, c), device=partials.device, dtype=torch.float32)
    beta = torch.empty_like(alpha)
    with torch.cuda.device(partials.device):
        _check(
            load().oflow_norm_stats_finalize(partials.data_ptr(), b, tiles, n_pad, c, float(eps), alpha.data_ptr(), beta.data_ptr(), _stream(partials.device)),
            "norm_stats",
        )
    return alpha, beta


def norm_apply(x: torch.Tensor, shape, alpha, beta, act: str, y: S32Slice, res=None, res_raw=None, res_act: str = "none",
               s2d: bool = False, res_raw_relu: bool = False) -> None:
    b, c, h, w = shape
    mode, rp, rps = 0, None, 0
    x2 = a2 = b2 = None
    if res is not None:
        mode, rp, rps = 1, res.ptr, res.ps
    elif res_raw is not None:
        mode = 3 if res_raw_relu else 2
        x2, a2, b2 = (t.data_ptr() for t in res_raw)
    with torch.cuda.device(x.device), _Timed("norm_apply", x.device):
        _check(
            load().oflow_norm_apply_s32(
                x.data_ptr(), c, b, h, w, alpha.data_ptr(), beta.data_ptr(), ACT[act], mode, rp, rps, x2, a2, b2,
                ACT[res_act], int(bool(s2d)), y.ptr, y.ps, _stream(x.device),
            ),
            "norm_apply",
        )


def pack_s32(x: torch.Tensor, act: str, y0: S32Slice, y1=None, nhwc=None, dst_channel: int = 0) -> None:
    what = "pack_s32"
    if x.device.type != "cuda" or x.dtype != torch.float32 or x.dim() != 4:
        raise RuntimeError(f"{what}: expected a 4-D fp32 ROCm tensor")
    b, c, h, w = x.shape
    if x.stride(3) != 1 or x.stride(2) != w or x.stride(1) != h * w:
        raise RuntimeError(f"{what}: the (C, H, W) part must be contiguous")
    need = dst_channel + ((c + 7) // 8) * 8
    if dst_channel % 8 or y0.ng * 32 < need or (y1 is not None and y1.ng * 32 < need):
        raise RuntimeError(f"{what}: destination slice too narrow or dst_channel not a multiple of 8")
    if nhwc is not None and (nhwc.dtype != torch.float32 or not nhwc.is_contiguous() or nhwc.numel() != b * h * w * c):
        raise RuntimeError(f"{what}: nhwc copy must be contiguous fp32 [P, C]")
    with torch.cuda.device(x.device):
        _check(
            load().oflow_pack_s32_f32(
                x.data_ptr(), x.stride(0), c, b, h, w, ACT[act], int(dst_channel), y0.ptr, y0.ps,
                y1.ptr if y1 is not None else None, y1.ps if y1 is not None else 0,
                nhwc.data_ptr() if nhwc is not None else None, c, _stream(x.device),
            ),
            what,
        )


def normalize_images(image0: torch.Tensor, image1: torch.Tensor):
    what = "normalize_images"
    x0 = _gpu_f32(image0, "image0", what).contiguous()
    x1 = _gpu_f32(image1, "image1", what).contiguous()
    if x0.shape != x1.shape or x0.device != x1.device:
        raise RuntimeError(f"{what}: the frames must have the same shape and device")
    y0, y1 = torch.empty_like(x0), torch.empty_like(x1)
    n = x0.numel()
    with torch.cuda.device(x0.device):
        _check(load().oflow_normalize_images_f32(x0.data_ptr(), x1.data_ptr(), n, y0.data_ptr(), y1.data_ptr(),
                                                 _stream(x0.device)), what)
    return y0, y1


def replicate_pad(inputs, pad):
    what = "replicate_pad"
    xs = [_gpu_f32(x, "input", what).contiguous() for x in inputs]
    if not 1 <= len(xs) <= 4 or any(x.shape != xs[0].shape or x.device != xs[0].device for x in xs) or xs[0].dim() < 2:
        raise RuntimeError(f"{what}: 1..4 tensors of one shape (>= 2 dims) on one device")
    left, right, top, bottom = (int(v) for v in pad)
    *lead, h, w = xs[0].shape
    outs = [torch.empty((*lead, h + top + bottom, w + left + right), device=xs[0].device, dtype=torch.float32) for _ in xs]
    planes = xs[0].numel() // (h * w)
    src = (ctypes.c_void_p * len(xs))(*[x.data_ptr() for x in xs])
    dst = (ctypes.c_void_p * len(xs))(*[o.data_ptr() for o in outs])
    with torch.cuda.device(xs[0].device):
        _check(load().oflow_replicate_pad_f32(src, dst, len(xs), planes, h, w, top, bottom, left, right,
                                              _stream(xs[0].device)), what)
    return outs


def flow_prep(coords: torch.Tensor, patches: Optional[torch.Tensor], flow0=None, flow1=None) -> None:
    co = _gpu_f32(coords, "coords", "flow_prep")
    b, _, h, w = co.shape
    if patches is None and flow0 is None:
        raise RuntimeError("flow_prep: nothing to write")
    if patches is not None and (tuple(patches.shape) != (b, h, w, 4, 2, 32) or patches.dtype != torch.float16):
        raise RuntimeError("flow_prep: patches must be S32 (B, H, W, 4, 2, 32)")
    f0 = (flow0[0].channel_ptr(flow0[1]), flow0[0].ps) if flow0 is not None else (None, 0)
    f1 = (flow1[0].channel_ptr(flow1[1]), flow1[0].ps) if flow1 is not None else (None, 0)
    with torch.cuda.device(co.device), _Timed("flow_prep", co.device):
        _check(load().oflow_flow_prep_s32(co.data_ptr(), b, h, w, patches.data_ptr() if patches is not None else None,
                                          f0[0], f0[1], f1[0], f1[1], _stream(co.device)), "flow_prep")


def corr_lookup_backward(grad_out: torch.Tensor, coords: torch.Tensor, radius: int, level0_hw, num_levels: int):
    h0, w0 = level0_hw
    return list(ops().corr_lookup_backward(grad_out, coords, int(radius), int(h0), int(w0), int(num_levels)))


def corr_pyramid_backward(level_grads, fmap1: torch.Tensor, fmap2: torch.Tensor):
    return tuple(ops().corr_pyramid_backward(list(level_grads), fmap1, fmap2))


def corr_lookup_tiled_nhwc(pyr: TiledPyramid, coords: torch.Tensor, radius: int, out: torch.Tensor) -> torch.Tensor:
    co = _tensor(coords, "coords", "corr_lookup")
    _no_grad_input(co, "coords", "corr_lookup")
    _run("corr_lookup", co.device, ops().corr_lookup_tiled_nhwc, pyr.levels, co, int(radius), out)
    return out
```

Measured before the change: 452.0 image-pairs/s.

## Skip structurally-zero taps in space-to-depth 2x2 convs via a compact step list

A stride-2 3x3 conv rewritten as a 2x2 conv over space-to-depth input has taps whose packed weights are all zero. This adds a KS step-list mainloop that iterates only the nonzero (group, tap) pairs, 9 per four channel blocks instead of 16, using a compacted weight pack, so those MFMA steps and weight loads are skipped. It also adds an optional fused 1x1 shortcut conv launched as extra grid columns, plus a two-input norm-stats finalize, but the shortcut is off by default. The cost is a more complex hand-scheduled pipeline with parity and tap templates, plus extra kernel instantiations.

```diff
diff --git a/include/oflow.h b/include/oflow.h
--- a/include/oflow.h
+++ b/include/oflow.h
@@ -32,6 +32,8 @@
 #define OFLOW_IN_IMG7S2 3
 #define OFLOW_IN_FLOW7 4
 #define OFLOW_EPI_FLOW_HEAD 3
+#define OFLOW_KSTEPS_DENSE 0
+#define OFLOW_KSTEPS_S2D 1
 
 int oflow_abi_version(void);
 const char* oflow_status_string(int status);
@@ -169,9 +171,24 @@
                        long long addend_pixel_stride, const void* d_wfrag, float* d_ksplit_slab,
                        unsigned* d_ksplit_ctr, long long ksplit_tiles, const float* d_fh_weights, float* d_fh_partial,
                        int fh_slabs, void* stream);
+int oflow_conv_s32_ex7(const void* d_x, long long x_pixel_stride, int in_groups, const void* d_wpack, int n_pad,
+                       const float* d_wscale, const float* d_bias, int N, int B, int H, int W, int kh, int kw,
+                       int block_n, int epilogue, int activation, float out_scale, void* d_y0, long long y0_pixel_stride,
+                       void* d_y1, long long y1_pixel_stride, float* d_f32, long long f32_batch_stride,
+                       long long f32_channel_stride, int f32_accumulate, float* d_gru_h, float* d_gru_z,
+                       int gru_channels, float* d_nhwc, int nhwc_pixel_stride, float* d_stats, const void* d_res,
+                       long long res_pixel_stride, int res_activation, int s2d, int in_format,
+                       const float* d_in_scale, const float* d_in_shift, const float* d_addend,
+                       long long addend_pixel_stride, const void* d_wfrag, float* d_ksplit_slab,
+                       unsigned* d_ksplit_ctr, long long ksplit_tiles, int k_steps, int shortcut,
+                       const void* d_sc_wpack, const float* d_sc_wscale, const float* d_sc_bias, int sc_activation,
+                       void* d_sc_y0, long long sc_y0_pixel_stride, float* d_sc_nhwc, int sc_nhwc_pixel_stride,
+                       float* d_sc_stats, void* stream);
 int oflow_stem_patches_s32(const float* d_img, int B, int C, int H, int W, void* d_out, int out_groups, void* stream);
 int oflow_norm_stats_finalize(const float* d_partials, int B, int tiles, int n_pad, int C, double eps, float* d_alpha,
                               float* d_beta, void* stream);
+int oflow_norm_stats_finalize2(const float* d_partials, const float* d_partials2, int B, int tiles, int n_pad, int C,
+                               double eps, float* d_alpha, float* d_beta, float* d_alpha2, float* d_beta2, void* stream);
 int oflow_norm_apply_s32(const float* d_x, int C, int B, int H, int W, const float* d_alpha, const float* d_beta,
                          int activation, int res_mode, const void* d_res, long long res_pixel_stride, const float* d_x2,
                          const float* d_alpha2, const float* d_beta2, int res_activation, int s2d, void* d_y,
diff --git a/torch-optical-flow_amd/csrc/conv_s32.hip b/torch-optical-flow_amd/csrc/conv_s32.hip
--- a/torch-optical-flow_amd/csrc/conv_s32.hip
+++ b/torch-optical-flow_amd/csrc/conv_s32.hip
@@ -80,6 +80,21 @@
   long long ks_tiles;
   const float* fhw;
   float* fhy;
+  int ksteps;
+  int sc;
+  const uint8_t* sc_w;
+  const float* sc_wsc;
+  const float* sc_bias;
+  int sc_act;
+  uint8_t* sc_y0;
+  long long sc_y0ps;
+  float* sc_fn;
+  int sc_fnps;
+  float* sc_stats;
+};
+template <int V>
+struct IC {
+  static constexpr int value = V;
 };
 constexpr int kEpiFlowHead = OFLOW_EPI_FLOW_HEAD;
 constexpr int kInS32 = OFLOW_IN_S32, kInF32Norm = OFLOW_IN_F32_NORM, kInF32 = OFLOW_IN_F32, kInImg = OFLOW_IN_IMG7S2,
@@ -179,7 +194,8 @@
   }
 }
 
-template <int KH, int KW, int BN, int WM, int WN, int EPI, int TY = kTY, int AIN = kInS32, bool BREG = false, int BD = 1>
+template <int KH, int KW, int BN, int WM, int WN, int EPI, int TY = kTY, int AIN = kInS32, bool BREG = false, int BD = 1,
+          int KS = 0>
 __global__ __launch_bounds__(64 * WM * WN, WM * WN == 8 ? 1 : 2) void conv_s32_kernel(ConvArgs a) {
   constexpr int NTH = 64 * WM * WN;
   constexpr int T = KH * KW;
@@ -261,6 +277,30 @@
   tile /= a.tiles_x;
   const int ty0 = (tile % a.tiles_y) * TY;
   const int b = tile / a.tiles_y;
+  bool sc = false;
+  if constexpr (KS != 0) {
+    const int nblk = a.npad / BN;
+    if (cblk >= nblk) {
+      sc = true;
+      cblk -= nblk;
+      a.kg >>= 2;
+      a.w = a.sc_w;
+      a.wbytes = a.kg * a.npad * 128;
+      a.wsc = a.sc_wsc;
+      a.bias = a.sc_bias;
+      a.act = a.sc_act;
+      a.oscale = 1.0f;
+      a.y0 = a.sc_y0;
+      a.y0ps = a.sc_y0ps;
+      a.y1 = nullptr;
+      a.f = nullptr;
+      a.fn = a.sc_fn;
+      a.fnps = a.sc_fnps;
+      a.stats = a.sc_stats;
+      a.res = nullptr;
+      a.s2d = 0;
+    }
+  }
   const int n0 = cblk * BN;
   const long long pix0 = (long long)b * a.H * a.W;
 
@@ -376,12 +416,12 @@
     if (BITEMS % NTH == 0 || item < BITEMS)                                                                     \
       *reinterpret_cast<u32x4*>(sB + (BUF) * B_BYTES + n * RSB + ((c ^ bswz(n)) << 4)) = RB[s_];                    \
   }
-#define OFLOW_READ_OPS(AH, AL, BH, BL, I, S_)                                                                        \
+#define OFLOW_READ_OPS(AH, AL, BH, BL, I, S_) OFLOW_READ_OPS_T(AH, AL, BH, BL, (I) % T, (I) & 1, S_)
+#define OFLOW_READ_OPS_T(AH, AL, BH, BL, TAP_, PAR_, S_)                                                             \
   {                                                                                                                  \
-    const int ii_ = (I);                                                                                              \
-    const int t_ = ii_ % T, ky_ = t_ / KW, kx_ = t_ - ky_ * KW;                                                       \
-    const uint8_t* bufA_ = sA + (ADB ? (ii_ & 1) * A_BYTES : 0);                                                      \
-    const uint8_t* bufB_ = sB + (ii_ & 1) * B_BYTES;                                                                  \
+    const int t_ = (TAP_), ky_ = t_ / KW, kx_ = t_ - ky_ * KW;                                                        \
+    const uint8_t* bufA_ = sA + (ADB ? (PAR_) * A_BYTES : 0);                                                         \
+    const uint8_t* bufB_ = sB + (PAR_) * B_BYTES;                                                                     \
     const int chi_ = 2 * (S_) + hh, clo_ = 4 + 2 * (S_) + hh;                                                        \
     _Pragma("unroll") for (int mt_ = 0; mt_ < MT; ++mt_) {                                                           \
       const int p_ = (wm * MT + mt_ + ky_) * HX + r + kx_;                                                           \
@@ -412,7 +452,7 @@
 #pragma unroll
       for (int e = 0; e < 16; ++e) acc[i][j][e] = 0.f;
 
-  const int S = a.kg * T;
+  const int S = KS != 0 ? (sc ? a.kg : (a.kg >> 2) * 9) : a.kg * T;
   for (int c = tid; c < BN; c += NTH) {
     const int n = min(n0 + c, a.N - 1);
     sSB[c] = make_float2(a.wsc[n], a.bias ? a.bias[n] : 0.f);
@@ -629,8 +669,79 @@
   __syncthreads();
   half8 xah[MT], xal[MT], xbh[NT], xbl[NT];
   half8 yah[MT], yal[MT], ybh[NT], ybl[NT];
-  OFLOW_READ_OPS(xah, xal, xbh, xbl, 0, 0);
-
+  OFLOW_READ_OPS_T(xah, xal, xbh, xbl, KS != 0 ? 3 : 0, 0, 0);
+
+  if constexpr (KS != 0) {
+  static_assert(KH == 2 && KW == 2 && BD == 2 && !ADB && AIN == kInS32, "space-to-depth step list: LDS-staged 2x2 on S32 input");
+  constexpr int PS = KS == 2 ? 1 : 0, PQ = PS ^ 1;
+  const int GB = sc ? a.kg : a.kg >> 2;
+  int i_ = 0, g = 0;
+  auto step = [&](auto par_, auto tap_, auto ntap_, auto glast_) __attribute__((always_inline)) {
+    constexpr int P = decltype(par_)::value, TAP = decltype(tap_)::value, NTAP = decltype(ntap_)::value;
+    u32x4 (&rb)[BPER] = rbr[(P + 1) % BD];
+    OFLOW_WRITE_B(rb, (P + 1) & 1);
+    {
+      const int i2 = i_ + 1 + BD < S ? i_ + 1 + BD : S - 1;
+      OFLOW_LOAD_B(rb, i2);
+    }
+    OFLOW_READ_OPS_T(yah, yal, ybh, ybl, TAP, P, 1);
+    OFLOW_MFMAS(xah, xal, xbh, xbl);
+    if constexpr (decltype(glast_)::value != 0) {
+      __syncthreads();
+      OFLOW_WRITE_A(rar[0], 0, g + 1 < a.kg ? g + 1 : g);
+      const int g2 = g + 2 < a.kg ? g + 2 : a.kg - 1;
+      OFLOW_LOAD_A(rar[0], g2);
+      ++g;
+    }
+    if (!OFLOW_ABL(64)) __syncthreads();
+    OFLOW_READ_OPS_T(xah, xal, xbh, xbl, NTAP, (P + 1) & 1, 0);
+    OFLOW_MFMAS(yah, yal, ybh, ybl);
+    ++i_;
+  };
+  const IC<0> c0;
+  const IC<1> c1;
+  const IC<2> c2;
+  const IC<3> c3;
+  const IC<PS> ps;
+  const IC<PQ> pq;
+  {
+    const int npair = (GB - (KS == 2 ? 1 : 2)) >> 1;
+#pragma nounroll
+    for (int q = 0; q < npair; ++q) {
+      step(c0, c3, c3, c1);
+      step(c1, c3, c3, c1);
+    }
+    if constexpr (KS == 2) {
+      step(c0, c3, c2, c1);
+    } else {
+      step(c0, c3, c3, c1);
+      step(c1, c3, c2, c1);
+    }
+  }
+  if (!sc) {
+#pragma nounroll
+  for (int q = 1; q < GB; ++q) {
+    step(ps, c2, c3, c0);
+    step(pq, c3, c2, c1);
+  }
+  step(ps, c2, c3, c0);
+  step(pq, c3, c1, c1);
+#pragma nounroll
+  for (int q = 1; q < GB; ++q) {
+    step(ps, c1, c3, c0);
+    step(pq, c3, c1, c1);
+  }
+  step(ps, c1, c3, c0);
+  step(pq, c3, c0, c1);
+#pragma nounroll
+  for (int q = 0; q < GB; ++q) {
+    step(ps, c0, c1, c0);
+    step(pq, c1, c2, c0);
+    step(ps, c2, c3, c0);
+    step(pq, c3, c0, c1);
+  }
+  }
+  } else {
   constexpr int GPB2 = (BD > 1 && (T % BD) != 0) ? BD : 1;
   for (int g0 = 0; g0 < a.kg; g0 += GPB2) {
 #pragma unroll
@@ -662,8 +773,10 @@
     }
   }
   }
+  }
 #undef OFLOW_MFMAS
 #undef OFLOW_READ_OPS
+#undef OFLOW_READ_OPS_T
 #undef OFLOW_LOAD_A
 #undef OFLOW_WRITE_A
 #undef OFLOW_LOAD_B
@@ -1059,14 +1172,25 @@
   return OFLOW_XCD_MAP ? dim3(ntiles * (a.npad / bn)) : dim3(ntiles, a.npad / bn);
 }
 
-template <int KH, int KW, int BN, int WM, int WN, int EPI, int TY, int AIN>
+template <int KH, int KW, int BN, int WM, int WN, int EPI, int TY, int AIN, int KS = 0>
 void launch_staged(const ConvArgs& a, dim3 grid, hipStream_t s) {
-  hipLaunchKernelGGL((conv_s32_kernel<KH, KW, BN, WM, WN, EPI, TY, AIN, false, 2>), grid, dim3(64 * WM * WN), 0, s, a);
-}
-
-template <int KH, int KW, int BN, int WM, int WN, int EPI, int TY = kTY, bool BREG = false>
+  hipLaunchKernelGGL((conv_s32_kernel<KH, KW, BN, WM, WN, EPI, TY, AIN, false, 2, KS>), grid, dim3(64 * WM * WN), 0, s, a);
+}
+
+template <int KH, int KW, int BN, int WM, int WN, int EPI, int TY = kTY, bool BREG = false, int KS = 0>
 int launch_conv(const ConvArgs& a0, hipStream_t s) {
   ConvArgs a = a0;
+  if constexpr (KS != 0) {
+    if (a.ain != kInS32) return OFLOW_E_MODE;
+    a.tiles_y = (a.H + TY - 1) / TY;
+    dim3 grid = conv_grid(a, BN);
+    if (a.sc) {
+      if (OFLOW_XCD_MAP) return OFLOW_E_MODE;
+      grid.y *= 2;
+    }
+    launch_staged<KH, KW, BN, WM, WN, EPI, TY, kInS32, KS>(a, grid, s);
+    return launch_status();
+  } else
   if constexpr (BREG) {
     a.tiles_y = (a.H + TY - 1) / TY;
     dim3 grid = conv_grid(a, BN);
@@ -1125,6 +1249,19 @@
 
 template <int KH, int KW, int EPI>
 int launch_bn(const ConvArgs& a, int bn, hipStream_t s) {
+  if constexpr (KH == 2 && KW == 2 && EPI == 0) {
+    if (a.ksteps == OFLOW_KSTEPS_S2D) {
+      const bool odd = ((a.kg >> 2) & 1) != 0;
+      if (small_grid(a, bn))
+        return odd ? launch_conv<2, 2, 64, 2, 2, 0, 2, false, 2>(a, s) : launch_conv<2, 2, 64, 2, 2, 0, 2, false, 1>(a, s);
+      if (bn == 128)
+        return odd ? launch_conv<2, 2, 128, 2, 2, 0, kTY, false, 2>(a, s) : launch_conv<2, 2, 128, 2, 2, 0, kTY, false, 1>(a, s);
+      if (bn == 96)
+        return odd ? launch_conv<2, 2, 96, 4, 1, 0, kTY, false, 2>(a, s) : launch_conv<2, 2, 96, 4, 1, 0, kTY, false, 1>(a, s);
+      return OFLOW_E_SHAPE;
+    }
+  }
+  if (a.ksteps != OFLOW_KSTEPS_DENSE) return OFLOW_E_MODE;
   if (small_grid(a, bn)) return launch_conv<KH, KW, 64, 2, 2, EPI, 2>(a, s);
   if constexpr (KH * KW > 1 && KH * KW != 4)
     if (use_breg(a, bn, KH * KW)) {
@@ -1302,6 +1439,38 @@
                                   int s2d, int in_format, const float* d_in_scale, const float* d_in_shift,
                                   const float* d_addend, long long addend_pixel_stride, const void* d_wfrag,
                                   float* d_ksplit_slab, unsigned* d_ksplit_ctr, long long ksplit_tiles, void* stream) {
+  return oflow_conv_s32_ex7(d_x, x_pixel_stride, in_groups, d_wpack, n_pad, d_wscale, d_bias, N, B, H, W, kh, kw,
+                            block_n, epilogue, activation, out_scale, d_y0, y0_pixel_stride, d_y1, y1_pixel_stride,
+                            d_f32, f32_batch_stride, f32_channel_stride, f32_accumulate, d_gru_h, d_gru_z, gru_channels,
+                            d_nhwc, nhwc_pixel_stride, d_stats, d_res, res_pixel_stride, res_activation, s2d, in_format,
+                            d_in_scale, d_in_shift, d_addend, addend_pixel_stride, d_wfrag, d_ksplit_slab, d_ksplit_ctr,
+                            ksplit_tiles, OFLOW_KSTEPS_DENSE, 0, nullptr, nullptr, nullptr, 0, nullptr, 0, nullptr, 0,
+                            nullptr, stream);
+}
+
+extern "C" int oflow_conv_s32_ex7(const void* d_x, long long x_pixel_stride, int in_groups, const void* d_wpack,
+                                  int n_pad, const float* d_wscale, const float* d_bias, int N, int B, int H, int W, int kh,
+                                  int kw, int block_n, int epilogue, int activation, float out_scale, void* d_y0,
+                                  long long y0_pixel_stride, void* d_y1, long long y1_pixel_stride, float* d_f32,
+                                  long long f32_batch_stride, long long f32_channel_stride, int f32_accumulate,
+                                  float* d_gru_h, float* d_gru_z, int gru_channels, float* d_nhwc, int nhwc_pixel_stride,
+                                  float* d_stats, const void* d_res, long long res_pixel_stride, int res_activation,
+                                  int s2d, int in_format, const float* d_in_scale, const float* d_in_shift,
+                                  const float* d_addend, long long addend_pixel_stride, const void* d_wfrag,
+                                  float* d_ksplit_slab, unsigned* d_ksplit_ctr, long long ksplit_tiles, int k_steps,
+                                  int shortcut, const void* d_sc_wpack, const float* d_sc_wscale,
+                                  const float* d_sc_bias, int sc_activation, void* d_sc_y0,
+                                  long long sc_y0_pixel_stride, float* d_sc_nhwc, int sc_nhwc_pixel_stride,
+                                  float* d_sc_stats, void* stream) {
+  if (k_steps != OFLOW_KSTEPS_DENSE && k_steps != OFLOW_KSTEPS_S2D) return OFLOW_E_MODE;
+  if (shortcut != 0 && shortcut != 1) return OFLOW_E_MODE;
+  if (shortcut) {
+    if (k_steps != OFLOW_KSTEPS_S2D || sc_activation < 0 || sc_activation > 3) return OFLOW_E_MODE;
+    if (!d_sc_wpack || !d_sc_wscale || (!d_sc_y0 && !d_sc_nhwc && !d_sc_stats)) return OFLOW_E_NULL;
+    if (((uintptr_t)d_sc_wpack & 15) || (d_sc_y0 && ((sc_y0_pixel_stride & 127) || ((uintptr_t)d_sc_y0 & 15))) ||
+        (d_sc_nhwc && (sc_nhwc_pixel_stride < N || ((uintptr_t)d_sc_nhwc & 15) || (sc_nhwc_pixel_stride & 3))))
+      return OFLOW_E_ALIGN;
+  }
   ConvArgs a;
   const int st = build_conv_args(a, d_x, x_pixel_stride, in_groups, d_wpack, n_pad, d_wscale, d_bias, N, B, H, W, kh, kw,
                                  block_n, epilogue, activation, out_scale, d_y0, y0_pixel_stride, d_y1, y1_pixel_stride,
@@ -1315,6 +1484,24 @@
     a.wf = static_cast<const uint8_t*>(d_wfrag);
   }
   if (in_format < kInS32 || in_format > kInFlow) return OFLOW_E_MODE;
+  if (k_steps == OFLOW_KSTEPS_S2D) {
+    if (kh != 2 || kw != 2 || epilogue != 0 || in_format != kInS32 || d_ksplit_slab || d_ksplit_ctr) return OFLOW_E_MODE;
+    if (in_groups % 4 || (block_n != 96 && block_n != 128)) return OFLOW_E_SHAPE;
+    a.ksteps = k_steps;
+    a.wbytes = (in_groups / 4) * 9 * n_pad * 128;
+    if (shortcut) {
+      a.sc = 1;
+      a.sc_w = static_cast<const uint8_t*>(d_sc_wpack);
+      a.sc_wsc = d_sc_wscale;
+      a.sc_bias = d_sc_bias;
+      a.sc_act = sc_activation;
+      a.sc_y0 = static_cast<uint8_t*>(d_sc_y0);
+      a.sc_y0ps = sc_y0_pixel_stride;
+      a.sc_fn = d_sc_nhwc;
+      a.sc_fnps = sc_nhwc_pixel_stride;
+      a.sc_stats = d_sc_stats;
+    }
+  }
   if (in_format == kInFlow) {
     if (kh != 1 || kw != 1 || epilogue != 0 || block_n != 128 || in_groups != (kImgK * kImgK * 2 + 31) / 32)
       return OFLOW_E_MODE;
diff --git a/torch-optical-flow_amd/csrc/encoder_s32.hip b/torch-optical-flow_amd/csrc/encoder_s32.hip
--- a/torch-optical-flow_amd/csrc/encoder_s32.hip
+++ b/torch-optical-flow_amd/csrc/encoder_s32.hip
@@ -77,7 +77,13 @@
 constexpr int kStatWaves = 16;
 __global__ __launch_bounds__(64 * kStatWaves) void norm_stats_kernel(const float* __restrict__ part, int B, int tiles,
                                                                      int npad, int C, double eps, float* alpha,
-                                                                     float* beta) {
+                                                                     float* beta, const float* __restrict__ part2,
+                                                                     float* alpha2, float* beta2) {
+  if (blockIdx.y != 0) {
+    part = part2;
+    alpha = alpha2;
+    beta = beta2;
+  }
   __shared__ double sN[kStatWaves][64], sS[kStatWaves][64], sQ[kStatWaves][64];
   const int lane = threadIdx.x & 63, wave = threadIdx.x >> 6;
   const int cblocks = (C + 63) / 64;
@@ -213,7 +219,18 @@
   if (!d_partials || !d_alpha || !d_beta) return OFLOW_E_NULL;
   if (B <= 0 || tiles <= 0 || C <= 0 || n_pad < C) return OFLOW_E_SHAPE;
   hipLaunchKernelGGL(norm_stats_kernel, dim3(B * ((C + 63) / 64)), dim3(64 * kStatWaves), 0, static_cast<hipStream_t>(stream),
-                     d_partials, B, tiles, n_pad, C, eps, d_alpha, d_beta);
+                     d_partials, B, tiles, n_pad, C, eps, d_alpha, d_beta, nullptr, nullptr, nullptr);
+  return launch_status();
+}
+
+extern "C" int oflow_norm_stats_finalize2(const float* d_partials, const float* d_partials2, int B, int tiles, int n_pad,
+                                          int C, double eps, float* d_alpha, float* d_beta, float* d_alpha2,
+                                          float* d_beta2, void* stream) {
+  if (!d_partials || !d_alpha || !d_beta || !d_partials2 || !d_alpha2 || !d_beta2) return OFLOW_E_NULL;
+  if (B <= 0 || tiles <= 0 || C <= 0 || n_pad < C) return OFLOW_E_SHAPE;
+  hipLaunchKernelGGL(norm_stats_kernel, dim3(B * ((C + 63) / 64), 2), dim3(64 * kStatWaves), 0,
+                     static_cast<hipStream_t>(stream), d_partials, B, tiles, n_pad, C, eps, d_alpha, d_beta, d_partials2,
+                     d_alpha2, d_beta2);
   return launch_status();
 }
 
diff --git a/torch-optical-flow_amd/methods/raft/model/extractor.py b/torch-optical-flow_amd/methods/raft/model/extractor.py
--- a/torch-optical-flow_amd/methods/raft/model/extractor.py
+++ b/torch-optical-flow_amd/methods/raft/model/extractor.py
@@ -201,6 +201,22 @@
             return _native.NhwcNormIn(raw, *shape, alpha, beta)
         return _native.S32Slice(self._conv_norm(x, cw, shape, "relu"))
 
+    def _conv1_down(self, x, cw, down, shape):
+        b, h, w = shape
+        bn = self._bn(cw.n)
+        V = _native.S32Slice
+        dev = x.device
+        if self.inorm:
+            tiles = _native.conv_tiles(h, w)
+            raw, raw_d = (torch.empty((b * h * w, cw.n), device=dev, dtype=torch.float32) for _ in range(2))
+            part, part_d = (torch.empty((b, tiles, cw.n_pad, 3), device=dev, dtype=torch.float32) for _ in range(2))
+            _native.conv_s32(x, cw, bn, nhwc=raw, stats=part, shortcut=_native.Shortcut(down, nhwc=raw_d, stats=part_d))
+            (alpha, beta), (alpha_d, beta_d) = _native.norm_stats2(part, part_d, b, tiles, cw.n_pad, cw.n, 1e-5)
+            return _native.NhwcNormIn(raw, b, h, w, alpha, beta), (raw_d, alpha_d, beta_d)
+        out, out_d = (_native.s32_empty(b, h, w, (cw.n + 31) // 32, dev) for _ in range(2))
+        _native.conv_s32(x, cw, bn, act="relu", y0=V(out), shortcut=_native.Shortcut(down, y0=V(out_d)))
+        return V(out), V(out_d)
+
     def stem_patches(self, x: Tensor) -> Tensor:
         x = x.float().contiguous()
         n, _, hh, ww = x.shape
@@ -252,10 +268,13 @@
                     cur = self._conv_norm(t, self.w[pre + "conv2"], (n, h, w), "relu", res=x_in, s2d=out_s2d)
                 else:
                     h, w = h // 2, w // 2
-                    t = self._conv1(V(cur), self.w[pre + "conv1"], (n, h, w))
-                    cin = self.w[pre + "down"].kg
-                    d = self._conv_norm(V(cur, 0, cin), self.w[pre + "down"], (n, h, w), "none", raw_only=True)
-                    res = d if self.inorm else V(d)
+                    cw1, down = self.w[pre + "conv1"], self.w[pre + "down"]
+                    if _native.s2d_shortcut_fusable(cw1, down, self._bn(cw1.n)):
+                        t, res = self._conv1_down(V(cur), cw1, down, (n, h, w))
+                    else:
+                        t = self._conv1(V(cur), cw1, (n, h, w))
+                        d = self._conv_norm(V(cur, 0, down.kg), down, (n, h, w), "none", raw_only=True)
+                        res = d if self.inorm else V(d)
                     cur = self._conv_norm(t, self.w[pre + "conv2"], (n, h, w), "relu", res=res, s2d=out_s2d)
                 if out_s2d:
                     pass
diff --git a/torch-optical-flow_amd/optical_flow/_native.py b/torch-optical-flow_amd/optical_flow/_native.py
--- a/torch-optical-flow_amd/optical_flow/_native.py
+++ b/torch-optical-flow_amd/optical_flow/_native.py
@@ -76,6 +76,8 @@
     "oflow_flow_error_stats_f32",
     "oflow_sequence_loss_f32",
     "oflow_sequence_loss_backward_f32",
+    "oflow_conv_s32_ex7",
+    "oflow_norm_stats_finalize2",
 )
 
 _lib = None
@@ -263,6 +265,11 @@
     lib.oflow_timing_event_elapsed_ms.argtypes = [P, P, ctypes.POINTER(ctypes.c_float)]
     lib.oflow_flow_head_col2im_f32.restype = I
     lib.oflow_flow_head_col2im_f32.argtypes = [P, P, I, I, I, P, P]
+    lib.oflow_conv_s32_ex7.restype = I
+    lib.oflow_conv_s32_ex7.argtypes = (list(lib.oflow_conv_s32_ex5.argtypes[:-1])
+                                       + [I, I, P, P, P, I, P, L, P, I, P, P])
+    lib.oflow_norm_stats_finalize2.restype = I
+    lib.oflow_norm_stats_finalize2.argtypes = [P, P, I, I, I, I, ctypes.c_double, P, P, P, P, P]
     lib.oflow_conv_s32_ex6.restype = I
     lib.oflow_conv_s32_ex6.argtypes = list(lib.oflow_conv_s32_ex5.argtypes[:-1]) + [P, P, I, P]
     lib.oflow_flow_head_finish_f32.restype = I
@@ -593,6 +600,9 @@
 CONV_BREG = True
 CONV_BREG64 = False
 CONV_BREG32 = False
+CONV_S2D_SKIP = True
+CONV_S2D_SHORTCUT = False
+KSTEPS_DENSE, KSTEPS_S2D = 0, 1
 
 
 def _range_check(x, what: str) -> None:
@@ -839,9 +849,29 @@
     return v[..., :c].permute(0, 3, 1, 2).contiguous()
 
 
+def s2d_ksteps(kg: int):
+    if kg <= 0 or kg % 4:
+        raise RuntimeError("s2d_ksteps: the four channel blocks must be whole 32-channel groups")
+    gb = kg // 4
+    steps = []
+    for g in range(kg):
+        a, b = divmod(g // gb, 2)
+        for t in range(4):
+            kyp, kxp = divmod(t, 2)
+            if 0 <= 2 * kyp + a - 1 <= 2 and 0 <= 2 * kxp + b - 1 <= 2:
+                steps.append((g, t))
+    return steps
+
+
+def nonzero_ksteps(pack: torch.Tensor):
+    nz = (pack != 0).flatten(2).any(dim=2).cpu()
+    return [(g, t) for g in range(nz.shape[0]) for t in range(nz.shape[1]) if bool(nz[g, t])]
+
+
 class ConvWeights:
 
-    __slots__ = ("pack", "wscale", "bias", "n", "n_pad", "kh", "kw", "kg", "layout", "cin", "_frag")
+    __slots__ = ("pack", "wscale", "bias", "n", "n_pad", "kh", "kw", "kg", "layout", "cin", "_frag", "steps", "ksteps",
+                 "pack_steps")
 
     def __init__(self, weight: torch.Tensor, bias, n_pad: int, patches: bool = False):
         w = weight.detach().float()
@@ -871,6 +901,13 @@
         self.cin = c
         self.layout = "conv"
         self._frag = None
+        self.steps, self.ksteps, self.pack_steps = None, KSTEPS_DENSE, None
+        if kh == 2 and kw == 2 and kg % 4 == 0 and not patches:
+            self.steps = nonzero_ksteps(self.pack)
+            pattern = s2d_ksteps(kg)
+            if set(self.steps) <= set(pattern):
+                self.ksteps = KSTEPS_S2D
+                self.pack_steps = torch.stack([self.pack[g, t] for g, t in pattern]).contiguous()
         if t > 1 and n_pad % 32 == 0:
             self.frag()
 
@@ -943,9 +980,24 @@
         self.ctr = torch.zeros(2 * self.tiles, device=device, dtype=torch.int32)
 
 
+class Shortcut:
+
+    __slots__ = ("cw", "act", "y0", "nhwc", "stats")
+
+    def __init__(self, cw: "ConvWeights", act: str = "none", y0=None, nhwc=None, stats=None):
+        self.cw, self.act, self.y0, self.nhwc, self.stats = cw, act, y0, nhwc, stats
+
+
+def s2d_shortcut_fusable(cw: "ConvWeights", down: "ConvWeights", block_n: int) -> bool:
+    return (CONV_S2D_SKIP and CONV_S2D_SHORTCUT and cw.ksteps == KSTEPS_S2D and int(block_n) in (96, 128)
+            and cw.layout == "conv" and down.layout == "conv" and down.kh * down.kw == 1 and down.kg * 4 == cw.kg
+            and down.n == cw.n and down.n_pad == cw.n_pad)
+
+
 def conv_s32(x: S32Slice, cw: ConvWeights, block_n: int, act: str = "none", out_scale: float = 1.0, y0=None, y1=None,
              f32=None, f32_accumulate: bool = False, epilogue: int = 0, gru_h=None, gru_z=None, nhwc=None, stats=None,
-             res=None, res_act: str = "none", s2d: bool = False, addend=None, ksplit: "KSplit" = None) -> None:
+             res=None, res_act: str = "none", s2d: bool = False, addend=None, ksplit: "KSplit" = None,
+             shortcut: "Shortcut" = None) -> None:
     what = "conv_s32"
     if CHECK_RANGE:
         _range_check(x, f"{what} {cw.kh}x{cw.kw}")
@@ -991,10 +1043,25 @@
                                                  or (CONV_BREG32 and int(block_n) == 32))
           and cw.kh * cw.kw > 1 and not nin
           and in_format == 0 and cw.layout == "conv" else None)
+    ksteps = (KSTEPS_S2D if CONV_S2D_SKIP and cw.ksteps == KSTEPS_S2D and int(block_n) in (96, 128) and not epilogue
+              and in_format == 0 and not nin and cw.layout == "conv" and ksplit is None else KSTEPS_DENSE)
     if _flops is not None:
         taps, p_out = cw.kh * cw.kw, b * h * w
         n_exec = -(-cw.n_pad // int(block_n)) * int(block_n)
-        _count(3 * 2 * p_out * n_exec * cw.kg * 32 * taps, 2 * p_out * cw.n * cw.cin * taps)
+        steps = cw.pack_steps.shape[0] if ksteps == KSTEPS_S2D else cw.kg * taps
+        if shortcut is not None:
+            _count(3 * 2 * p_out * n_exec * shortcut.cw.kg * 32, 2 * p_out * cw.n * shortcut.cw.cin)
+        _count(3 * 2 * p_out * n_exec * steps * 32, 2 * p_out * cw.n * cw.cin * taps)
+    sc = shortcut
+    if sc is not None:
+        if ksteps != KSTEPS_S2D or not s2d_shortcut_fusable(cw, sc.cw, block_n):
+            raise RuntimeError(f"{what}: shortcut needs the space-to-depth step list and a 1x1 conv of the same N over its first channel block")
+        if sc.y0 is not None and (tuple(sc.y0.t.shape[:3]) != (b, h, w) or sc.y0.t.device != x.device):
+            raise RuntimeError(f"{what}: shortcut destination shape/device mismatch")
+        if sc.nhwc is not None and (sc.nhwc.dtype != torch.float32 or not sc.nhwc.is_contiguous() or sc.nhwc.numel() != b * h * w * cw.n):
+            raise RuntimeError(f"{what}: shortcut nhwc destination must be contiguous fp32 [P, {cw.n}]")
+        if sc.stats is not None and (sc.stats.dtype != torch.float32 or sc.stats.numel() < b * conv_tiles(h, w) * cw.n_pad * 3):
+            raise RuntimeError(f"{what}: shortcut stats partials buffer too small")
     ks_slab = ks_ctr = None
     ks_tiles = 0
     if ksplit is not None and wf is not None:
@@ -1004,8 +1071,8 @@
         ks_tiles = ksplit.tiles * (ksplit.block_n // int(block_n))
     with torch.cuda.device(dev), _Timed(f"conv{cw.kh}x{cw.kw}", dev):
         _check(
-            load().oflow_conv_s32_ex5(
-                x.ptr, x.ps, cw.kg, cw.pack.data_ptr(), cw.n_pad, cw.wscale.data_ptr(),
+            load().oflow_conv_s32_ex7(
+                x.ptr, x.ps, cw.kg, (cw.pack_steps if ksteps == KSTEPS_S2D else cw.pack).data_ptr(), cw.n_pad, cw.wscale.data_ptr(),
                 cw.bias.data_ptr() if cw.bias is not None else None, cw.n, b, h, w, cw.kh, cw.kw, int(block_n),
                 int(epilogue), ACT[act], float(out_scale), y0.ptr if y0 is not None else None, y0.ps if y0 is not None else 0,
                 y1.ptr if y1 is not None else None, y1.ps if y1 is not None else 0, fp or None, fbs, fcs,
@@ -1014,7 +1081,15 @@
                 stats.data_ptr() if stats is not None else None,
                 res.ptr if res is not None else None, res.ps if res is not None else 0, ACT[res_act], int(bool(s2d)),
                 in_format, x.scale.data_ptr() if nin else None, x.shift.data_ptr() if nin else None,
-                ap or None, aps, wf, ks_slab, ks_ctr, ks_tiles, _stream(dev),
+                ap or None, aps, wf, ks_slab, ks_ctr, ks_tiles, ksteps,
+                int(sc is not None), sc.cw.pack.data_ptr() if sc is not None else None,
+                sc.cw.wscale.data_ptr() if sc is not None else None,
+                sc.cw.bias.data_ptr() if sc is not None and sc.cw.bias is not None else None,
+                ACT[sc.act] if sc is not None else 0,
+                sc.y0.ptr if sc is not None and sc.y0 is not None else None,
+                sc.y0.ps if sc is not None and sc.y0 is not None else 0,
+                sc.nhwc.data_ptr() if sc is not None and sc.nhwc is not None else None, cw.n,
+                sc.stats.data_ptr() if sc is not None and sc.stats is not None else None, _stream(dev),
             ),
             what,
         )
@@ -1166,6 +1241,18 @@
     return alpha, beta
 
 
+def norm_stats2(partials: torch.Tensor, partials2: torch.Tensor, b: int, tiles: int, n_pad: int, c: int, eps: float):
+    out = [torch.empty((b, c), device=partials.device, dtype=torch.float32) for _ in range(4)]
+    with torch.cuda.device(partials.device):
+        _check(
+            load().oflow_norm_stats_finalize2(partials.data_ptr(), partials2.data_ptr(), b, tiles, n_pad, c, float(eps),
+                                              out[0].data_ptr(), out[1].data_ptr(), out[2].data_ptr(), out[3].data_ptr(),
+                                              _stream(partials.device)),
+            "norm_stats2",
+        )
+    return (out[0], out[1]), (out[2], out[3])
+
+
 def norm_apply(x: torch.Tensor, shape, alpha, beta, act: str, y: S32Slice, res=None, res_raw=None, res_act: str = "none",
                s2d: bool = False, res_raw_relu: bool = False) -> None:
     b, c, h, w = shape
```

After: 455.7 image-pairs/s (median of 6 runs). About the same (+0.8%).
